# kspalaiologos/bzip3

Hardware: AMD Instinct MI355X
Metric: MiB/s encode+decode round-trip, 8 MiB blocks (higher is better)
Workload: dtype u8

## Files before the change

### bzip3_amd/__init__.py

```python
import ctypes as C
import os

_HERE = os.path.dirname(os.path.abspath(__file__))
LIB_PATH = os.path.join(_HERE, "lib", "libbzip3.so")

BZ3_OK = 0
BZ3_ERR_OUT_OF_BOUNDS = -1
BZ3_ERR_BWT = -2
BZ3_ERR_CRC = -3
BZ3_ERR_MALFORMED_HEADER = -4
BZ3_ERR_TRUNCATED_DATA = -5
BZ3_ERR_DATA_TOO_BIG = -6
BZ3_ERR_INIT = -7
BZ3_ERR_DATA_SIZE_TOO_SMALL = -8

T_NAMES = ["crc", "rle", "lzp", "bwt", "cm", "copy", "_6", "_7"]

_lib = None


def _declare(L, strict=True):
    vp, i32, u32, sz = C.c_void_p, C.c_int32, C.c_uint32, C.c_size_t
    sig = {
        "bz3_version": (C.c_char_p, []),
        "bz3_last_error": (C.c_int8, [vp]),
        "bz3_strerror": (C.c_char_p, [vp]),
        "bz3_new": (vp, [i32]),
        "bz3_free": (None, [vp]),
        "bz3_bound": (sz, [sz]),
        "bz3_compress": (C.c_int, [u32, vp, vp, sz, C.POINTER(sz)]),
        "bz3_decompress": (C.c_int, [vp, vp, sz, C.POINTER(sz)]),
        "bz3_min_memory_needed": (sz, [i32]),
        "bz3_encode_block": (i32, [vp, vp, i32]),
        "bz3_decode_block": (i32, [vp, vp, sz, i32, i32]),
        "bz3_encode_blocks": (None, [vp, vp, vp, i32]),
        "bz3_decode_blocks": (None, [vp, vp, vp, vp, vp, i32]),
        "bz3_orig_size_sufficient_for_decode": (C.c_int, [vp, sz, i32]),
        "bz3_hip_device_count": (C.c_int, []),
        "bz3_hip_bind_device": (C.c_int, [C.c_int]),
        "bz3_hip_state_device": (C.c_int, [vp]),
        "bz3_hip_set_cm_mode": (C.c_int, [C.c_int]),
        "bz3_hip_cm_blocks_given_up": (C.c_uint, []),
        "bz3_hip_cm_blocks_routed_full": (C.c_uint, []),
        "bz3_hip_debug_bwt_big_rounds": (None, [C.c_int]),
        "bz3_hip_debug_peak_concurrent_groups": (C.c_int, [C.c_int]),
        "bz3_hip_debug_front_end_ring": (C.c_int, []),
        "bz3_hip_debug_arena_swap_buffers": (C.c_int, [C.c_int]),
        "bz3_hip_cm_variant_for": (C.c_int, [C.c_int, C.c_int, C.c_int]),
        "bz3_hip_set_lean_states": (C.c_int, [C.c_int]),
        "bz3_hip_release_cached_memory": (None, []),
        "bz3_hip_set_keep_workspace": (C.c_int, [C.c_int]),
        "bz3_hip_set_front_end_duo": (C.c_int, [C.c_int]),
        "bz3_hip_set_workspace_headroom": (None, [C.c_longlong]),
        "bz3_hip_workspace_headroom": (sz, []),
        "bz3_hip_debug_headroom_events": (C.c_uint, [C.c_int, C.POINTER(C.c_uint)]),
        "bz3_hip_debug_ring_contexts": (sz, [sz, sz, sz, sz, sz, sz, C.c_int, sz]),
        "bz3_hip_debug_arena_slack": (sz, [sz]),
        "bz3_hip_debug_cm_launches": (C.c_uint, [C.c_int]),
        "bz3_hip_debug_workspace_bytes": (sz, [sz, C.c_int]),
        "bz3_hip_debug_cached_bytes": (sz, [C.c_int]),
        "bz3_hip_encode_block_device": (i32, [vp, vp, i32]),
        "bz3_hip_decode_block_device": (i32, [vp, vp, sz, i32, i32]),
        "bz3_hip_encode_blocks_device": (None, [vp, vp, vp, i32]),
        "bz3_hip_decode_blocks_device": (None, [vp, vp, vp, vp, vp, i32]),
        "bz3_hip_compress_device": (C.c_int, [u32, vp, vp, sz, C.POINTER(sz)]),
        "bz3_hip_decompress_device": (C.c_int, [vp, vp, sz, C.POINTER(sz)]),
        "bz3_hip_frame_decoded_size_device": (C.c_int, [vp, sz, C.POINTER(sz)]),
        "bz3_hip_compress_device_many": (C.c_int, [u32, i32, C.POINTER(vp), C.POINTER(sz), C.POINTER(vp), C.POINTER(sz), C.POINTER(C.c_int)]),
        "bz3_hip_decompress_device_many": (C.c_int, [i32, C.POINTER(vp), C.POINTER(sz), C.POINTER(vp), C.POINTER(sz), C.POINTER(C.c_int)]),
        "bz3_hip_frame_decoded_sizes_device": (C.c_int, [i32, C.POINTER(vp), C.POINTER(sz), C.POINTER(sz), C.POINTER(C.c_int)]),
        "bz3_hip_debug_copy_segments": (i32, [vp, vp, C.POINTER(C.c_uint64), i32]),
        "bz3_hip_compress_device_planes": (C.c_int, [u32, u32, vp, vp, sz, C.POINTER(sz)]),
        "bz3_hip_decompress_device_planes": (C.c_int, [u32, vp, vp, sz, C.POINTER(sz)]),
        "bz3_hip_compress_device_planes_many": (C.c_int, [u32, i32, C.POINTER(u32), C.POINTER(vp), C.POINTER(sz), C.POINTER(vp), C.POINTER(sz), C.POINTER(C.c_int)]),
        "bz3_hip_decompress_device_planes_many": (C.c_int, [i32, C.POINTER(u32), C.POINTER(vp), C.POINTER(sz), C.POINTER(vp), C.POINTER(sz), C.POINTER(C.c_int)]),
        "bz3_hip_debug_planes": (i32, [vp, vp, C.POINTER(C.c_uint64), i32]),
        "bz3_hip_compress_device_delta": (C.c_int, [u32, u32, vp, vp, vp, sz, C.POINTER(sz)]),
        "bz3_hip_decompress_device_delta": (C.c_int, [u32, vp, vp, sz, vp, sz, C.POINTER(sz)]),
        "bz3_hip_compress_device_delta_many": (C.c_int, [u32, i32, C.POINTER(u32), C.POINTER(vp), C.POINTER(vp), C.POINTER(sz), C.POINTER(vp), C.POINTER(sz), C.POINTER(C.c_int)]),
        "bz3_hip_decompress_device_delta_many": (C.c_int, [i32, C.POINTER(u32), C.POINTER(vp), C.POINTER(sz), C.POINTER(vp), C.POINTER(sz), C.POINTER(vp), C.POINTER(sz), C.POINTER(C.c_int)]),
        "bz3_hip_crc32c_device": (C.c_int, [vp, sz, u32, C.POINTER(u32)]),
        "bz3_hip_debug_delta": (i32, [vp, vp, vp, C.POINTER(C.c_uint64), i32]),
        "bz3_hip_decompress_device_range": (C.c_int, [u32, vp, sz, C.c_uint64, vp, sz, vp, C.POINTER(sz)]),
        "bz3_hip_decompress_device_range_many": (C.c_int, [i32, C.POINTER(u32), C.POINTER(vp), C.POINTER(sz), C.POINTER(C.c_uint64), C.POINTER(vp), C.POINTER(sz),
                                                           C.POINTER(vp), C.POINTER(sz), C.POINTER(C.c_int)]),
        "bz3_hip_debug_range": (i32, [vp, vp, vp, C.POINTER(C.c_uint64), i32]),
        "bz3_hip_last_timings": (None, [vp, C.POINTER(C.c_float)]),
        "bz3_hip_last_bwt_stats": (None, [vp, C.POINTER(i32), C.POINTER(i32), C.POINTER(C.c_uint64)]),
        "bz3_hip_stage_crc32c": (u32, [vp, sz, u32]),
        "bz3_hip_stage_mrle_encode": (i32, [vp, i32, vp]),
        "bz3_hip_stage_mrle_decode": (C.c_int, [vp, vp, i32, i32]),
        "bz3_hip_stage_lzp_encode": (i32, [vp, i32, vp]),
        "bz3_hip_stage_lzp_decode": (i32, [vp, i32, vp, i32]),
        "bz3_hip_stage_bwt": (i32, [vp, vp, i32]),
        "bz3_hip_stage_unbwt": (i32, [vp, vp, i32, i32]),
        "bz3_hip_stage_last_ms": (C.c_float, []),
        "bz3_hip_debug_sort_u32": (i32, [vp, u32, C.c_int, C.c_int, vp, vp]),
        "bz3_hip_debug_scan_u32": (i32, [vp, u32, vp]),
        "bz3_hip_debug_cu_masks": (i32, [C.c_int, C.c_int, vp, vp]),
        "bz3_hip_set_collect_window_us": (None, [C.c_int]),
        "bz3_hip_debug_collected_batches": (C.c_uint, [C.c_int, C.POINTER(C.c_uint)]),
        "bz3_hip_stage_cm_encode": (i32, [vp, i32, vp]),
        "bz3_hip_stage_cm_decode": (None, [vp, i32, vp, i32]),
        "bz3_hip_stage_cm_decode_many": (C.c_float, [vp, i32, vp, i32, i32, vp]),
        "bz3_hip_stage_cm_encode_many": (C.c_float, [vp, i32, vp, C.POINTER(i32), i32]),
        "bz3_hip_encode_stream": (C.c_int, [C.c_int, C.c_int, i32, i32]),
        "bz3_hip_decode_stream": (C.c_int, [C.c_int, C.c_int, i32]),
    }
    for name, (res, args) in sig.items():
        if not strict and not hasattr(L, name):
            continue
        fn = getattr(L, name)
        fn.restype = res
        fn.argtypes = args
    return L


EXPORTED_SYMBOLS = None


def _share_hip_runtime_with_torch():
    if os.environ.get("BZ3_HIP_SYSTEM_RUNTIME") == "1":
        return
    try:
        import importlib.util

        spec = importlib.util.find_spec("torch")
        if spec is None or not spec.origin:
            return
        cand = os.path.join(os.path.dirname(spec.origin), "lib", "libamdhip64.so")
        if os.path.exists(cand):
            C.CDLL(cand, mode=C.RTLD_GLOBAL)
    except Exception:
        pass


def load(path=None):
    global _lib
    if _lib is not None and path is None:
        return _lib
    if path is None:
        _share_hip_runtime_with_torch()
    p = path or LIB_PATH
    if not os.path.exists(p):
        raise RuntimeError(
            f"{p} is missing: the HIP extension has not been built (python -m bzip3_amd.build). "
            "bzip3_amd has no CPU or PyTorch fallback by design."
        )
    L = _declare(C.CDLL(p), strict=path is None)
    if path is None:
        _lib = L
    return L


def _cbuf(data, cap):
    cap = max(1, cap)
    if len(data) == cap:
        return (C.c_uint8 * cap).from_buffer_copy(data)
    buf = (C.c_uint8 * cap)()
    if len(data):
        C.memmove(buf, data if isinstance(data, bytes) else bytes(data), len(data))
    return buf


class StageApi:

    def __init__(self, lib=None):
        self.lib = lib or load()

    def crc32c(self, data, init=1):
        return self.lib.bz3_hip_stage_crc32c(_cbuf(data, len(data)), len(data), init)

    def mrle_encode(self, data):
        out = (C.c_uint8 * (len(data) + 64))()
        n = self.lib.bz3_hip_stage_mrle_encode(_cbuf(data, len(data)), len(data), out)
        return C.string_at(out, n)

    def mrle_decode(self, data, outlen, maxin=None):
        maxin = len(data) if maxin is None else maxin
        out = (C.c_uint8 * max(1, outlen))()
        rc = self.lib.bz3_hip_stage_mrle_decode(_cbuf(data, len(data)), out, outlen, maxin)
        return rc, C.string_at(out, outlen)

    def lzp_encode(self, data):
        out = (C.c_uint8 * (len(data) + 64))()
        n = self.lib.bz3_hip_stage_lzp_encode(_cbuf(data, len(data)), len(data), out)
        return n, (C.string_at(out, n) if n > 0 else b"")

    def lzp_decode(self, data, maxout):
        out = (C.c_uint8 * max(8, maxout))()
        n = self.lib.bz3_hip_stage_lzp_decode(_cbuf(data, len(data)), len(data), out, maxout)
        return n, (C.string_at(out, n) if n > 0 else b"")

    def bwt(self, data):
        out = (C.c_uint8 * max(1, len(data)))()
        idx = self.lib.bz3_hip_stage_bwt(_cbuf(data, len(data)), out, len(data))
        return idx, C.string_at(out, len(data))

    def unbwt(self, data, idx):
        out = (C.c_uint8 * max(1, len(data)))()
        rc = self.lib.bz3_hip_stage_unbwt(_cbuf(data, len(data)), out, len(data), idx)
        return rc, C.string_at(out, len(data))

    def cm_encode(self, data):
        out = (C.c_uint8 * (len(data) + len(data) // 50 + 64))()
        n = self.lib.bz3_hip_stage_cm_encode(_cbuf(data, len(data)), len(data), out)
        return C.string_at(out, n)

    def cm_decode(self, data, n):
        out = (C.c_uint8 * max(1, n))()
        self.lib.bz3_hip_stage_cm_decode(_cbuf(data, len(data)), len(data), out, n)
        return C.string_at(out, n)


class State:

    def __init__(self, block_size, lib=None):
        self.lib = lib or load()
        self.block_size = block_size
        self.ptr = self.lib.bz3_new(block_size)
        if not self.ptr:
            raise RuntimeError(f"bz3_new({block_size}) returned NULL (invalid size, no HIP device, or out of device memory)")

    def close(self):
        if self.ptr:
            self.lib.bz3_free(self.ptr)
            self.ptr = None

    def __del__(self):
        try:
            self.close()
        except Exception:
            pass

    def __enter__(self):
        return self

    def __exit__(self, *a):
        self.close()

    @property
    def last_error(self):
        return self.lib.bz3_last_error(self.ptr)

    def strerror(self):
        return self.lib.bz3_strerror(self.ptr).decode()

    def timings(self):
        t = (C.c_float * 8)()
        self.lib.bz3_hip_last_timings(self.ptr, t)
        return {T_NAMES[i]: t[i] for i in range(6)}

    def bwt_stats(self):
        r, p, e = C.c_int32(), C.c_int32(), C.c_uint64()
        self.lib.bz3_hip_last_bwt_stats(self.ptr, C.byref(r), C.byref(p), C.byref(e))
        return {"rounds": r.value, "radix_passes": p.value, "sorted_elements": e.value}

    def encode_block(self, data):
        cap = self.lib.bz3_bound(max(len(data), self.block_size)) + 64
        buf = _cbuf(data, cap)
        n = self.lib.bz3_encode_block(self.ptr, buf, len(data))
        return n, self.last_error, (C.string_at(buf, n) if n > 0 else b"")

    def decode_block(self, data, orig_size, buffer_size=None, comp_size=None):
        cap = self.lib.bz3_bound(self.block_size) + 64
        buffer_size = cap if buffer_size is None else buffer_size
        comp_size = len(data) if comp_size is None else comp_size
        buf = _cbuf(data, max(cap, buffer_size, len(data) + 1))
        n = self.lib.bz3_decode_block(self.ptr, buf, buffer_size, comp_size, orig_size)
        return n, self.last_error, (C.string_at(buf, n) if n > 0 else b"")


def encode_block(data, block_size, lib=None):
    with State(block_size, lib) as st:
        return st.encode_block(data)


def decode_block(data, orig_size, block_size, lib=None, **kw):
    with State(block_size, lib) as st:
        return st.decode_block(data, orig_size, **kw)


class Bz3Error(RuntimeError):

    def __init__(self, code, what, out=None, index=None, codes=None, outs=None):
        super().__init__(f"{what} failed with {code} ({_ERR_NAMES.get(code, 'unknown error')})" + ("" if index is None else f" at frame {index}"))
        self.code = code
        self.out = out
        self.index = index
        self.codes = codes
        self.outs = outs


_ERR_NAMES = {v: k for k, v in globals().items() if k.startswith("BZ3_ERR_")}


def _device_u8(x, what):
    import torch

    if not isinstance(x, torch.Tensor) or x.device.type != "cuda" or x.dtype != torch.uint8 or not x.is_contiguous():
        raise TypeError(f"{what} must be a contiguous torch.uint8 tensor on a GPU")
    return x


def _planes_arg(planes, n):
    ks = [int(planes)] * n if isinstance(planes, int) else [int(k) for k in planes]
    if len(ks) != n:
        raise ValueError(f"planes: {len(ks)} element sizes for {n} tensors")
    for k in ks:
        if k not in (1, 2, 4, 8):
            raise ValueError(f"planes must be 1, 2, 4 or 8, not {k}")
    return ks


def _base_u8(base, x, what, same_size=True):
    if base is None:
        return None
    base = _device_u8(base, what)
    if base.device != x.device:
        raise ValueError(f"{what} is on {base.device}, the tensor on {x.device}")
    if same_size and base.numel() != x.numel():
        raise ValueError(f"{what} holds {base.numel()} bytes, the tensor {x.numel()}")
    return base


def _bases_arg(bases, n):
    bases = [None] * n if bases is None else list(bases)
    if len(bases) != n:
        raise ValueError(f"bases: {len(bases)} entries for {n} tensors")
    return bases


def _ptrs_or_null(ts):
    return (C.c_void_p * len(ts))(*[None if t is None else t.data_ptr() for t in ts])


def compress_tensor(x, block_size=16 << 20, lib=None, planes=1, base=None):
    import torch

    x = _device_u8(x, "x")
    (k,) = _planes_arg(planes, 1)
    base = _base_u8(base, x, "base")
    L = lib or load()
    n = x.numel()
    out = torch.empty(L.bz3_bound(n), dtype=torch.uint8, device=x.device)
    size = C.c_size_t(out.numel())
    torch.cuda.synchronize(x.device)
    rc = L.bz3_hip_compress_device_delta(block_size, k, C.c_void_p(x.data_ptr()), None if base is None else C.c_void_p(base.data_ptr()),
                                         C.c_void_p(out.data_ptr()), n, C.byref(size))
    if rc != BZ3_OK:
        raise Bz3Error(rc, "bz3_hip_compress_device_delta")
    return out[: size.value]


def decompress_tensor(frame, out=None, lib=None, planes=1, base=None):
    import torch

    frame = _device_u8(frame, "frame")
    (k,) = _planes_arg(planes, 1)
    base = _base_u8(base, frame, "base", same_size=False)
    L = lib or load()
    torch.cuda.synchronize(frame.device)
    if out is None:
        need = C.c_size_t(0)
        L.bz3_hip_frame_decoded_size_device(C.c_void_p(frame.data_ptr()), frame.numel(), C.byref(need))
        out = torch.empty(need.value, dtype=torch.uint8, device=frame.device)
    else:
        out = _device_u8(out, "out")
    size = C.c_size_t(out.numel())
    rc = L.bz3_hip_decompress_device_delta(k, C.c_void_p(frame.data_ptr()), None if base is None else C.c_void_p(base.data_ptr()),
                                           0 if base is None else base.numel(), C.c_void_p(out.data_ptr()), frame.numel(), C.byref(size))
    if rc != BZ3_OK:
        raise Bz3Error(rc, "bz3_hip_decompress_device_delta", out[: size.value])
    return out[: size.value]


def _same_device(ts, what):
    dev = ts[0].device
    for t in ts:
        if t.device != dev:
            raise ValueError(f"{what}: all tensors must be on one GPU ({dev} and {t.device})")
    return dev


def _ptrs(ts):
    return (C.c_void_p * len(ts))(*[t.data_ptr() for t in ts])


def _carve(total, sizes, device):
    import torch

    offs, o = [], 0
    for n in sizes:
        offs.append(o)
        o += (n + 15) & ~15
    buf = torch.empty(max(o, 1), dtype=torch.uint8, device=device)
    return [buf[a : a + n] for a, n in zip(offs, sizes)]


def _compress_many(L, xs, block_sizes, ks, dev, slack=False, bases=None):
    import torch

    n = len(xs)
    bases = _bases_arg(bases, n)
    caps = [L.bz3_bound(x.numel()) + ((13 + 8 * (x.numel() // _KiB65 + 2) + 15) & ~15 if slack else 0) for x in xs]
    outs = _carve(sum(caps), caps, dev)
    frames, codes = [None] * n, [BZ3_OK] * n
    torch.cuda.synchronize(dev)
    for bs in sorted(set(block_sizes)):
        idx = [i for i in range(n) if block_sizes[i] == bs]
        g = len(idx)
        out_sizes = (C.c_size_t * g)(*[caps[i] for i in idx])
        rcs = (C.c_int * g)()
        L.bz3_hip_compress_device_delta_many(bs, g, (C.c_uint32 * g)(*[ks[i] for i in idx]), _ptrs([xs[i] for i in idx]), _ptrs_or_null([bases[i] for i in idx]),
                                             (C.c_size_t * g)(*[xs[i].numel() for i in idx]), _ptrs([outs[i] for i in idx]), out_sizes, rcs)
        for j, i in enumerate(idx):
            frames[i], codes[i] = outs[i][: out_sizes[j]], rcs[j]
    if any(c != BZ3_OK for c in codes):
        idx = next(i for i, c in enumerate(codes) if c != BZ3_OK)
        raise Bz3Error(codes[idx], "bz3_hip_compress_device_delta_many", index=idx, codes=codes, outs=frames)
    return frames


def compress_tensors(xs, block_size=16 << 20, lib=None, planes=1, bases=None):
    xs = [_device_u8(x, f"xs[{i}]") for i, x in enumerate(xs)]
    if not xs:
        return []
    ks = _planes_arg(planes, len(xs))
    bases = [_base_u8(b, x, f"bases[{i}]") for i, (b, x) in enumerate(zip(_bases_arg(bases, len(xs)), xs))]
    dev = _same_device(xs, "compress_tensors")
    return _compress_many(lib or load(), xs, [block_size] * len(xs), ks, dev, bases=bases)


def decompress_tensors(frames, outs=None, lib=None, planes=1, bases=None):
    import torch

    frames = [_device_u8(f, f"frames[{i}]") for i, f in enumerate(frames)]
    if not frames:
        return []
    ks = _planes_arg(planes, len(frames))
    bases = [_base_u8(b, f, f"bases[{i}]", same_size=False) for i, (b, f) in enumerate(zip(_bases_arg(bases, len(frames)), frames))]
    dev = _same_device(frames, "decompress_tensors")
    L = lib or load()
    n = len(frames)
    in_ptrs = _ptrs(frames)
    in_sizes = (C.c_size_t * n)(*[f.numel() for f in frames])
    torch.cuda.synchronize(dev)
    if outs is None:
        need = (C.c_size_t * n)()
        rcs = (C.c_int * n)()
        L.bz3_hip_frame_decoded_sizes_device(n, in_ptrs, in_sizes, need, rcs)
        outs = _carve(sum(need), list(need), dev)
    else:
        outs = [_device_u8(o, f"outs[{i}]") for i, o in enumerate(outs)]
        if len(outs) != n:
            raise ValueError(f"decompress_tensors: {n} frames and {len(outs)} outputs")
        _same_device(frames + outs, "decompress_tensors")
    out_sizes = (C.c_size_t * n)(*[o.numel() for o in outs])
    rcs = (C.c_int * n)()
    rc = L.bz3_hip_decompress_device_delta_many(n, (C.c_uint32 * n)(*ks), in_ptrs, in_sizes, _ptrs_or_null(bases),
                                                (C.c_size_t * n)(*[0 if b is None else b.numel() for b in bases]), _ptrs(outs), out_sizes, rcs)
    res = [o[: out_sizes[i]] for i, o in enumerate(outs)]
    if rc != BZ3_OK:
        codes = list(rcs)
        idx = next(i for i, c in enumerate(codes) if c != BZ3_OK)
        raise Bz3Error(rc, "bz3_hip_decompress_device_delta_many", index=idx, codes=codes, outs=res)
    return res


def decompress_tensors_range(frames, offsets, nbytes, outs=None, planes=1, bases=None, lib=None):
    import torch

    frames = [_device_u8(f, f"frames[{i}]") for i, f in enumerate(frames)]
    n = len(frames)
    offsets, nbytes = [int(o) for o in offsets], [int(w) for w in nbytes]
    if len(offsets) != n or len(nbytes) != n:
        raise ValueError(f"decompress_tensors_range: {n} frames, {len(offsets)} offsets and {len(nbytes)} sizes")
    if any(o < 0 for o in offsets) or any(w < 0 for w in nbytes):
        raise ValueError("decompress_tensors_range: offsets and sizes must not be negative")
    if not frames:
        return []
    ks = _planes_arg(planes, n)
    bases = [_base_u8(b, f, f"bases[{i}]", same_size=False) for i, (b, f) in enumerate(zip(_bases_arg(bases, n), frames))]
    dev = _same_device(frames, "decompress_tensors_range")
    L = lib or load()
    if outs is None:
        outs = _carve(sum(nbytes), nbytes, dev)
    else:
        outs = [_device_u8(o, f"outs[{i}]") for i, o in enumerate(outs)]
        if len(outs) != n:
            raise ValueError(f"decompress_tensors_range: {n} frames and {len(outs)} outputs")
        _same_device(frames + outs, "decompress_tensors_range")
    for i, (o, b, w) in enumerate(zip(outs, bases, nbytes)):
        if o.numel() < w or (b is not None and b.numel() < w):
            raise ValueError(f"decompress_tensors_range: outs[{i}] / bases[{i}] hold fewer than the {w} bytes asked for")
    torch.cuda.synchronize(dev)
    out_sizes = (C.c_size_t * n)(*nbytes)
    rcs = (C.c_int * n)()
    rc = L.bz3_hip_decompress_device_range_many(n, (C.c_uint32 * n)(*ks), _ptrs(frames), (C.c_size_t * n)(*[f.numel() for f in frames]), (C.c_uint64 * n)(*offsets),
                                                _ptrs_or_null(bases), (C.c_size_t * n)(*[0 if b is None else w for b, w in zip(bases, nbytes)]), _ptrs(outs), out_sizes, rcs)
    res = [o[: out_sizes[i]] for i, o in enumerate(outs)]
    if rc != BZ3_OK:
        codes = list(rcs)
        idx = next(i for i, c in enumerate(codes) if c != BZ3_OK)
        raise Bz3Error(rc, "bz3_hip_decompress_device_range_many", index=idx, codes=codes, outs=res)
# ... 285 lines not shown
```

### bzip3_amd/csrc/api.hip

```cpp
#include <atomic>
#include <chrono>
#include <condition_variable>
#include <cstdio>
#include <cstdlib>
#include <exception>
#include <mutex>
#include <new>
#include <stdexcept>
#include <thread>
#include <type_traits>
#include <vector>

#include "../../include/bz3_hip.h"
#include "frame.hpp"
#include "planes.hpp"
#include "prims.hpp"
#include "sort.hpp"
#include "stages.hpp"

using namespace bz3;

namespace {

constexpr s32 KiB65 = 65 * 1024;
// ... 193 lines not shown
__attribute__((constructor)) static void bz3_hip_on_load() {
    const char * e = getenv("BZ3_HIP_SET_HW_QUEUES");
    if (!e || atoi(e) != 0) (void)setenv("GPU_MAX_HW_QUEUES", "8", 0);
}
#endif

int device_count() {
    std::lock_guard<std::mutex> lk(g_mu);
    if (g_device_count < 0) {
        int n = 0;
        if (hipGetDeviceCount(&n) != hipSuccess) n = 0;
        g_device_count = n;
        g_ctx.assign((size_t)(n > 0 ? n : 0), nullptr);
    }
    return g_device_count;
}

DeviceCtx * get_ctx(int dev) {
    const int n = device_count();
    if (dev < 0 || dev >= n) return nullptr;
    std::lock_guard<std::mutex> lk(g_mu);
    if (!g_ctx[dev]) {
        HIP_CHECK(hipSetDevice(dev));
        DeviceCtx * c = new DeviceCtx;
        c->device = dev;
        CrcTables t;
        memset(&t, 0, sizeof t);
        crc_build_tables(t);
        HIP_CHECK(hipMalloc((void **)&c->d_crc, sizeof(CrcTables)));
        HIP_CHECK(hipMemcpy(c->d_crc, &t, sizeof t, hipMemcpyHostToDevice));
#ifndef BZ3_EMU
        int cus = 0;
        if (hipDeviceGetAttribute(&cus, hipDeviceAttributeMultiprocessorCount, dev) == hipSuccess && cus > 0) c->cus = cus;
#endif
        if (const char * e = getenv("BZ3_HIP_CUS"))
            if (atoi(e) > 0) c->cus = atoi(e);
        g_ctx[dev] = c;
    }
    return g_ctx[dev];
}

int pick_device() {
    const int n = device_count();
    if (n <= 0) return -1;
    int b = g_bound_device.load();
    if (b == -2) {
        const char * e = getenv("BZ3_HIP_DEVICE");
        b = (e && *e) ? atoi(e) : -1;
        if (b >= n) b = -1;
        g_bound_device.store(b);
    }
    if (b >= 0) return b;
    return (int)(g_rr.fetch_add(1) % (unsigned)n);
}

size_t front_a_scratch_bytes(u64 n) { return (size_t)n * 30 + radix_temp_bytes(n, 9) + scan_temp_words(n / 8 + 4096) * 4 + (4u << 20); }
size_t front_b_scratch_bytes(u64 n) { return bwt_workspace_bytes(n) + (size_t)(n / 1024 + 4096) * 4; }
size_t workspace_bytes_for(u64 n) {
    size_t a = bwt_workspace_bytes(n), b = unbwt_workspace_bytes(n);
    size_t c = (size_t)n * 30 + radix_temp_bytes(n, 9) + scan_temp_words(n / 8 + 4096) * 4 + (4u << 20);
    size_t m = a > b ? a : b;
    return m > c ? m : c;
}

std::atomic<int> g_cm_mode{-2};

int cm_mode() {
    int m = g_cm_mode.load();
    if (m == -2) {
        const char * e = getenv("BZ3_HIP_CM_MODE");
        m = -1;
        if (e && !strcmp(e, "full")) m = CM_VARIANT_FULL;
        else if (e && !strcmp(e, "rows")) m = CM_VARIANT_ROWS;
        else if (e && !strcmp(e, "rows3")) m = CM_VARIANT_ROWS3;
#ifdef BZ3_EMU
        else if (e && !strcmp(e, "rows-test")) m = CM_VARIANT_ROWS_TEST;
#endif
        g_cm_mode.store(m);
    }
    return m;
}

bool lean_states() {
    int v = g_lean.load();
    if (v < 0) {
        const char * e = getenv("BZ3_HIP_LEAN");
        v = (e && *e && strcmp(e, "0")) ? 1 : 0;
        g_lean.store(v);
    }
    return v != 0;
}

int cm_variant_for(const DeviceCtx * ctx, size_t njobs, bool encode) {
    (void)encode;
    const int m = cm_mode();
    const size_t c = (size_t)ctx->cus;
    if (m >= 0) return m;
    if (njobs > 2 * c) return CM_VARIANT_ROWS3;
    if (njobs > c) return CM_VARIANT_ROWS;
    return CM_VARIANT_FULL;
}

size_t cm_scratch_bytes(size_t njobs) { return njobs * (CM_SPILL_BYTES + 256) + 4096 + CM_CLAIM_WORDS * 4 + 256; }

template <class Job, class Launch>
float run_cm_jobs(const DeviceCtx * ctx, Arena & arena, std::vector<Job> & jobs, Job * d_jobs, hipStream_t s, hipEvent_t ev0, hipEvent_t ev1, Launch && go,
                  const std::vector<char> * to_full = nullptr) {
    if (jobs.empty()) return 0.f;
    std::vector<Job> direct;
    if (to_full && cm_mode() < 0 && cm_variant_has_rows(cm_variant_for(ctx, jobs.size(), std::is_same<Job, CmEncodeJob>::value))) {
        std::vector<Job> keep;
        for (size_t i = 0; i < jobs.size(); i++) ((*to_full)[i] ? direct : keep).push_back(jobs[i]);
        if (!direct.empty()) {
            g_cm_routed_full.fetch_add((unsigned)direct.size());
            jobs.swap(keep);
        }
    }
    if (jobs.empty()) {
        float ms0 = 0.f;
        HIP_CHECK(hipMemcpyAsync(d_jobs, direct.data(), sizeof(Job) * direct.size(), hipMemcpyHostToDevice, s));
        HIP_CHECK(hipEventRecord(ev0, s));
        g_cm_launches.fetch_add(1);
        go(d_jobs, (u32)direct.size(), s, (int)CM_VARIANT_FULL);
        HIP_CHECK(hipEventRecord(ev1, s));
        HIP_CHECK(hipStreamSynchronize(s));
        (void)hipEventElapsedTime(&ms0, ev0, ev1);
        jobs.swap(direct);
        return ms0;
    }
    const int variant = cm_variant_for(ctx, jobs.size(), std::is_same<Job, CmEncodeJob>::value);
    const size_t mk = arena.mark();
    if constexpr (std::is_same<Job, CmEncodeJob>::value) {
        static const bool no_claim = getenv("BZ3_CM_NO_CLAIM") != nullptr;
        if (!no_claim) {
            u32 * claim = arena.take<u32>(CM_CLAIM_WORDS);
            HIP_CHECK(hipMemsetAsync(claim, 0, CM_CLAIM_WORDS * sizeof(u32), s));
            for (auto & j : jobs) j.claim = dev_addr(claim);
            for (auto & j : direct) j.claim = dev_addr(claim);
        }
    }
    u32 * d_status = nullptr;
    if (cm_variant_has_rows(variant)) {
        u8 * spill = arena.take<u8>(jobs.size() * CM_SPILL_BYTES);
        d_status = arena.take<u32>(jobs.size());
        HIP_CHECK(hipMemsetAsync(d_status, 0, jobs.size() * 4, s));
        for (size_t i = 0; i < jobs.size(); i++) {
            jobs[i].spill = dev_addr(spill + i * CM_SPILL_BYTES);
            jobs[i].status = dev_addr(d_status + i);
            jobs[i].miss_base = cm_variant_is_test(variant) ? 64u : CM_MISS_BASE;
            jobs[i].miss_shift = cm_variant_is_test(variant) ? 3u : CM_MISS_SHIFT;
        }
    }
    float ms = 0.f, ms2 = 0.f;
    HIP_CHECK(hipMemcpyAsync(d_jobs, jobs.data(), sizeof(Job) * jobs.size(), hipMemcpyHostToDevice, s));
    HIP_CHECK(hipEventRecord(ev0, s));
    g_cm_launches.fetch_add(1);
    go(d_jobs, (u32)jobs.size(), s, variant);
    HIP_CHECK(hipEventRecord(ev1, s));
    HIP_CHECK(hipStreamSynchronize(s));
    (void)hipEventElapsedTime(&ms, ev0, ev1);
    if (cm_variant_has_rows(variant)) {
        std::vector<u32> status(jobs.size());
        HIP_CHECK(hipMemcpyAsync(status.data(), d_status, jobs.size() * 4, hipMemcpyDeviceToHost, s));
        HIP_CHECK(hipStreamSynchronize(s));
        std::vector<Job> again;
        for (size_t i = 0; i < jobs.size(); i++)
            if (status[i]) again.push_back(jobs[i]);
        g_cm_given_up.fetch_add((unsigned)again.size());
        again.insert(again.end(), direct.begin(), direct.end());
        direct.clear();
        if (!again.empty()) {
            HIP_CHECK(hipMemcpyAsync(d_jobs, again.data(), sizeof(Job) * again.size(), hipMemcpyHostToDevice, s));
            HIP_CHECK(hipEventRecord(ev0, s));
            g_cm_launches.fetch_add(1);
            go(d_jobs, (u32)again.size(), s, (int)CM_VARIANT_FULL);
            HIP_CHECK(hipEventRecord(ev1, s));
            HIP_CHECK(hipStreamSynchronize(s));
            (void)hipEventElapsedTime(&ms2, ev0, ev1);
        }
    }
    if (!direct.empty()) {
        HIP_CHECK(hipMemcpyAsync(d_jobs, direct.data(), sizeof(Job) * direct.size(), hipMemcpyHostToDevice, s));
        HIP_CHECK(hipEventRecord(ev0, s));
        g_cm_launches.fetch_add(1);
        go(d_jobs, (u32)direct.size(), s, (int)CM_VARIANT_FULL);
        HIP_CHECK(hipEventRecord(ev1, s));
        HIP_CHECK(hipStreamSynchronize(s));
        float ms3 = 0.f;
        (void)hipEventElapsedTime(&ms3, ev0, ev1);
        ms2 += ms3;
    }
    arena.release(mk);
    return ms + ms2;
}

__global__ void k_write_header(u8 * __restrict__ b, const u32 * __restrict__ crc, const u32 * __restrict__ idx_word, u32 model, u32 lzp_size, u32 rle_size) {
    if (threadIdx.x != 0) return;
    const u32 c = *crc, idx = *idx_word;
    b[0] = (u8)c; b[1] = (u8)(c >> 8); b[2] = (u8)(c >> 16); b[3] = (u8)(c >> 24);
    b[4] = (u8)idx; b[5] = (u8)(idx >> 8); b[6] = (u8)(idx >> 16); b[7] = (u8)(idx >> 24);
    b[8] = (u8)model;
    u32 o = 9;
    if (model & 2u) { b[o] = (u8)lzp_size; b[o + 1] = (u8)(lzp_size >> 8); b[o + 2] = (u8)(lzp_size >> 16); b[o + 3] = (u8)(lzp_size >> 24); o += 4; }
    if (model & 4u) { b[o] = (u8)rle_size; b[o + 1] = (u8)(rle_size >> 8); b[o + 2] = (u8)(rle_size >> 16); b[o + 3] = (u8)(rle_size >> 24); }
}

__global__ void __launch_bounds__(64) k_store_small(u8 * __restrict__ b, u32 n, const u32 * __restrict__ crc) {
    const u32 t = threadIdx.x;
    const u8 v = t < n ? b[t] : (u8)0;
    __syncthreads();
    if (t < n) b[8 + t] = v;
    if (t == 0) {
        const u32 c = *crc;
        b[0] = (u8)c; b[1] = (u8)(c >> 8); b[2] = (u8)(c >> 16); b[3] = (u8)(c >> 24);
        b[4] = b[5] = b[6] = b[7] = 0xFF;
    }
}
__global__ void __launch_bounds__(128) k_unstore_small(u8 * __restrict__ b, u32 n) {
    const u32 t = threadIdx.x;
    const u8 v = t < n ? b[8 + t] : (u8)0;
    __syncthreads();
    if (t < n) b[t] = v;
}

}

struct bz3_state {
    s32 block_size = 0;
    s8 last_error = BZ3_OK;
    int device = 0;
    DeviceCtx * ctx = nullptr;
    hipStream_t stream = nullptr;
    hipStream_t xs = nullptr;
    u8 * d_swap = nullptr;
    bool lean = false;
    bool timed = true;
    u8 * d_io = nullptr;
    size_t cap = 0;
    u32 * d_words = nullptr;
    hipEvent_t ev0 = nullptr, ev1 = nullptr;
    float t[BZ3_HIP_T_COUNT] = {0};
    BwtStats bwt;

    enum Pending { NONE, ENC_STORED, ENC_CODED, DEC_STORED, DEC_CODED, FAILED } pending = NONE;
    u8 * user = nullptr;
    u8 * b1 = nullptr, * b2 = nullptr;
    s32 size = 0, overhead = 0, result = -1;
    u32 n_cm = 0;
    const u8 * cm_in = nullptr;
    u32 cm_in_size = 0;
    u8 * side = nullptr;
    bool hold_swap = false;
    bool skip = false;
    size_t buffer_size = 0;
    u32 crc = 0;
    s32 bwt_idx = 0, model = 0, lzp_size = -1, rle_size = -1, orig_size = 0, size_before_bwt = 0, size_src = 0;
};

namespace {

struct DeviceGuard {
    explicit DeviceGuard(int d) { HIP_CHECK(hipSetDevice(d)); }
};

struct DrainOnUnwind {
    hipStream_t main;
    hipStream_t * side;
    int n_side;
    int live = std::uncaught_exceptions();
    ~DrainOnUnwind() {
        if (std::uncaught_exceptions() > live) {
            if (main) (void)hipStreamSynchronize(main);
            for (int k = 0; k < n_side; k++)
                if (side[k]) (void)hipStreamSynchronize(side[k]);
        }
    }
};

void state_release(bz3_state * st) {
    if (!st) return;
    (void)hipSetDevice(st->device);
    if (st->stream) (void)hipStreamSynchronize(st->stream);
    if (st->ev0) (void)hipEventDestroy(st->ev0);
    if (st->ev1) (void)hipEventDestroy(st->ev1);
    if (st->d_swap && st->lean && st->ctx) st->ctx->temp_put(st->d_swap);
    else if (st->d_swap) (void)hipFree(st->d_swap);
    if (st->d_io) (void)hipFree(st->d_io);
    if (st->d_words) (void)hipFree(st->d_words);
    if (st->stream) (void)hipStreamDestroy(st->stream);
    delete st;
}

void ensure_io(bz3_state * st) {
    if (!st->d_io) HIP_CHECK(hipMalloc((void **)&st->d_io, st->cap));
}

u32 read_word(hipStream_t s, const u32 * d) {
    u32 v = 0;
    HIP_CHECK(hipMemcpyAsync(&v, d, 4, hipMemcpyDeviceToHost, s));
    HIP_CHECK(hipStreamSynchronize(s));
    return v;
}

inline bool sizes_fit(size_t buffer_size, s32 lzp_size, s32 rle_size, s32 orig_size) {
    const size_t a = lzp_size < 0 ? 0 : (size_t)lzp_size, b = rle_size < 0 ? 0 : (size_t)rle_size, c = orig_size < 0 ? 0 : (size_t)orig_size;
    return a <= buffer_size && b <= buffer_size && c <= buffer_size;
}

std::atomic<long long> g_ws_headroom{-1};
inline size_t ws_headroom() {
    static const long long env = [] {
        const char * e = getenv("BZ3_HIP_WS_HEADROOM_MB");
        return e && *e ? (long long)strtoull(e, nullptr, 10) << 20 : (long long)4 << 30;
    }();
    const long long v = g_ws_headroom.load();
    return (size_t)(v < 0 ? env : v);
}
inline size_t ring_contexts_for(size_t free_b, size_t have, size_t need, size_t fixed, size_t ctx_bytes, size_t cap, bool lean, size_t headroom) {
    const size_t total = free_b + have;
    const size_t base = need + fixed;
    if (total <= base || !ctx_bytes) return 0;
    size_t by_share = (total - base) / 10 * 7 / ctx_bytes;
    const size_t aside = headroom + ((size_t)513 << 20) + ((size_t)64 << 20);
    const size_t room = total > base + aside ? total - base - aside : 0;
    if (!lean) {
        const size_t by_room = room / ctx_bytes;
        return by_share < by_room ? by_share : by_room;
    }
    return room / (ctx_bytes + cap);
}
void enforce_headroom(DeviceCtx * ctx, hipStream_t s);

#ifndef BZ3_FRONT_DUO_DEFAULT
#define BZ3_FRONT_DUO_DEFAULT 0
#endif
std::atomic<int> g_keep_ws{-1};
inline bool keep_workspace() {
    static const bool env_on = [] {
        const char * e = getenv("BZ3_HIP_KEEP_WS");
        return e && atoi(e) != 0;
    }();
    const int v = g_keep_ws.load();
    return v < 0 ? env_on : v != 0;
}
std::atomic<int> g_front_duo{-1};
inline bool front_end_duo() {
    static const int env_on = [] {
        const char * e = getenv("BZ3_HIP_FRONT_DUO");
        return e ? (atoi(e) != 0 ? 1 : 0) : BZ3_FRONT_DUO_DEFAULT;
    }();
    const int v = g_front_duo.load();
    return v < 0 ? env_on != 0 : v != 0;
}
inline void lean_borrow(bz3_state * st) {
    if (st->lean && !st->d_swap) st->d_swap = st->ctx->temp_get(st->cap);
}
inline void lean_return(bz3_state * st) {
    if (st->lean && st->d_swap) {
        st->ctx->temp_put(st->d_swap);
        st->d_swap = nullptr;
    }
}
constexpr u32 CM_SIDE_BYTES = 64 * 1024;

void encode_front_a(bz3_state * st, u8 * buf, s32 data_size, Arena & arena, Arena & ctx_arena, LzpEncodeCtx & c) {
    st->pending = bz3_state::FAILED;
    st->result = -1;
    c.active = false;
    if (st->skip) return;
    if (data_size > st->block_size || data_size < 0) {
        st->last_error = BZ3_ERR_DATA_TOO_BIG;
        return;
    }
    hipStream_t s = st->xs;
    for (float & x : st->t) x = 0.f;
    double t0 = now_ms();
    crc32c_device(buf, (u64)data_size, 1u, st->ctx->d_crc, st->d_words, s);
    st->user = buf;
    st->size = data_size;
    if (data_size < 64) {
        launch(k_store_small, dim3(1), dim3(64), 0, s, buf, (u32)data_size, (const u32 *)(st->d_words + 1));
        st->pending = bz3_state::ENC_STORED;
        return;
    }
    if (st->timed) {
        HIP_CHECK(hipStreamSynchronize(s));
        st->t[BZ3_HIP_T_CRC] = (float)(now_ms() - t0);
    }

    u32 n = (u32)data_size;
    lean_borrow(st);
    u8 *b1 = buf, *b2 = st->d_swap;
    st->model = 0;
    st->rle_size = 0;
    t0 = now_ms();
    {
        MrleEncScratch sc;
        const size_t mk = arena.mark();
        mrle_encode_size(b1, n, sc, arena, s);
        st->rle_size = (s32)(32u + read_word(s, sc.total));
        if (st->rle_size < (s32)n) {
            mrle_encode_write(b1, n, sc, b2, s);
            if (st->timed) HIP_CHECK(hipStreamSynchronize(s));
            u8 * tmp = b1; b1 = b2; b2 = tmp;
            n = (u32)st->rle_size;
            st->model |= 4;
        }
        arena.release(mk);
    }
    st->t[BZ3_HIP_T_RLE] = (float)(now_ms() - t0);
    st->b1 = b1;
    st->b2 = b2;
    st->n_cm = n;
    t0 = now_ms();
    lzp_encode_prepare(b1, n, c, ctx_arena, arena, s);
    st->t[BZ3_HIP_T_LZP] = (float)(now_ms() - t0);
    st->pending = bz3_state::ENC_CODED;
}

void encode_front_b(bz3_state * st, Arena & arena, const LzpEncodeCtx & c, float driver_ms) {
    if (st->pending != bz3_state::ENC_CODED) return;
    st->pending = bz3_state::FAILED;
    hipStream_t s = st->xs;
    u8 *b1 = st->b1, *b2 = st->b2;
    u32 n = st->n_cm;
    double t0 = now_ms();
    const s32 lzp_size = lzp_encode_finish(c, b2, arena, s);
    if (lzp_size > 0 && lzp_size < (s32)n) {
        u8 * tmp = b1; b1 = b2; b2 = tmp;
        n = (u32)lzp_size;
        st->model |= 2;
    }
    st->lzp_size = lzp_size;
    st->t[BZ3_HIP_T_LZP] += driver_ms + (float)(now_ms() - t0);

    t0 = now_ms();
    u32 * const d_idx = st->d_words + 6;
    u32 * const d_out8 = st->d_words + 8;
    if (!st->lean) {
        (void)bwt_forward(b1, n, b2, arena, s, &st->bwt, d_idx, d_out8);
    } else {
        u8 * tail = st->user + bz3_bound((size_t)st->size) - n;
        if (b1 != st->user) {
            (void)bwt_forward(b1, n, tail, arena, s, &st->bwt, d_idx, d_out8);
        } else {
            (void)bwt_forward(b1, n, b2, arena, s, &st->bwt, d_idx, d_out8);
            HIP_CHECK(hipMemcpyAsync(tail, b2, n, hipMemcpyDeviceToDevice, s));
        }
        b1 = st->user;
        b2 = tail;
    }
    if (st->timed) {
        HIP_CHECK(hipStreamSynchronize(s));
        st->t[BZ3_HIP_T_BWT] = (float)(now_ms() - t0);
    }
    s32 overhead = 2;
    if (st->model & 2) overhead++;
    if (st->model & 4) overhead++;
    launch(k_write_header, dim3(1), dim3(64), 0, s, b1, (const u32 *)(st->d_words + 1), (const u32 *)d_idx, (u32)st->model, (u32)lzp_size, (u32)st->rle_size);
    if (st->lean && !st->hold_swap) lean_return(st);
    st->b1 = b1;
    st->b2 = b2;
    st->n_cm = n;
    st->overhead = overhead;
    st->pending = bz3_state::ENC_CODED;
}

void encode_finish(bz3_state * st, float cm_ms) {
    const bz3_state::Pending p = st->pending;
    st->pending = bz3_state::NONE;
    if (p == bz3_state::FAILED || p == bz3_state::NONE) return;
    HIP_CHECK(hipStreamSynchronize(st->xs));
    if (p == bz3_state::ENC_STORED) {
        st->result = st->size + 8;
        return;
    }
    st->t[BZ3_HIP_T_CM] = cm_ms;
    const u32 coded = read_word(st->xs, st->d_words + 2);
    if (coded == 0xFFFFFFFFu) {
        st->last_error = BZ3_ERR_BWT;
        return;
    }
    const s32 total = (s32)coded + st->overhead * 4 + 1;
    if (st->lean) {
        const u32 sw = read_word(st->xs, st->d_words + 3);
        if (sw != 0xFFFFFFFFu && coded > sw)
            HIP_CHECK(hipMemcpyAsync(st->user + st->overhead * 4 + 1 + sw, st->side, coded - sw, hipMemcpyDeviceToDevice, st->xs));
        HIP_CHECK(hipStreamSynchronize(st->xs));
    }
    st->last_error = BZ3_OK;
    if (st->b1 != st->user) {
        double t0 = now_ms();
        HIP_CHECK(hipMemcpyAsync(st->user, st->b1, (size_t)total, hipMemcpyDeviceToDevice, st->xs));
        HIP_CHECK(hipStreamSynchronize(st->xs));
        st->t[BZ3_HIP_T_COPY] += (float)(now_ms() - t0);
    }
    st->result = total;
}

std::atomic<unsigned> g_headroom_trims{0}, g_headroom_releases{0};
void enforce_headroom(DeviceCtx * ctx, hipStream_t s) {
    const size_t h = ws_headroom();
    size_t free_b = 0, total_b = 0;
    if (!h || hipMemGetInfo(&free_b, &total_b) != hipSuccess || free_b >= h) return;
    if (ctx->temp_idle_bytes() > 0) {
        ctx->temp_trim();
        g_headroom_trims.fetch_add(1);
        if (hipMemGetInfo(&free_b, &total_b) != hipSuccess || free_b >= h) return;
    }
    if (ctx->ws) {
        (void)hipStreamSynchronize(s);
        (void)hipDeviceSynchronize();
        (void)hipFree(ctx->ws);
        ctx->ws = nullptr;
        ctx->ws_cap = 0;
        g_headroom_releases.fetch_add(1);
    }
}

void pipeline_shape(s32 contexts, s32 n, s32 & window, s32 & ns) {
    if (contexts < 2) contexts = 2;
    ns = 2;
    for (s32 cand = DeviceCtx::RING_SLOTS; cand > 2; cand--)
        if (contexts / cand >= 3 && n >= cand * 3) {
            ns = cand;
            break;
        }
    window = contexts / ns;
    if (window > 8) window = 8;
    if (const char * e = getenv("BZ3_HIP_LZP_PIPE")) {
        int w = 0, q = 0;
        if (sscanf(e, "%d,%d", &w, &q) == 2 && w >= 1 && q >= 2 && q <= DeviceCtx::AUX) {
            window = w;
            ns = q;
        }
    }
    if (window > n) window = n;
    if (window < 1) window = 1;
}

void encode_group(bz3_state ** sts, u8 ** bufs, const s32 * sizes, s32 n) {
    if (n <= 0) return;
    bz3_state * lead = sts[0];
    DeviceGuard g(lead->device);
    std::lock_guard<std::mutex> lk(lead->ctx->mu);
    for (s32 i = 0; i < n; i++) {
        sts[i]->xs = lead->stream;
        sts[i]->timed = i == 0;
    }
    size_t need = 0, need_a = 0, need_b = 0;
    for (s32 i = 0; i < n; i++) {
        const u64 nb = (u64)(sizes[i] > 0 ? sizes[i] : 0) + 64;
        const size_t w = workspace_bytes_for(nb), wa = front_a_scratch_bytes(nb), wb = front_b_scratch_bytes(nb);
        if (w > need) need = w;
        if (wa > need_a) need_a = wa;
        if (wb > need_b) need_b = wb;
    }
    const bool duo_wanted = front_end_duo() && n >= 16;
    if (duo_wanted) need = need_a + need_b + 65536;
    u64 n_max = 64;
    for (s32 i = 0; i < n; i++)
        if (sizes[i] > 0 && (u64)sizes[i] > n_max) n_max = (u64)sizes[i];
    const size_t ctx_bytes = lzp_encode_ctx_bytes(n_max + 64) + 65536;
    const size_t headroom = ws_headroom();
    const size_t fixed = (size_t)n * (sizeof(CmEncodeJob) + CM_SIDE_BYTES + 256) + cm_scratch_bytes((size_t)n) + 65536 + (size_t)DeviceCtx::AUX * 8 * (sizeof(LzpDriverJob) + 256);
    size_t contexts = ((size_t)32 << 30) / ctx_bytes;
    {
        size_t free_b = 0, total_b = 0;
        const s32 full = DeviceCtx::RING_SLOTS * 8;
        if (lead->lean && lead->ctx->temp_idle_bytes() > 0 && hipMemGetInfo(&free_b, &total_b) == hipSuccess) {
            if (ring_contexts_for(free_b, lead->ctx->ws_cap, need, fixed, ctx_bytes, lead->cap, true, headroom) < (size_t)(n < full ? n : full)) lead->ctx->temp_trim();
        }
        if (hipMemGetInfo(&free_b, &total_b) == hipSuccess)
            contexts = ring_contexts_for(free_b, lead->ctx->ws_cap, need, fixed, ctx_bytes, lead->cap, lead->lean, headroom);
    }
    s32 window = 1, ns = 2;
    pipeline_shape((s32)(contexts < 1024 ? contexts : 1024), n, window, ns);
    lead->ctx->ensure_aux();
    hipStream_t s = lead->stream;
    DrainOnUnwind drain{s, lead->ctx->aux, DeviceCtx::AUX};
    static const bool front_rest = [] { const char * e = getenv("BZ3_HIP_FRONT_REST"); return e && atoi(e) != 0; }();
    if (front_rest && lead->ctx->rest && n > 1) {
        s = lead->ctx->rest;
        for (s32 i = 0; i < n; i++) sts[i]->xs = s;
    }
    DrainOnUnwind drain_rest{s == lead->stream ? nullptr : s, nullptr, 0};
    Arena arena;
    for (;;) {
        try {
            arena = lead->ctx->arena_for(need + (size_t)ns * (size_t)window * (ctx_bytes + sizeof(LzpDriverJob) + 256) +
                                         (size_t)n * (sizeof(CmEncodeJob) + CM_SIDE_BYTES + 256) + cm_scratch_bytes((size_t)n) + 65536);
            break;
        } catch (const HipError &) {
            if (ns == 2 && window == 1) throw;
            (void)hipGetLastError();
            if (ns > 2) ns = 2;
            else window = (window + 1) / 2;
        }
    }
    g_front_end_ring.store(window | (ns << 16));
    CmEncodeJob * d_jobs = arena.take<CmEncodeJob>((size_t)n);
    u8 * sides = arena.take<u8>((size_t)n * CM_SIDE_BYTES);
    struct Window {
        s32 w0 = 0, w1 = 0;
        Arena slot;
        LzpDriverJob * d_lz = nullptr;
        std::vector<LzpEncodeCtx> ctxs;
        std::vector<LzpDriverJob> lz;
    } win[DeviceCtx::AUX];
    for (int k = 0; k < ns; k++) {
        win[k].slot.base = arena.take<char>((size_t)window * ctx_bytes);
        win[k].slot.cap = (size_t)window * ctx_bytes;
        win[k].d_lz = arena.take<LzpDriverJob>((size_t)window);
    }
    std::vector<CmEncodeJob> jobs;
    std::vector<s32> job_owner;
    const s32 nwin = (n + window - 1) / window;
    const s32 lag = ns - 1;
    static const bool trace_rings = getenv("BZ3_HIP_TRACE_RINGS") != nullptr;
    double tr_prep = 0, tr_wait = 0, tr_fin = 0, tr_t0 = now_ms();
    auto prepare = [&](s32 k, hipStream_t sp, Arena & scr, hipEvent_t ev) {
        const int q = (int)(k % ns);
        Window & w = win[q];
        w.w0 = k * window;
        w.w1 = (w.w0 + window < n) ? w.w0 + window : n;
        w.slot.used = 0;
        w.ctxs.assign((size_t)(w.w1 - w.w0), LzpEncodeCtx());
        w.lz.clear();
        for (s32 i = w.w0; i < w.w1; i++) {
            sts[i]->xs = sp;
            sts[i]->hold_swap = false;
            encode_front_a(sts[i], bufs[i], sizes[i], scr, w.slot, w.ctxs[(size_t)(i - w.w0)]);
            if (sts[i]->pending == bz3_state::ENC_CODED && w.ctxs[(size_t)(i - w.w0)].active) w.lz.push_back(lzp_driver_job(w.ctxs[(size_t)(i - w.w0)]));
        }
        HIP_CHECK(hipEventRecord(ev, sp));
        if (!w.lz.empty()) {
            hipStream_t sq = lead->ctx->aux[q];
            HIP_CHECK(hipStreamWaitEvent(sq, ev, 0));
            HIP_CHECK(hipEventRecord(lead->ctx->ev_d0[q], sq));
            lzp_driver_batch(w.lz.data(), w.d_lz, (u32)w.lz.size(), sq);
            HIP_CHECK(hipEventRecord(lead->ctx->ev_d1[q], sq));
        }
    };
    auto finish = [&](s32 j, hipStream_t sf, Arena & scr, std::vector<bz3_state *> * held) {
        const int q = (int)(j % ns);
        Window & w = win[q];
        float driver_ms = 0.f;
        if (!w.lz.empty()) {
            const double t0 = now_ms();
            HIP_CHECK(hipEventSynchronize(lead->ctx->ev_d1[q]));
            (void)hipEventElapsedTime(&driver_ms, lead->ctx->ev_d0[q], lead->ctx->ev_d1[q]);
            tr_wait += now_ms() - t0;
        }
        for (s32 i = w.w0; i < w.w1; i++) {
            sts[i]->xs = sf;
            sts[i]->hold_swap = held != nullptr;
            encode_front_b(sts[i], scr, w.ctxs[(size_t)(i - w.w0)], driver_ms);
            sts[i]->hold_swap = false;
            if (sts[i]->pending == bz3_state::ENC_CODED) {
                CmEncodeJob j2{dev_addr(sts[i]->b2), dev_addr(sts[i]->b1 + sts[i]->overhead * 4 + 1), dev_addr(sts[i]->d_words + 2), sts[i]->n_cm, 0u};
                if (sts[i]->lean) {
                    sts[i]->side = sides + (size_t)i * CM_SIDE_BYTES;
                    j2.gap = (u32)(sts[i]->b2 - (sts[i]->b1 + sts[i]->overhead * 4 + 1));
                    j2.side = dev_addr(sts[i]->side);
                    j2.side_cap = CM_SIDE_BYTES;
                }
                jobs.push_back(j2);
                job_owner.push_back(i);
            }
            if (held) {
                if (sts[i]->lean && sts[i]->d_swap) held->push_back(sts[i]);
            } else {
                lean_return(sts[i]);
            }
        }
    };
    const bool duo = duo_wanted && nwin >= 3 && lead->ctx->aux_ready && s == lead->stream;
    if (!duo) {
        for (s32 k = 0; k < nwin + lag; k++) {
            const double tr_a = now_ms();
            if (k < nwin) prepare(k, s, arena, lead->ctx->ev_prep);
            const double tr_b = now_ms();
            tr_prep += tr_b - tr_a;
            if (k >= lag) finish(k - lag, s, arena, nullptr);
            tr_fin += now_ms() - tr_b;
        }
    } else {
        g_front_end_ring.fetch_or(1 << 29);
        hipStream_t sA = lead->ctx->duo;
        DrainOnUnwind drain_duo{sA, nullptr, 0};
        Arena scr_a;
        scr_a.base = arena.take<char>(need_a);
        scr_a.cap = need_a;
        struct Events {
            std::vector<hipEvent_t> e;
            ~Events() {
                for (hipEvent_t x : e)
                    if (x) (void)hipEventDestroy(x);
            }
        } evs;
        evs.e.assign((size_t)2 * (size_t)nwin, nullptr);
        for (auto & x : evs.e) HIP_CHECK(hipEventCreateWithFlags(&x, hipEventDisableTiming));
        hipEvent_t * evA = evs.e.data(), * evB = evs.e.data() + nwin;
        struct Shared {
            std::mutex m;
            std::condition_variable cv;
            s32 prepared = 0, finished = 0;
            bool abort = false;
            std::exception_ptr err;
            std::mutex pool;
            hipEvent_t last_return = nullptr;
            double prep_ms = 0;
        } sh;
        const int device = lead->device;
        std::thread ta([&] {
            try {
                DeviceGuard gd(device);
                for (s32 k = 0; k < nwin; k++) {
                    {
                        std::unique_lock<std::mutex> ul(sh.m);
                        sh.cv.wait(ul, [&] { return sh.abort || sh.finished >= k - ns + 1; });
                        if (sh.abort) return;
                    }
                    const double t0 = now_ms();
                    if (k >= ns) HIP_CHECK(hipStreamWaitEvent(sA, evB[k - ns], 0));
                    {
                        hipEvent_t ev = nullptr;
                        const s32 w0 = k * window, w1 = (w0 + window < n) ? w0 + window : n;
                        {
                            std::lock_guard<std::mutex> pl(sh.pool);
                            for (s32 i = w0; i < w1; i++) lean_borrow(sts[i]);
                            ev = sh.last_return;
                        }
                        if (ev) HIP_CHECK(hipStreamWaitEvent(sA, ev, 0));
                    }
                    prepare(k, sA, scr_a, evA[k]);
                    {
                        std::lock_guard<std::mutex> ul(sh.m);
                        sh.prepared = k + 1;
                        sh.prep_ms += now_ms() - t0;
                    }
                    sh.cv.notify_all();
                }
            } catch (...) {
                {
                    std::lock_guard<std::mutex> ul(sh.m);
                    sh.err = std::current_exception();
                    sh.abort = true;
                }
                sh.cv.notify_all();
            }
        });
        struct Joiner {
            std::thread & t;
            Shared & sh;
            int live = std::uncaught_exceptions();
            ~Joiner() {
                if (std::uncaught_exceptions() > live) {
                    std::lock_guard<std::mutex> ul(sh.m);
                    sh.abort = true;
                }
                sh.cv.notify_all();
                if (t.joinable()) t.join();
            }
        } joiner{ta, sh};
        std::vector<bz3_state *> held;
        for (s32 j = 0; j < nwin; j++) {
            const double tr_b = now_ms();
            {
                std::unique_lock<std::mutex> ul(sh.m);
                sh.cv.wait(ul, [&] { return sh.abort || sh.prepared >= j + 1; });
                if (sh.abort) break;
            }
            HIP_CHECK(hipStreamWaitEvent(s, evA[j], 0));
            held.clear();
            finish(j, s, arena, &held);
            HIP_CHECK(hipEventRecord(evB[j], s));
            {
                std::lock_guard<std::mutex> pl(sh.pool);
                for (bz3_state * st : held) lean_return(st);
                sh.last_return = evB[j];
            }
            {
                std::lock_guard<std::mutex> ul(sh.m);
                sh.finished = j + 1;
            }
            sh.cv.notify_all();
            tr_fin += now_ms() - tr_b;
        }
        ta.join();
        if (sh.err) std::rethrow_exception(sh.err);
        HIP_CHECK(hipStreamSynchronize(sA));
        tr_prep = sh.prep_ms;
        for (s32 i = 0; i < n; i++) sts[i]->xs = s;
    }
    if (trace_rings)
        fprintf(stderr, "[bz3 rings] encode front end: %d blocks, %d windows of %d x %d slots: %.1f ms = CRC / mRLE / LZP prepare %.1f + waiting for a window's LZP drivers %.1f + LZP emit / BWT / header %.1f\n",
                (int)n, (int)nwin, (int)window, (int)ns, now_ms() - tr_t0, tr_prep, tr_wait, tr_fin - tr_wait);
    if (s != lead->stream) {
        HIP_CHECK(hipStreamSynchronize(s));
        s = lead->stream;
        for (s32 i = 0; i < n; i++) sts[i]->xs = s;
    }
    std::vector<char> to_full(jobs.size(), 0);
    if (jobs.size() > (size_t)lead->ctx->cus) {
        std::vector<u32> outside(jobs.size(), 0u);
        for (size_t k = 0; k < jobs.size(); k++) HIP_CHECK(hipMemcpyAsync(&outside[k], sts[job_owner[k]]->d_words + 8, 4, hipMemcpyDeviceToHost, lead->stream));
        HIP_CHECK(hipStreamSynchronize(lead->stream));
        for (size_t k = 0; k < jobs.size(); k++) to_full[k] = outside[k] > jobs[k].n / 4u ? 1 : 0;
    }
    const float cm_ms = run_cm_jobs(lead->ctx, arena, jobs, d_jobs, lead->stream, lead->ev0, lead->ev1,
                                    [](const CmEncodeJob * j, u32 nj, hipStream_t st, int variant) { cm_encode_batch(j, nj, st, variant); }, &to_full);
    for (s32 i = 0; i < n; i++) encode_finish(sts[i], cm_ms);
    size_t slack = (size_t)16 << 30;
    if (const char * e = getenv("BZ3_HIP_WS_KEEP_MB")) slack = (size_t)strtoull(e, nullptr, 10) << 20;
    if (lead->ctx->ws_cap > 2 * need + slack && !(keep_workspace() && lead->lean)) {
        HIP_CHECK(hipStreamSynchronize(s));
        (void)hipFree(lead->ctx->ws);
        lead->ctx->ws = nullptr;
        lead->ctx->ws_cap = 0;
        g_front_end_ring.fetch_or(1 << 30);
    }
    enforce_headroom(lead->ctx, lead->stream);
}

void decode_front(bz3_state * st, u8 * buf, size_t buffer_size, s32 compressed_size, s32 orig_size, const u8 * hdr) {
    st->pending = bz3_state::FAILED;
    st->result = -1;
    if (st->skip) return;
    if (buffer_size < 9 || buffer_size < (size_t)compressed_size) {
        st->last_error = BZ3_ERR_DATA_SIZE_TOO_SMALL;
        return;
    }
    const u32 crc = rd_le32(hdr);
    const s32 bwt_idx = (s32)rd_le32(hdr + 4);
    const size_t bound = bz3_bound((size_t)st->block_size);
    if (compressed_size < 0 || (size_t)compressed_size > bound) {
        st->last_error = BZ3_ERR_MALFORMED_HEADER;
        return;
    }
    hipStream_t s = st->xs;
    for (float & x : st->t) x = 0.f;
    st->user = buf;
    st->buffer_size = buffer_size;
    st->crc = crc;
    if (bwt_idx == -1) {
        if (compressed_size - 8 > 64 || compressed_size < 8) {
            st->last_error = BZ3_ERR_MALFORMED_HEADER;
            return;
        }
        if ((size_t)(compressed_size - 8) > buffer_size) {
            st->last_error = BZ3_ERR_DATA_SIZE_TOO_SMALL;
            return;
        }
        st->size = compressed_size - 8;
        launch(k_unstore_small, dim3(1), dim3(128), 0, s, buf, (u32)st->size);
        crc32c_device(buf, (u64)st->size, 1u, st->ctx->d_crc, st->d_words, s);
        st->pending = bz3_state::DEC_STORED;
        return;
    }
    const s32 model = (s8)hdr[8];
    const size_t need = 9 + (size_t)((model & 2) * 4) + (size_t)((model & 4) * 4);
    if (buffer_size < need) {
        st->last_error = BZ3_ERR_DATA_SIZE_TOO_SMALL;
        return;
    }
    s32 lzp_size = -1, rle_size = -1, p = 0;
    if (model & 2) lzp_size = (s32)rd_le32(hdr + 9 + 4 * p++);
    if (model & 4) rle_size = (s32)rd_le32(hdr + 9 + 4 * p++);
    p += 2;
    compressed_size -= p * 4 + 1;
    if (((model & 2) && (lzp_size < 0 || (size_t)lzp_size > bound)) || ((model & 4) && (rle_size < 0 || (size_t)rle_size > bound))) {
        st->last_error = BZ3_ERR_MALFORMED_HEADER;
        return;
    }
    if (orig_size < 0 || (size_t)orig_size > bound) {
        st->last_error = BZ3_ERR_MALFORMED_HEADER;
        return;
    }
    const s32 size_before_bwt = (model & 2) ? lzp_size : (model & 4) ? rle_size : orig_size;
    if (!sizes_fit(buffer_size, lzp_size, rle_size, orig_size)) {
        st->last_error = BZ3_ERR_DATA_SIZE_TOO_SMALL;
        return;
    }
    st->bwt_idx = bwt_idx;
    st->model = model;
    st->lzp_size = lzp_size;
    st->rle_size = rle_size;
    st->orig_size = orig_size;
    st->size_before_bwt = size_before_bwt;
    st->cm_in = buf + p * 4 + 1;
    st->cm_in_size = (u32)(compressed_size < 0 ? 0 : compressed_size);
    st->pending = bz3_state::DEC_CODED;
}

bool decode_unbwt(bz3_state * st, Arena & arena, float cm_ms) {
    hipStream_t s = st->xs;
    st->t[BZ3_HIP_T_CM] = cm_ms;
    const s32 n = st->size_before_bwt;
    if (st->bwt_idx > n) {
        st->last_error = BZ3_ERR_MALFORMED_HEADER;
        return false;
    }
    u8 *b1 = st->d_swap, *b2 = st->user;
    if (st->lean) {
        b1 = st->user;
        b2 = st->d_swap;
    }
    const double t0 = now_ms();
    if (n <= 1) {
        if (st->bwt_idx != n) { st->last_error = BZ3_ERR_BWT; return false; }
        if (n == 1) HIP_CHECK(hipMemcpyAsync(b2, b1, 1, hipMemcpyDeviceToDevice, s));
    } else {
        if (st->bwt_idx <= 0) { st->last_error = BZ3_ERR_BWT; return false; }
        bwt_inverse(b1, (u32)n, (u32)st->bwt_idx, b2, arena, s);
    }
    st->b1 = b2;
    st->b2 = b1;
    st->size_src = n;
    st->t[BZ3_HIP_T_BWT] = (float)(now_ms() - t0);
    return true;
}

void decode_finish(bz3_state * st, Arena & arena) {
    hipStream_t s = st->xs;
    const size_t bound = bz3_bound((size_t)st->block_size);
    (void)bound;
    u8 *b1 = st->b1, *b2 = st->b2;
    s32 size_src = st->size_src;
    if (st->model & 2) {
        size_src = (s32)read_word(s, st->d_words + 5);
        if (size_src == -1) { st->last_error = BZ3_ERR_CRC; return; }
        if ((size_t)size_src > st->buffer_size) { st->last_error = BZ3_ERR_DATA_SIZE_TOO_SMALL; return; }
        u8 * tmp = b1; b1 = b2; b2 = tmp;
    }
    if (st->model & 4) {
        const double t0 = now_ms();
        bool bad = size_src < 32;
        if (!bad) {
            mrle_decode(b1, (u32)size_src, b2, (u32)st->orig_size, st->d_words + 4, arena, s);
            bad = read_word(s, st->d_words + 4) != (u32)st->orig_size;
        }
        st->t[BZ3_HIP_T_RLE] = (float)(now_ms() - t0);
        if (bad) { st->last_error = BZ3_ERR_CRC; return; }
        size_src = st->orig_size;
        u8 * tmp = b1; b1 = b2; b2 = tmp;
    }
    st->last_error = BZ3_OK;
    if (size_src > st->block_size || size_src < 0) {
        st->last_error = BZ3_ERR_MALFORMED_HEADER;
        return;
    }
    if (b1 != st->user) {
        const double t0 = now_ms();
        HIP_CHECK(hipMemcpyAsync(st->user, b1, (size_t)size_src, hipMemcpyDeviceToDevice, s));
        HIP_CHECK(hipStreamSynchronize(s));
        st->t[BZ3_HIP_T_COPY] += (float)(now_ms() - t0);
    }
    const double t0 = now_ms();
    crc32c_device(st->user, (u64)size_src, 1u, st->ctx->d_crc, st->d_words, s);
    const u32 got = read_word(s, st->d_words + 1);
    st->t[BZ3_HIP_T_CRC] = (float)(now_ms() - t0);
    if (got != st->crc) {
        st->last_error = BZ3_ERR_CRC;
        return;
    }
    st->result = size_src;
}

void decode_group(bz3_state ** sts, u8 ** bufs, const size_t * buffer_sizes, const s32 * sizes, const s32 * orig_sizes, const u8 * hdrs, s32 n) {
    if (n <= 0) return;
    bz3_state * lead = sts[0];
    DeviceGuard g(lead->device);
    std::lock_guard<std::mutex> lk(lead->ctx->mu);
    hipStream_t s = lead->stream;
    for (s32 i = 0; i < n; i++) sts[i]->xs = s;
    size_t need = 0;
    bool any_lean = false;
    for (s32 i = 0; i < n; i++) {
        const size_t w = workspace_bytes_for(bz3_bound((size_t)sts[i]->block_size) + 64);
        if (w > need) need = w;
        any_lean = any_lean || sts[i]->lean;
    }
    std::vector<s32> coded;
    for (s32 i = 0; i < n; i++) {
        decode_front(sts[i], bufs[i], buffer_sizes[i], sizes[i], orig_sizes[i], hdrs + 17 * (size_t)i);
        if (sts[i]->pending == bz3_state::DEC_CODED) coded.push_back(i);
    }
    auto stage_bytes = [&](s32 i) { return sts[i]->lean ? (((size_t)sts[i]->cm_in_size + 64 + 255) & ~(size_t)255) : (size_t)0; };
    size_t stage_budget = (size_t)48 << 30;
    {
        size_t free_b = 0, total_b = 0;
        if (any_lean && hipMemGetInfo(&free_b, &total_b) == hipSuccess) {
            const size_t have = lead->ctx->ws_cap;
            const size_t aside = need + ws_headroom() + ((size_t)577 << 20);
            const size_t room = free_b + have > aside ? free_b + have - aside : 0;
            stage_budget = room - room / 4;
        }
    }
    std::vector<size_t> round_end;
    size_t max_round = 0;
    for (size_t k = 0; k < coded.size();) {
        size_t bytes = 0, e = k;
        while (e < coded.size() && (e == k || bytes + stage_bytes(coded[e]) <= stage_budget)) bytes += stage_bytes(coded[e++]);
        round_end.push_back(e);
        if (bytes > max_round) max_round = bytes;
        k = e;
    }
    s32 tail_slots = n >= 128 ? 4 : 2;
    s32 tail_window = tail_slots == 4 ? 16 : 32;
    if (tail_slots == 4) {
        size_t cap_max = 0;
        for (s32 i = 0; i < n; i++)
            if (sts[i]->lean && sts[i]->cap > cap_max) cap_max = sts[i]->cap;
        const size_t cap_al = (cap_max + 255) & ~(size_t)255;
        size_t free_b = 0, total_b = 0;
        const bool have_info = hipMemGetInfo(&free_b, &total_b) == hipSuccess;
        for (s32 w : {30, 25, 20}) {
            if (n < 4 * w || lead->ctx->reserved_cus_wanted() < 64) continue;
            const size_t bufs = (size_t)4 * (size_t)w;
            const bool from_arena = keep_workspace() && any_lean && lead->ctx->ws_cap >= need + need / 16 + bufs * cap_al + ((size_t)64 << 20);
            if (!any_lean || from_arena || (have_info && free_b >= bufs * cap_max + ws_headroom() + ((size_t)2 << 30) + max_round)) {
                tail_window = w;
                break;
            }
        }
    }
    lead->ctx->ensure_aux();
    if (const char * e = getenv("BZ3_HIP_TAIL_PIPE")) {
        int w = 0, q = 0;
        if (sscanf(e, "%d,%d", &w, &q) == 2 && w >= 1 && q >= 2 && q <= DeviceCtx::AUX) {
            tail_window = w;
            tail_slots = q;
        }
    }
    if (tail_window > n) tail_window = n;
    size_t lzp_in_window = 0;
    for (s32 w0 = 0; w0 < n; w0 += tail_window) {
        size_t c = 0;
        for (s32 i = w0; i < n && i < w0 + tail_window; i++)
            if (sts[i]->pending == bz3_state::DEC_CODED && (sts[i]->model & 2)) c++;
        if (c > lzp_in_window) lzp_in_window = c;
    }
    Arena arena = lead->ctx->arena_for(need + (size_t)tail_slots * lzp_in_window * (LZP_LUT_WORDS * 4 + sizeof(LzpDecodeJob) + 256) + (size_t)n * 256 + cm_scratch_bytes(coded.size()) + max_round + 65536);
    float cm_ms = 0.f;
    for (size_t r = 0, k0 = 0; r < round_end.size(); k0 = round_end[r++]) {
        const size_t mk = arena.mark();
        std::vector<CmDecodeJob> cm_jobs;
        std::vector<char> to_full;
        for (size_t k = k0; k < round_end[r]; k++) {
            bz3_state * st = sts[coded[k]];
            to_full.push_back((u64)st->cm_in_size * 10u >= (u64)(u32)st->size_before_bwt * 9u ? 1 : 0);
            const u8 * in = st->cm_in;
            if (st->lean) {
                u8 * stage = arena.take<u8>(stage_bytes(coded[k]));
                if (st->cm_in_size) HIP_CHECK(hipMemcpyAsync(stage, st->cm_in, st->cm_in_size, hipMemcpyDeviceToDevice, s));
                in = stage;
            }
            cm_jobs.push_back(CmDecodeJob{dev_addr(in), dev_addr(st->lean ? st->user : st->d_swap), st->cm_in_size, (u32)st->size_before_bwt, 0u, 0u});
        }
        CmDecodeJob * d_jobs = arena.take<CmDecodeJob>(cm_jobs.size());
        cm_ms += run_cm_jobs(lead->ctx, arena, cm_jobs, d_jobs, s, lead->ev0, lead->ev1,
                             [](const CmDecodeJob * j, u32 nj, hipStream_t st, int variant) { cm_decode_batch(j, nj, st, variant); }, &to_full);
        arena.release(mk);
    }
    struct TailWindow {
        s32 w0 = 0, w1 = 0;
        std::vector<LzpDecodeJob> lz_jobs;
        std::vector<s32> lz_owner;
        std::vector<char> alive;
        LzpDecodeJob * d_lz = nullptr;
        u32 * luts = nullptr;
    } tw[DeviceCtx::AUX];
    for (int k = 0; k < tail_slots; k++) {
        tw[k].d_lz = lzp_in_window ? arena.take<LzpDecodeJob>(lzp_in_window) : nullptr;
        tw[k].luts = lzp_in_window ? arena.take<u32>(lzp_in_window * LZP_LUT_WORDS) : nullptr;
    }
    std::vector<u8 *> arena_swaps;
    size_t swap_cap = 0;
    if (keep_workspace() && any_lean) {
        for (s32 i = 0; i < n; i++)
            if (sts[i]->lean && sts[i]->cap > swap_cap) swap_cap = sts[i]->cap;
        const size_t want = (size_t)tail_slots * (size_t)tail_window;
        const size_t step = (swap_cap + 255) & ~(size_t)255;
        const size_t keep_free = need + need / 32 + 65536;
        while (swap_cap && arena_swaps.size() < want && arena.cap - arena.used >= keep_free + step) arena_swaps.push_back(arena.take<u8>(swap_cap));
    }
    std::vector<char> from_arena((size_t)n, 0);
    auto borrow = [&](s32 i) {
        bz3_state * st = sts[i];
        if (st->lean && !st->d_swap && !arena_swaps.empty() && st->cap <= swap_cap) {
            st->d_swap = arena_swaps.back();
            arena_swaps.pop_back();
            from_arena[(size_t)i] = 1;
            g_arena_swaps.fetch_add(1);
        } else {
            lean_borrow(st);
        }
    };
    auto give_back = [&](s32 i) {
        bz3_state * st = sts[i];
        if (from_arena[(size_t)i]) {
            if (st->d_swap) arena_swaps.push_back(st->d_swap);
            st->d_swap = nullptr;
            from_arena[(size_t)i] = 0;
        } else {
            lean_return(st);
        }
    };
    lead->ctx->ensure_aux();
    DrainOnUnwind drain{s, lead->ctx->aux, DeviceCtx::AUX};
    hipStream_t s_cm = s;
    hipStream_t * side_streams = lead->ctx->aux;
    static const s32 part_min = [] { const char * e = getenv("BZ3_HIP_CU_PARTITION_MIN_BLOCKS"); return e && atoi(e) > 0 ? (s32)atoi(e) : (s32)128; }();
    if (lead->ctx->rest && n >= part_min && tail_slots <= DeviceCtx::RING_SLOTS) {
        side_streams = lead->ctx->aux_m;
        HIP_CHECK(hipStreamSynchronize(s));
        s = lead->ctx->rest;
        for (s32 i = 0; i < n; i++) sts[i]->xs = s;
    }
    DrainOnUnwind drain_rest{s == s_cm ? nullptr : s, side_streams == lead->ctx->aux ? nullptr : side_streams, side_streams == lead->ctx->aux ? 0 : DeviceCtx::AUX};
    const s32 nwin = (n + tail_window - 1) / tail_window;
    const s32 lag = tail_slots - 1;
    static const bool trace_rings = getenv("BZ3_HIP_TRACE_RINGS") != nullptr;
    double tr_unbwt = 0, tr_wait = 0, tr_finish = 0, tr_t0 = now_ms();
    for (s32 k = 0; k < nwin + lag; k++) {
        const double tr_a = now_ms();
        if (k < nwin) {
            const int q = (int)(k % tail_slots);
            hipStream_t s2 = side_streams[q];
            TailWindow & w = tw[q];
            w.w0 = k * tail_window;
            w.w1 = (w.w0 + tail_window < n) ? w.w0 + tail_window : n;
            w.lz_jobs.clear();
            w.lz_owner.clear();
            w.alive.assign((size_t)(w.w1 - w.w0), 0);
            for (s32 i = w.w0; i < w.w1; i++) {
                bz3_state * st = sts[i];
                if (st->pending == bz3_state::DEC_STORED) {
                    HIP_CHECK(hipStreamSynchronize(st->xs));
                    if (read_word(st->xs, st->d_words + 1) != st->crc) st->last_error = BZ3_ERR_CRC;
                    else st->result = st->size;
                    continue;
                }
                if (st->pending != bz3_state::DEC_CODED) continue;
                borrow(i);
                if (!decode_unbwt(st, arena, cm_ms)) continue;
                w.alive[(size_t)(i - w.w0)] = 1;
                if (st->model & 2) {
                    if (st->lzp_size < 4) {
                        st->last_error = BZ3_ERR_CRC;
                        w.alive[(size_t)(i - w.w0)] = 0;
                        continue;
                    }
                    const size_t bound = bz3_bound((size_t)st->block_size);
                    const size_t room = st->lean && st->buffer_size < bound ? st->buffer_size : bound;
                    w.lz_jobs.push_back(LzpDecodeJob{dev_addr(st->b1), dev_addr(st->b2), dev_addr(w.luts + w.lz_jobs.size() * LZP_LUT_WORDS), dev_addr(st->d_words + 5),
                                                     (u32)st->lzp_size, (u32)room});
                    w.lz_owner.push_back(i);
                }
            }
            if (!w.lz_jobs.empty()) {
                HIP_CHECK(hipEventRecord(lead->ctx->ev_prep, s));
                HIP_CHECK(hipStreamWaitEvent(s2, lead->ctx->ev_prep, 0));
                HIP_CHECK(hipEventRecord(lead->ctx->ev_d0[q], s2));
                lzp_decode_batch(w.lz_jobs.data(), w.d_lz, (u32)w.lz_jobs.size(), s2);
                HIP_CHECK(hipEventRecord(lead->ctx->ev_d1[q], s2));
            }
        }
        const double tr_b = now_ms();
        tr_unbwt += tr_b - tr_a;
        if (k >= lag) {
            const int q = (int)((k - lag) % tail_slots);
            TailWindow & w = tw[q];
            if (!w.lz_jobs.empty()) {
                HIP_CHECK(hipEventSynchronize(lead->ctx->ev_d1[q]));
                tr_wait += now_ms() - tr_b;
                float ms = 0.f;
                (void)hipEventElapsedTime(&ms, lead->ctx->ev_d0[q], lead->ctx->ev_d1[q]);
                for (s32 i : w.lz_owner) sts[i]->t[BZ3_HIP_T_LZP] = ms;
                for (size_t j = 0; j < w.lz_jobs.size(); j++) {
                    bz3_state * st = sts[w.lz_owner[j]];
                    const size_t bound = bz3_bound((size_t)st->block_size);
                    if (!st->lean || st->buffer_size >= bound || read_word(s, st->d_words + 5) != w.lz_jobs[j].max_out) continue;
                    u8 * big = st->ctx->temp_get(st->cap);
                    LzpDecodeJob again = w.lz_jobs[j];
                    again.out = dev_addr(big);
                    again.max_out = (u32)bound;
                    again.lut = dev_addr(w.luts);
                    lzp_decode_batch(&again, w.d_lz, 1u, s);
                    HIP_CHECK(hipStreamSynchronize(s));
                    st->ctx->temp_put(big);
                }
            }
            for (s32 i = w.w0; i < w.w1; i++) {
                if (w.alive[(size_t)(i - w.w0)]) decode_finish(sts[i], arena);
                give_back(i);
            }
        }
        tr_finish += now_ms() - tr_b;
    }
    if (trace_rings)
        fprintf(stderr, "[bz3 rings] decode tail: %d blocks, %d windows of %d x %d slots: %.1f ms = inverse BWTs + LZP launches %.1f + waiting for a window's LZP decoders %.1f + mRLE / CRC / hand-back %.1f\n",
                (int)n, (int)nwin, (int)tail_window, (int)tail_slots, now_ms() - tr_t0, tr_unbwt, tr_wait, tr_finish - tr_wait);
    for (s32 i = 0; i < n; i++) sts[i]->pending = bz3_state::NONE;
    if (s != s_cm) (void)hipStreamSynchronize(s);
    enforce_headroom(lead->ctx, s_cm);
}

void on_failure(bz3_state * st) {
    if (st) {
        lean_return(st);
        st->last_error = BZ3_ERR_BWT;
        st->pending = bz3_state::NONE;
        st->result = -1;
    }
}

std::atomic<int> g_groups_running{0}, g_groups_peak{0};

template <typename F>
void for_each_device_group(bz3_state ** states, s32 n, F && f) {
    std::vector<std::vector<s32>> groups;
    std::vector<char> done((size_t)n, 0);
    for (s32 i = 0; i < n; i++) {
        if (done[(size_t)i]) continue;
        groups.emplace_back();
        for (s32 j = i; j < n; j++)
            if (!done[(size_t)j] && states[j]->device == states[i]->device) { groups.back().push_back(j); done[(size_t)j] = 1; }
    }
    auto run = [&](const std::vector<s32> & idx) {
        const int now = g_groups_running.fetch_add(1) + 1;
        int peak = g_groups_peak.load();
        while (now > peak && !g_groups_peak.compare_exchange_weak(peak, now)) {}
        try {
            f(idx);
        } catch (const HipError & e) {
            fprintf(stderr, "bzip3_amd: HIP failure '%s' at %s:%d\n", e.what, e.file, e.line);
            for (s32 j : idx) on_failure(states[j]);
        } catch (...) {
            for (s32 j : idx) on_failure(states[j]);
        }
        g_groups_running.fetch_sub(1);
    };
    std::vector<std::thread> workers;
    struct Joiner {
        std::vector<std::thread> & w;
        ~Joiner() {
            for (std::thread & t : w)
                if (t.joinable()) t.join();
        }
    } joiner{workers};
    size_t spawned = 1;
    for (size_t g = 1; g < groups.size(); g++) {
        try {
            workers.emplace_back(run, std::cref(groups[g]));
        } catch (const std::system_error &) {
            break;
        }
        spawned = g + 1;
    }
    if (!groups.empty()) run(groups[0]);
    for (size_t g = spawned; g < groups.size(); g++) run(groups[g]);
}

void stage_in(bz3_state * st, const void * host, size_t bytes, hipStream_t s) {
    try {
        ensure_io(st);
        if (bytes) HIP_CHECK(hipMemcpyAsync(st->d_io, host, bytes, hipMemcpyHostToDevice, s));
    } catch (...) {
        on_failure(st);
        st->skip = true;
    }
}

void run_encode(bz3_state ** states, void ** buffers, s32 * sizes, s32 n, bool host) {
    for_each_device_group(states, n, [&](const std::vector<s32> & idx) {
        std::vector<bz3_state *> sts;
        std::vector<u8 *> bufs;
        std::vector<s32> szs;
        DeviceGuard g(states[idx[0]]->device);
        hipStream_t s = states[idx[0]]->stream;
        const double t0 = now_ms();
        for (s32 j : idx) {
            bz3_state * st = states[j];
            st->skip = false;
            if (host) stage_in(st, buffers[j], (sizes[j] >= 0 && sizes[j] <= st->block_size) ? (size_t)sizes[j] : 0, s);
            sts.push_back(st);
            bufs.push_back(host ? st->d_io : (u8 *)buffers[j]);
            szs.push_back(sizes[j]);
        }
        if (host) HIP_CHECK(hipStreamSynchronize(s));
        const float in_ms = (float)(now_ms() - t0);
        encode_group(sts.data(), bufs.data(), szs.data(), (s32)idx.size());
        if (!host) return;
        const double t1 = now_ms();
        for (s32 j : idx) {
            bz3_state * st = states[j];
            if (st->result > 0 && !st->skip) HIP_CHECK(hipMemcpyAsync(buffers[j], st->d_io, (size_t)st->result, hipMemcpyDeviceToHost, s));
        }
        HIP_CHECK(hipStreamSynchronize(s));
        const float out_ms = (float)(now_ms() - t1);
        for (s32 j : idx) states[j]->t[BZ3_HIP_T_COPY] += (in_ms + out_ms) / (float)idx.size();
    });
    for (s32 i = 0; i < n; i++) {
        sizes[i] = states[i]->result;
        states[i]->skip = false;
    }
}

void run_decode(bz3_state ** states, void ** buffers, const size_t * buffer_sizes, const s32 * sizes, const s32 * orig_sizes, const u8 * hdrs, s32 n, bool host) {
    for_each_device_group(states, n, [&](const std::vector<s32> & idx) {
        std::vector<bz3_state *> sts;
        std::vector<u8 *> bufs;
        std::vector<size_t> bsz;
        std::vector<s32> csz, osz;
        std::vector<u8> hd;
        DeviceGuard g(states[idx[0]]->device);
        hipStream_t s = states[idx[0]]->stream;
        const double t0 = now_ms();
        for (s32 j : idx) {
            bz3_state * st = states[j];
            st->skip = false;
            if (host) {
                const bool copy_ok = buffer_sizes[j] >= 9 && buffer_sizes[j] >= (size_t)sizes[j] && sizes[j] >= 0 &&
                                     (size_t)sizes[j] <= bz3_bound((size_t)st->block_size);
                stage_in(st, buffers[j], copy_ok ? (size_t)sizes[j] : 0, s);
            }
            sts.push_back(st); bufs.push_back(host ? st->d_io : (u8 *)buffers[j]); bsz.push_back(buffer_sizes[j]); csz.push_back(sizes[j]); osz.push_back(orig_sizes[j]);
            hd.insert(hd.end(), hdrs + 17 * (size_t)j, hdrs + 17 * (size_t)j + 17);
        }
        if (host) HIP_CHECK(hipStreamSynchronize(s));
        const float in_ms = (float)(now_ms() - t0);
        decode_group(sts.data(), bufs.data(), bsz.data(), csz.data(), osz.data(), hd.data(), (s32)idx.size());
        if (!host) return;
        const double t1 = now_ms();
        for (s32 j : idx) {
            bz3_state * st = states[j];
            if (st->result > 0 && !st->skip) HIP_CHECK(hipMemcpyAsync(buffers[j], st->d_io, (size_t)st->result, hipMemcpyDeviceToHost, s));
        }
        HIP_CHECK(hipStreamSynchronize(s));
        const float out_ms = (float)(now_ms() - t1);
        for (s32 j : idx) states[j]->t[BZ3_HIP_T_COPY] += (in_ms + out_ms) / (float)idx.size();
    });
    for (s32 i = 0; i < n; i++) states[i]->skip = false;
}

void fetch_headers(bz3_state ** states, void ** buffers, const size_t * buffer_sizes, s32 n, std::vector<u8> & hdrs) {
    hdrs.assign(17 * (size_t)n, 0);
    for (s32 i = 0; i < n; i++) {
        const size_t take = buffer_sizes[i] < 17 ? buffer_sizes[i] : 17;
        if (take < 9) continue;
        try {
            HIP_CHECK(hipSetDevice(states[i]->device));
            HIP_CHECK(hipMemcpyAsync(hdrs.data() + 17 * (size_t)i, buffers[i], take, hipMemcpyDeviceToHost, states[i]->stream));
            HIP_CHECK(hipStreamSynchronize(states[i]->stream));
        } catch (const HipError &) {
        }
    }
}

bz3_state * new_state_on(int32_t block_size, int dev) {
    if (block_size < KiB65 || block_size > MiB511) return nullptr;
    bz3_state * st = nullptr;
    try {
        DeviceCtx * ctx = get_ctx(dev);
        if (!ctx) return nullptr;
        st = new bz3_state;
        st->block_size = block_size;
        st->device = dev;
        st->ctx = ctx;
        HIP_CHECK(hipSetDevice(dev));
        HIP_CHECK(hipStreamCreateWithFlags(&st->stream, hipStreamNonBlocking));
        st->xs = st->stream;
        HIP_CHECK(hipEventCreate(&st->ev0));
        HIP_CHECK(hipEventCreate(&st->ev1));
        st->cap = (bz3_bound((size_t)block_size) + 4096 + 255) & ~(size_t)255;
        st->lean = lean_states();
        if (!st->lean) HIP_CHECK(hipMalloc((void **)&st->d_swap, st->cap));
        HIP_CHECK(hipMalloc((void **)&st->d_words, 64 * sizeof(u32)));
        st->last_error = BZ3_OK;
        return st;
    } catch (const HipError & e) {
        fprintf(stderr, "bzip3_amd: bz3_new failed: %s (%s:%d)\n", e.what, e.file, e.line);
        state_release(st);
        return nullptr;
    } catch (const std::bad_alloc &) {
        state_release(st);
        return nullptr;
    }
}

}

extern "C" {

BZIP3_API const char * bz3_version(void) { return "1.5.2-mi355x"; }

BZIP3_API int8_t bz3_last_error(struct bz3_state * state) { return state->last_error; }

BZIP3_API size_t bz3_bound(size_t input_size) { return input_size + input_size / 50 + 32; }

BZIP3_API const char * bz3_strerror(struct bz3_state * state) {
    switch (state->last_error) {
        case BZ3_OK: return "No error";
        case BZ3_ERR_OUT_OF_BOUNDS: return "Data index out of bounds";
        case BZ3_ERR_BWT: return "Burrows-Wheeler transform failed";
        case BZ3_ERR_CRC: return "CRC32 check failed";
        case BZ3_ERR_MALFORMED_HEADER: return "Malformed header";
        case BZ3_ERR_TRUNCATED_DATA: return "Truncated data";
        case BZ3_ERR_DATA_TOO_BIG: return "Too much data";
        case BZ3_ERR_DATA_SIZE_TOO_SMALL:
            return "Size of buffer `buffer_size` passed to the block decoder (bz3_decode_block) is too small. See function docs for details.";
        default: return "Unknown error";
    }
}

BZIP3_API struct bz3_state * bz3_new(int32_t block_size) {
    if (block_size < KiB65 || block_size > MiB511) return nullptr;
    const int dev = pick_device();
    if (dev < 0) {
        fprintf(stderr, "bzip3_amd: no HIP device available -- this library has no CPU code path\n");
        return nullptr;
    }
    return new_state_on(block_size, dev);
}

BZIP3_API void bz3_free(struct bz3_state * state) { state_release(state); }

BZIP3_API size_t bz3_min_memory_needed(int32_t block_size) {
    if (block_size < KiB65 || block_size > MiB511) return 0;
    const size_t cap = (bz3_bound((size_t)block_size) + 4096 + 255) & ~(size_t)255;
    return sizeof(bz3_state) + cap + 64 * sizeof(u32);
}

BZIP3_API void bz3_hip_encode_blocks_device(struct bz3_state * states[], void * buffers[], int32_t sizes[], int32_t n) {
    run_encode(states, buffers, sizes, n, false);
}

BZIP3_API void bz3_hip_decode_blocks_device(struct bz3_state * states[], void * buffers[], size_t buffer_sizes[], int32_t sizes[],
                                            int32_t orig_sizes[], int32_t n) {
    std::vector<u8> hdrs;
    fetch_headers(states, buffers, buffer_sizes, n, hdrs);
    run_decode(states, buffers, buffer_sizes, sizes, orig_sizes, hdrs.data(), n, false);
}

BZIP3_API int32_t bz3_hip_encode_block_device(struct bz3_state * st, void * buffer, int32_t size) {
    s32 sz = size;
    run_encode(&st, &buffer, &sz, 1, false);
    return sz;
}

BZIP3_API int32_t bz3_hip_decode_block_device(struct bz3_state * st, void * buffer, size_t buffer_size, int32_t compressed_size,
                                              int32_t orig_size) {
    bz3_hip_decode_blocks_device(&st, &buffer, &buffer_size, &compressed_size, &orig_size, 1);
    return st->result;
}

BZIP3_API void bz3_encode_blocks(struct bz3_state * states[], uint8_t * buffers[], int32_t sizes[], int32_t n) {
    run_encode(states, (void **)buffers, sizes, n, true);
}

BZIP3_API void bz3_decode_blocks(struct bz3_state * states[], uint8_t * buffers[], size_t buffer_sizes[], int32_t sizes[], int32_t orig_sizes[],
                                 int32_t n) {
    std::vector<u8> hdrs(17 * (size_t)n, 0);
    for (s32 i = 0; i < n; i++) memcpy(hdrs.data() + 17 * (size_t)i, buffers[i], buffer_sizes[i] < 17 ? buffer_sizes[i] : 17);
    run_decode(states, (void **)buffers, buffer_sizes, sizes, orig_sizes, hdrs.data(), n, true);
}

namespace {
struct SingleReq {
    bz3_state * st;
    u8 * buffer;
    size_t buffer_size;
    s32 size, orig_size;
    bool done = false;
};
struct Collector {
    std::mutex mu;
    std::condition_variable cv;
    std::vector<SingleReq *> pending[2];
    bool leader[2] = {false, false};
    size_t last_size[2] = {0, 0};
    int lonely[2] = {0, 0};
};
Collector g_collect;
std::atomic<int> g_collect_window_us{200};
std::atomic<unsigned> g_collect_batches{0}, g_collect_largest{0};

void run_collected(int kind, std::vector<SingleReq *> & batch) {
    const s32 n = (s32)batch.size();
    g_collect_batches.fetch_add(1u);
    unsigned big = g_collect_largest.load();
    while ((unsigned)n > big && !g_collect_largest.compare_exchange_weak(big, (unsigned)n)) {}
    std::vector<bz3_state *> sts((size_t)n);
    std::vector<u8 *> bufs((size_t)n);
    std::vector<s32> sizes((size_t)n), orig((size_t)n);
    std::vector<size_t> bsz((size_t)n);
    for (s32 i = 0; i < n; i++) {
        sts[(size_t)i] = batch[(size_t)i]->st;
        bufs[(size_t)i] = batch[(size_t)i]->buffer;
        sizes[(size_t)i] = batch[(size_t)i]->size;
        orig[(size_t)i] = batch[(size_t)i]->orig_size;
        bsz[(size_t)i] = batch[(size_t)i]->buffer_size;
    }
    if (kind == 0) {
        bz3_encode_blocks(sts.data(), bufs.data(), sizes.data(), n);
// ... 893 lines not shown
bool ranges_overlap(const void * a, size_t a_size, const void * b, size_t b_size) {
    const u64 x = (u64)a, y = (u64)b;
    return a_size && b_size && x < y + b_size && y < x + a_size;
}

bool elem_sizes_ok(s32 n, const u32 * elem_sizes) {
    for (s32 i = 0; i < n; i++)
        if (!planes_elem_size_ok(elem_sizes[i])) return false;
    return true;
}

}

BZIP3_API int bz3_hip_compress_device_delta(uint32_t block_size, uint32_t elem_size, const void * in, const void * base, void * out, size_t in_size,
                                            size_t * out_size) {
    if (!planes_elem_size_ok(elem_size)) return BZ3_ERR_INIT;
    const int dev = device_of(out);
    if (dev < 0 || (in_size && device_of(in) != dev)) return BZ3_ERR_INIT;
    if (base && in_size && (device_of(base) != dev || ranges_overlap(out, *out_size, base, in_size) || ranges_overlap(out, *out_size, in, in_size))) return BZ3_ERR_INIT;
    const u8 * ins[1] = {(const u8 *)in};
    const u8 * bases[1] = {(const u8 *)base};
    u8 * outs[1] = {(u8 *)out};
    int rc = BZ3_OK;
    compress_frames(dev, block_size, 1, &elem_size, ins, bases, &in_size, outs, out_size, &rc);
    return rc;
}

BZIP3_API int bz3_hip_compress_device_planes(uint32_t block_size, uint32_t elem_size, const void * in, void * out, size_t in_size, size_t * out_size) {
    return bz3_hip_compress_device_delta(block_size, elem_size, in, nullptr, out, in_size, out_size);
}

BZIP3_API int bz3_hip_compress_device(uint32_t block_size, const void * in, void * out, size_t in_size, size_t * out_size) {
    return bz3_hip_compress_device_planes(block_size, 1, in, out, in_size, out_size);
}

BZIP3_API int bz3_hip_decompress_device_delta(uint32_t elem_size, const void * in, const void * base, size_t base_size, void * out, size_t in_size,
                                              size_t * out_size) {
    if (!planes_elem_size_ok(elem_size)) return BZ3_ERR_INIT;
    if (in_size < 13) return BZ3_ERR_MALFORMED_HEADER;
    const int dev = device_of(in);
    if (dev < 0 || (*out_size && device_of(out) != dev)) return BZ3_ERR_INIT;
    if (base && base_size && (device_of(base) != dev || (base != out && ranges_overlap(out, *out_size, base, base_size)))) return BZ3_ERR_INIT;
    const u8 * ins[1] = {(const u8 *)in};
    const u8 * bases[1] = {(const u8 *)base};
    u8 * outs[1] = {(u8 *)out};
    int rc = BZ3_OK;
    decompress_frames(dev, 1, &elem_size, ins, &in_size, bases, &base_size, outs, out_size, &rc);
    return rc;
}

BZIP3_API int bz3_hip_decompress_device_planes(uint32_t elem_size, const void * in, void * out, size_t in_size, size_t * out_size) {
    return bz3_hip_decompress_device_delta(elem_size, in, nullptr, 0, out, in_size, out_size);
}

BZIP3_API int bz3_hip_decompress_device(const void * in, void * out, size_t in_size, size_t * out_size) {
    return bz3_hip_decompress_device_planes(1, in, out, in_size, out_size);
}

BZIP3_API int bz3_hip_frame_decoded_size_device(const void * in, size_t in_size, size_t * decoded_size) {
    *decoded_size = 0;
    if (in_size < 13) return BZ3_ERR_MALFORMED_HEADER;
    const int dev = device_of(in);
    if (dev < 0) return BZ3_ERR_INIT;
    const u8 * ins[1] = {(const u8 *)in};
    int rc = BZ3_OK;
    decoded_sizes_frames(dev, 1, ins, &in_size, decoded_size, &rc);
    return rc;
}

BZIP3_API int bz3_hip_compress_device_delta_many(uint32_t block_size, int32_t n, const uint32_t elem_sizes[], const void * const ins[], const void * const bases[],
                                                 const size_t in_sizes[], void * const outs[], size_t out_sizes[], int rcs[]) {
    if (n == 0) return BZ3_OK;
    if (n < 0 || !ins || !in_sizes || !outs || !out_sizes || !rcs) return fail_frames(n, rcs, out_sizes, BZ3_ERR_INIT);
    if (elem_sizes && !elem_sizes_ok(n, elem_sizes)) return fail_frames(n, rcs, out_sizes, BZ3_ERR_INIT);
    int dev = frames_device(n, ins, in_sizes, (const void * const *)outs, out_sizes);
    if (dev == -2) return fail_frames(n, rcs, out_sizes, BZ3_ERR_INIT);
    for (s32 i = 0; bases && i < n; i++) {
        if (!bases[i] || !in_sizes[i]) continue;
        if (device_of(bases[i]) != dev || ranges_overlap(outs[i], out_sizes[i], bases[i], in_sizes[i]) || ranges_overlap(outs[i], out_sizes[i], ins[i], in_sizes[i]))
            return fail_frames(n, rcs, out_sizes, BZ3_ERR_INIT);
    }
    compress_frames(dev, block_size, n, elem_sizes, (const u8 * const *)ins, (const u8 * const *)bases, in_sizes, (u8 * const *)outs, out_sizes, rcs);
    return first_error(n, rcs);
}

BZIP3_API int bz3_hip_compress_device_planes_many(uint32_t block_size, int32_t n, const uint32_t elem_sizes[], const void * const ins[], const size_t in_sizes[],
                                                  void * const outs[], size_t out_sizes[], int rcs[]) {
    return bz3_hip_compress_device_delta_many(block_size, n, elem_sizes, ins, nullptr, in_sizes, outs, out_sizes, rcs);
}

BZIP3_API int bz3_hip_compress_device_many(uint32_t block_size, int32_t n, const void * const ins[], const size_t in_sizes[], void * const outs[],
                                           size_t out_sizes[], int rcs[]) {
    return bz3_hip_compress_device_planes_many(block_size, n, nullptr, ins, in_sizes, outs, out_sizes, rcs);
}

BZIP3_API int bz3_hip_decompress_device_delta_many(int32_t n, const uint32_t elem_sizes[], const void * const ins[], const size_t in_sizes[],
                                                   const void * const bases[], const size_t base_sizes[], void * const outs[], size_t out_sizes[], int rcs[]) {
    if (n == 0) return BZ3_OK;
    if (n < 0 || !ins || !in_sizes || !outs || !out_sizes || !rcs || (bases && !base_sizes)) return fail_frames(n, rcs, out_sizes, BZ3_ERR_INIT);
    if (elem_sizes && !elem_sizes_ok(n, elem_sizes)) return fail_frames(n, rcs, out_sizes, BZ3_ERR_INIT);
    const int dev = frames_device(n, ins, in_sizes, (const void * const *)outs, out_sizes);
    if (dev == -2) return fail_frames(n, rcs, out_sizes, BZ3_ERR_INIT);
    for (s32 i = 0; bases && i < n; i++) {
        if (!bases[i] || !base_sizes[i]) continue;
        if (device_of(bases[i]) != dev || (bases[i] != outs[i] && ranges_overlap(outs[i], out_sizes[i], bases[i], base_sizes[i])))
            return fail_frames(n, rcs, out_sizes, BZ3_ERR_INIT);
    }
    decompress_frames(dev, n, elem_sizes, (const u8 * const *)ins, in_sizes, (const u8 * const *)bases, base_sizes, (u8 * const *)outs, out_sizes, rcs);
    return first_error(n, rcs);
}

BZIP3_API int bz3_hip_decompress_device_range_many(int32_t n, const uint32_t elem_sizes[], const void * const ins[], const size_t in_sizes[],
                                                   const uint64_t offsets[], const void * const bases[], const size_t base_sizes[], void * const outs[],
                                                   size_t out_sizes[], int rcs[]) {
    if (n == 0) return BZ3_OK;
    if (n < 0 || !ins || !in_sizes || !outs || !out_sizes || !rcs || (bases && !base_sizes)) return fail_frames(n, rcs, out_sizes, BZ3_ERR_INIT);
    if (elem_sizes && !elem_sizes_ok(n, elem_sizes)) return fail_frames(n, rcs, out_sizes, BZ3_ERR_INIT);
    const int dev = frames_device(n, ins, in_sizes, (const void * const *)outs, out_sizes);
    if (dev == -2) return fail_frames(n, rcs, out_sizes, BZ3_ERR_INIT);
    for (s32 i = 0; bases && i < n; i++) {
        if (!bases[i] || !base_sizes[i]) continue;
        const u64 w = out_sizes[i] < base_sizes[i] ? out_sizes[i] : base_sizes[i], x = (u64)outs[i], y = (u64)bases[i];
        if (device_of(bases[i]) != dev || (x != y && (x > y ? x - y : y - x) < w)) return fail_frames(n, rcs, out_sizes, BZ3_ERR_INIT);
    }
    decompress_frames(dev, n, elem_sizes, (const u8 * const *)ins, in_sizes, (const u8 * const *)bases, base_sizes, (u8 * const *)outs, out_sizes, rcs, true,
                      (const u64 *)offsets);
    return first_error(n, rcs);
}

BZIP3_API int bz3_hip_decompress_device_range(uint32_t elem_size, const void * in, size_t in_size, uint64_t offset, const void * base, size_t base_size, void * out,
                                              size_t * out_size) {
    if (!out_size) return BZ3_ERR_INIT;
    const void * ins[1] = {in};
    const void * bases[1] = {base};
    void * outs[1] = {out};
    int rc = BZ3_OK;
    return bz3_hip_decompress_device_range_many(1, &elem_size, ins, &in_size, &offset, bases, &base_size, outs, out_size, &rc);
}

BZIP3_API int bz3_hip_decompress_device_planes_many(int32_t n, const uint32_t elem_sizes[], const void * const ins[], const size_t in_sizes[], void * const outs[],
                                                    size_t out_sizes[], int rcs[]) {
    return bz3_hip_decompress_device_delta_many(n, elem_sizes, ins, in_sizes, nullptr, nullptr, outs, out_sizes, rcs);
}

BZIP3_API int bz3_hip_decompress_device_many(int32_t n, const void * const ins[], const size_t in_sizes[], void * const outs[], size_t out_sizes[],
                                             int rcs[]) {
    return bz3_hip_decompress_device_planes_many(n, nullptr, ins, in_sizes, outs, out_sizes, rcs);
}

BZIP3_API int bz3_hip_frame_decoded_sizes_device(int32_t n, const void * const ins[], const size_t in_sizes[], size_t decoded_sizes[], int rcs[]) {
    if (n == 0) return BZ3_OK;
    if (n < 0 || !ins || !in_sizes || !decoded_sizes || !rcs) return fail_frames(n, rcs, decoded_sizes, BZ3_ERR_INIT);
    const int dev = frames_device(n, ins, in_sizes, nullptr, nullptr);
    if (dev == -2) return fail_frames(n, rcs, decoded_sizes, BZ3_ERR_INIT);
    decoded_sizes_frames(dev, n, (const u8 * const *)ins, in_sizes, decoded_sizes, rcs);
    return first_error(n, rcs);
}

namespace {
int32_t debug_move_segments(const void * src, const void * base, void * dst, const uint64_t * segs, int32_t n, int width) {
    if (n < 0 || (n > 0 && !segs)) return BZ3_ERR_INIT;
    for (s32 i = 0; width >= 4 && i < n; i++) {
        const u64 mode = segs[width * i + width - 1];
        if (!planes_elem_size_ok(mode & 0xff) || (mode >> 9)) return BZ3_ERR_INIT;
    }
    const int dev = device_of(dst);
    if (dev < 0 || device_of(src) != dev || (width == 5 && device_of(base) != dev)) return BZ3_ERR_INIT;
    u8 * d_tab = nullptr;
    hipStream_t s = nullptr;
    int rc = BZ3_OK;
    try {
        DeviceGuard g(dev);
        std::vector<CopySeg> v((size_t)n);
        for (s32 i = 0; i < n; i++) {
            const uint64_t * q = segs + (size_t)width * i;
            if (width == 5) v[(size_t)i] = {(u64)src + q[0], (u64)dst + q[2], q[3], q[4], q[1] == UINT64_MAX ? 0 : (u64)base + q[1]};
            else v[(size_t)i] = {(u64)src + q[0], (u64)dst + q[1], q[2], width == 4 ? q[3] : 0, 0};
        }
        std::vector<u8> staging;
        HIP_CHECK(hipStreamCreateWithFlags(&s, hipStreamNonBlocking));
        HIP_CHECK(hipMalloc((void **)&d_tab, copy_table_bytes((size_t)n)));
        copy_segments(v, staging, d_tab, s);
        HIP_CHECK(hipStreamSynchronize(s));
    } catch (...) {
        rc = BZ3_ERR_INIT;
    }
    if (s) (void)hipStreamSynchronize(s);
    if (d_tab) (void)hipFree(d_tab);
    if (s) (void)hipStreamDestroy(s);
    return rc;
}
}

BZIP3_API int32_t bz3_hip_debug_copy_segments(const void * src, void * dst, const uint64_t * segs, int32_t n) { return debug_move_segments(src, nullptr, dst, segs, n, 3); }

BZIP3_API int32_t bz3_hip_debug_planes(const void * src, void * dst, const uint64_t * segs, int32_t n) { return debug_move_segments(src, nullptr, dst, segs, n, 4); }

BZIP3_API int32_t bz3_hip_debug_delta(const void * src, const void * base, void * dst, const uint64_t * segs, int32_t n) {
    return debug_move_segments(src, base, dst, segs, n, 5);
}

BZIP3_API int32_t bz3_hip_debug_range(const void * src, const void * base, void * dst, const uint64_t * segs, int32_t n) {
    if (n < 0 || (n > 0 && !segs)) return BZ3_ERR_INIT;
    bool any_base = false;
    for (s32 i = 0; i < n; i++) {
        const uint64_t * q = segs + (size_t)7 * i;
        if (!planes_elem_size_ok(q[4] & 0xff) || (q[4] >> 8) != 1 || q[5] > q[6] || q[6] > q[3]) return BZ3_ERR_INIT;
        any_base |= q[1] != UINT64_MAX;
    }
    const int dev = device_of(dst);
    if (dev < 0 || device_of(src) != dev || (any_base && device_of(base) != dev)) return BZ3_ERR_INIT;
    u8 * d_tab = nullptr;
    hipStream_t s = nullptr;
    int rc = BZ3_OK;
    try {
        DeviceGuard g(dev);
        std::vector<CopySeg> v;
        std::vector<u64> clips;
        for (s32 i = 0; i < n; i++) {
            const uint64_t * q = segs + (size_t)7 * i;
            push_range_segment(v, clips, (u64)src + q[0], q[3], q[4] & 0xff, q[5], q[6], (u64)dst + q[2], q[1] == UINT64_MAX ? 0 : (u64)base + q[1]);
        }
        std::vector<u8> staging;
        HIP_CHECK(hipStreamCreateWithFlags(&s, hipStreamNonBlocking));
        HIP_CHECK(hipMalloc((void **)&d_tab, range_table_bytes((size_t)n)));
        copy_segments(v, staging, d_tab, s, &clips);
        HIP_CHECK(hipStreamSynchronize(s));
    } catch (...) {
        rc = BZ3_ERR_INIT;
    }
    if (s) (void)hipStreamSynchronize(s);
    if (d_tab) (void)hipFree(d_tab);
    if (s) (void)hipStreamDestroy(s);
    return rc;
}

BZIP3_API int bz3_hip_crc32c_device(const void * p, size_t n, uint32_t init, uint32_t * crc) {
    if (!crc) return BZ3_ERR_INIT;
    if (!n) {
        *crc = init;
        return BZ3_OK;
    }
    const int dev = device_of(p);
    DeviceCtx * ctx = nullptr;
    try {
        ctx = dev < 0 ? nullptr : get_ctx(dev);
    } catch (...) {
        ctx = nullptr;
    }
    if (!ctx) return BZ3_ERR_INIT;
    hipStream_t s = nullptr;
    u32 * d_words = nullptr;
    int rc = BZ3_OK;
    try {
        DeviceGuard g(dev);
        HIP_CHECK(hipStreamCreateWithFlags(&s, hipStreamNonBlocking));
        HIP_CHECK(hipMalloc((void **)&d_words, 64));
        const u8 * d = (const u8 *)p;
        const size_t head = std::min(n, (size_t)((0 - (u64)d) & 3));
        u32 reg = init;
        if (head) {
            u8 h[4] = {0};
            HIP_CHECK(hipMemcpyAsync(h, d, head, hipMemcpyDeviceToHost, s));
            HIP_CHECK(hipStreamSynchronize(s));
            for (size_t i = 0; i < head; i++) {
                reg ^= h[i];
                for (int k = 0; k < 8; k++) reg = (reg >> 1) ^ (0x82F63B78u & (0u - (reg & 1u)));
            }
        }
        if (n > head) {
            crc32c_device(d + head, (u64)(n - head), reg, ctx->d_crc, d_words, s);
            reg = read_word(s, d_words + 1);
        }
        *crc = reg;
    } catch (...) {
        rc = BZ3_ERR_INIT;
    }
    if (s) (void)hipStreamSynchronize(s);
    if (d_words) (void)hipFree(d_words);
    if (s) (void)hipStreamDestroy(s);
    return rc;
}

BZIP3_API int bz3_hip_device_count(void) { return device_count(); }

BZIP3_API int bz3_hip_bind_device(int device) {
    if (device < -1 || device >= device_count()) return -1;
    g_bound_device.store(device);
    return 0;
}

BZIP3_API int bz3_hip_state_device(struct bz3_state * st) { return st->device; }

BZIP3_API int bz3_hip_set_cm_mode(int mode) {
    bool ok = mode >= -1 && mode <= CM_VARIANT_ROWS3;
#ifdef BZ3_EMU
    ok = ok || mode == CM_VARIANT_ROWS_TEST;
#endif
    if (!ok) return -1;
    g_cm_mode.store(mode);
    return 0;
}

BZIP3_API unsigned bz3_hip_cm_blocks_given_up(void) { return g_cm_given_up.load(); }

BZIP3_API void bz3_hip_debug_bwt_big_rounds(int k) { bwt_set_big_rounds(k); }

BZIP3_API int bz3_hip_cm_variant_for(int device, int blocks, int encode) {
    DeviceCtx * c = get_ctx(device);
    return (c && blocks > 0) ? cm_variant_for(c, (size_t)blocks, encode != 0) : -1;
}

BZIP3_API int bz3_hip_debug_front_end_ring(void) { return g_front_end_ring.load(); }
BZIP3_API int bz3_hip_debug_arena_swap_buffers(int reset) { return reset ? g_arena_swaps.exchange(0) : g_arena_swaps.load(); }

BZIP3_API int bz3_hip_debug_peak_concurrent_groups(int reset) {
    const int v = g_groups_peak.load();
    if (reset) g_groups_peak.store(0);
    return v;
}

BZIP3_API int bz3_hip_set_lean_states(int on) {
    g_lean.store(on ? 1 : 0);
    return 0;
}

BZIP3_API void bz3_hip_release_cached_memory(void) {
    const int n = device_count();
    for (int d = 0; d < n; d++) {
        DeviceCtx * c = nullptr;
        {
            std::lock_guard<std::mutex> lk(g_mu);
            c = g_ctx[(size_t)d];
        }
        if (!c) continue;
        (void)hipSetDevice(d);
        std::lock_guard<std::mutex> lk(c->mu);
        c->temp_trim();
        if (c->ws) (void)hipFree(c->ws);
        c->ws = nullptr;
        c->ws_cap = 0;
    }
}

BZIP3_API void bz3_hip_last_timings(struct bz3_state * st, float ms[BZ3_HIP_T_COUNT]) {
    for (int i = 0; i < BZ3_HIP_T_COUNT; i++) ms[i] = st->t[i];
}

BZIP3_API void bz3_hip_last_bwt_stats(struct bz3_state * st, int32_t * rounds, int32_t * radix_passes, uint64_t * sorted_elements) {
    if (rounds) *rounds = st->bwt.rounds;
    if (radix_passes) *radix_passes = st->bwt.radix_passes;
    if (sorted_elements) *sorted_elements = st->bwt.sorted_elements;
}

}

namespace {

struct StageEnv {
    DeviceCtx * ctx = nullptr;
    hipStream_t s = nullptr;
    std::vector<void *> allocs;
    std::unique_lock<std::mutex> lock;
    StageEnv() {
        int dev = pick_device();
        if (dev < 0) {
            fprintf(stderr, "bzip3_amd: no HIP device available -- this library has no CPU code path\n");
            abort();
        }
        ctx = get_ctx(dev);
        HIP_CHECK(hipSetDevice(dev));
        HIP_CHECK(hipStreamCreateWithFlags(&s, hipStreamNonBlocking));
        lock = std::unique_lock<std::mutex>(ctx->mu);
    }
    ~StageEnv() {
        (void)hipStreamSynchronize(s);
        for (void * p : allocs) (void)hipFree(p);
        (void)hipStreamDestroy(s);
    }
    u8 * dev(size_t bytes, const void * init = nullptr, size_t init_bytes = 0) {
        void * p = nullptr;
        HIP_CHECK(hipMalloc(&p, bytes + 4096));
        allocs.push_back(p);
        if (init && init_bytes) HIP_CHECK(hipMemcpy(p, init, init_bytes, hipMemcpyHostToDevice));
        return (u8 *)p;
    }
    void down(void * host, const void * d, size_t bytes) {
        HIP_CHECK(hipStreamSynchronize(s));
        if (bytes) HIP_CHECK(hipMemcpy(host, d, bytes, hipMemcpyDeviceToHost));
    }
    u32 word(const u32 * d) {
        u32 v = 0;
        down(&v, d, 4);
        return v;
    }
};

template <typename F>
auto stage_guard(F && f) -> decltype(f()) {
    try {
        return f();
    } catch (const HipError & e) {
        fprintf(stderr, "bzip3_amd: HIP failure '%s' at %s:%d\n", e.what, e.file, e.line);
        abort();
    }
}

}

extern "C" {

BZIP3_API uint32_t bz3_hip_stage_crc32c(const uint8_t * data, size_t n, uint32_t init) {
    return stage_guard([&]() -> u32 {
        StageEnv e;
        u8 * d = e.dev(n + 16, data, n);
        u32 * w = (u32 *)e.dev(64);
        crc32c_device(d, n, init, e.ctx->d_crc, w, e.s);
        return e.word(w + 1);
    });
}

BZIP3_API int32_t bz3_hip_stage_mrle_encode(const uint8_t * in, int32_t n, uint8_t * out) {
    return stage_guard([&]() -> s32 {
        StageEnv e;
        u8 * d = e.dev((size_t)n + 16, in, (size_t)n);
        u8 * o = e.dev((size_t)n + 64);
        Arena a = e.ctx->arena_for(workspace_bytes_for((u64)n + 64));
        MrleEncScratch sc;
        mrle_encode_size(d, (u32)n, sc, a, e.s);
        const s32 size = (s32)(32u + e.word(sc.total));
        mrle_encode_write(d, (u32)n, sc, o, e.s);
        e.down(out, o, (size_t)size);
        return size;
    });
}

BZIP3_API int bz3_hip_stage_mrle_decode(const uint8_t * in, uint8_t * out, int32_t outlen, int32_t maxin) {
    return stage_guard([&]() -> int {
        if (maxin < 32) return 1;
        StageEnv e;
        u8 * d = e.dev((size_t)maxin + 16, in, (size_t)maxin);
        u8 * o = e.dev((size_t)outlen + 64);
        u32 * w = (u32 *)e.dev(64);
        Arena a = e.ctx->arena_for(workspace_bytes_for((u64)maxin + 64));
        mrle_decode(d, (u32)maxin, o, (u32)outlen, w, a, e.s);
        const u32 got = e.word(w);
        e.down(out, o, (size_t)(got < (u32)outlen ? got : (u32)outlen));
        return got != (u32)outlen;
    });
}

BZIP3_API int32_t bz3_hip_stage_lzp_encode(const uint8_t * in, int32_t n, uint8_t * out) {
    return stage_guard([&]() -> s32 {
        StageEnv e;
        u8 * d = e.dev((size_t)n + 64, in, (size_t)n);
        u8 * o = e.dev((size_t)n + 64);
        Arena a = e.ctx->arena_for(workspace_bytes_for((u64)n + 64));
        const s32 r = lzp_encode(d, (u32)n, o, a, e.s);
        if (r > 0) e.down(out, o, (size_t)r);
        return r;
    });
}

BZIP3_API int32_t bz3_hip_stage_lzp_decode(const uint8_t * in, int32_t n, uint8_t * out, int32_t max) {
    return stage_guard([&]() -> s32 {
        StageEnv e;
        u8 * d = e.dev((size_t)n + 64, in, (size_t)n);
        u8 * o = e.dev((size_t)max + 64);
        Arena a = e.ctx->arena_for(workspace_bytes_for((u64)n + 64));
        if (n < 4) return -1;
        u32 * d_result = a.take<u32>(4);
        LzpDecodeJob job{dev_addr(d), dev_addr(o), dev_addr(a.take<u32>(LZP_LUT_WORDS)), dev_addr(d_result), (u32)n, (u32)max};
        LzpDecodeJob * d_job = a.take<LzpDecodeJob>(1);
        lzp_decode_batch(&job, d_job, 1, e.s);
        const s32 r = (s32)e.word(d_result);
        if (r > 0) e.down(out, o, (size_t)r);
        return r;
    });
}

static std::atomic<float> g_stage_ms{0.f};
BZIP3_API float bz3_hip_stage_last_ms(void) { return g_stage_ms.load(); }

BZIP3_API int32_t bz3_hip_stage_bwt(const uint8_t * in, uint8_t * out, int32_t n) {
    return stage_guard([&]() -> s32 {
        StageEnv e;
        u8 * d = e.dev((size_t)n + 64, in, (size_t)n);
        u8 * o = e.dev((size_t)n + 64);
        Arena a = e.ctx->arena_for(workspace_bytes_for((u64)n + 64));
        HIP_CHECK(hipStreamSynchronize(e.s));
        const auto t0 = std::chrono::steady_clock::now();
        const s32 idx = bwt_forward(d, (u32)n, o, a, e.s, nullptr);
        g_stage_ms.store(std::chrono::duration<float, std::milli>(std::chrono::steady_clock::now() - t0).count());
        e.down(out, o, (size_t)n);
        return idx;
    });
}

BZIP3_API int32_t bz3_hip_stage_unbwt(const uint8_t * in, uint8_t * out, int32_t n, int32_t idx) {
    return stage_guard([&]() -> s32 {
        if (n < 0) return -1;
        if (n <= 1) {
            if (idx != n) return -1;
            if (n == 1) out[0] = in[0];
            return 0;
        }
        if (idx <= 0 || idx > n) return -1;
        StageEnv e;
        u8 * d = e.dev((size_t)n + 64, in, (size_t)n);
        u8 * o = e.dev((size_t)n + 64);
        Arena a = e.ctx->arena_for(workspace_bytes_for((u64)n + 64));
        HIP_CHECK(hipStreamSynchronize(e.s));
        const auto t0 = std::chrono::steady_clock::now();
        bwt_inverse(d, (u32)n, (u32)idx, o, a, e.s);
        HIP_CHECK(hipStreamSynchronize(e.s));
        g_stage_ms.store(std::chrono::duration<float, std::milli>(std::chrono::steady_clock::now() - t0).count());
        e.down(out, o, (size_t)n);
        return 0;
    });
}

BZIP3_API int32_t bz3_hip_debug_cu_masks(int cus, int reserve, uint32_t * side, uint32_t * rest) {
    if (cus < 32 || cus > 1024 || reserve < 8 || !side || !rest) return -1;
    std::vector<uint32_t> a, b;
    DeviceCtx::cu_masks(cus, reserve, a, b);
    for (size_t k = 0; k < a.size(); k++) {
        side[k] = a[k];
        rest[k] = b[k];
    }
    return (int32_t)a.size();
}

BZIP3_API int32_t bz3_hip_debug_scan_u32(uint32_t * data, uint32_t n, uint32_t * total) {
    return stage_guard([&]() -> s32 {
        if (n == 0) return -1;
        StageEnv e;
        u32 * d = (u32 *)e.dev((size_t)n * 4 + 64, data, (size_t)n * 4);
        u32 * t = (u32 *)e.dev(64);
        Arena a = e.ctx->arena_for(scan_temp_words(n) * 4 + (1u << 20));
        exclusive_scan_u32(d, n, t, a, e.s);
        e.down(data, d, (size_t)n * 4);
        if (total) *total = e.word(t);
        return 0;
    });
}

BZIP3_API int32_t bz3_hip_debug_sort_u32(const uint32_t * keys, uint32_t n, int key_bits, int digit_bits, uint32_t * sorted_keys, uint32_t * sorted_index) {
    return stage_guard([&]() -> s32 {
        if ((digit_bits != 8 && digit_bits != 9) || key_bits < 1 || key_bits > 32 || n == 0) return -1;
        StageEnv e;
        u32 * k[2] = {(u32 *)e.dev((size_t)n * 4 + 64, keys, (size_t)n * 4), (u32 *)e.dev((size_t)n * 4 + 64)};
        u32 * v[2] = {(u32 *)e.dev((size_t)n * 4 + 64), (u32 *)e.dev((size_t)n * 4 + 64)};
        Arena a = e.ctx->arena_for(radix_temp_bytes(n, digit_bits) + (1u << 20));
        int cur = 0, passes = 0;
        for (int shift = 0; shift < key_bits; shift += digit_bits, passes++) {
            const u32 * vin = passes ? v[cur] : nullptr;
            if (digit_bits == 9) radix_pass_bits<u32, 9>(k[cur], k[cur ^ 1], vin, v[cur ^ 1], n, shift, 0xFFFFFFFFu, 0u, a, e.s);
            else radix_pass<u32>(k[cur], k[cur ^ 1], vin, v[cur ^ 1], n, shift, 0xFFFFFFFFu, 0u, a, e.s);
            cur ^= 1;
        }
        e.down(sorted_keys, k[cur], (size_t)n * 4);
        e.down(sorted_index, v[cur], (size_t)n * 4);
        return passes;
    });
}

extern "C++" template <class Job, class Launch>
void stage_cm_job(StageEnv & e, Job job, Launch && go) {
    const int variant = cm_variant_for(e.ctx, 1, std::is_same<Job, CmEncodeJob>::value);
    u32 * status = nullptr;
    if (cm_variant_has_rows(variant)) {
        job.spill = dev_addr(e.dev(CM_SPILL_BYTES));
        status = (u32 *)e.dev(64);
        HIP_CHECK(hipMemsetAsync(status, 0, 64, e.s));
        job.status = dev_addr(status);
        job.miss_base = cm_variant_is_test(variant) ? 64u : CM_MISS_BASE;
        job.miss_shift = cm_variant_is_test(variant) ? 3u : CM_MISS_SHIFT;
    }
    Job * d_job = (Job *)e.dev(sizeof job, &job, sizeof job);
    go(d_job, 1u, e.s, variant);
    if (cm_variant_has_rows(variant) && e.word(status) != 0u) {
        g_cm_given_up.fetch_add(1u);
        go(d_job, 1u, e.s, (int)CM_VARIANT_FULL);
    }
}

BZIP3_API int32_t bz3_hip_stage_cm_encode(const uint8_t * in, int32_t n, uint8_t * out) {
    return stage_guard([&]() -> s32 {
        StageEnv e;
        u8 * d = e.dev((size_t)n + 64, in, (size_t)n);
        u8 * o = e.dev(bz3_bound((size_t)n) + 64);
        u32 * w = (u32 *)e.dev(64);
        const char * dbg = getenv("BZ3_CM_DEBUG");
        CmEncodeJob job{dev_addr(d), dev_addr(o), dev_addr(w), (u32)n, dbg ? (u32)atoi(dbg) : 0u};
        const char * tg = getenv("BZ3_CM_TEST_GAP");
        u8 * side = nullptr;
        if (tg) {
            const size_t g = (size_t)atol(tg);
            const char * ts = getenv("BZ3_CM_TEST_SIDE");
            const size_t side_cap = ts ? (size_t)atol(ts) : CM_SIDE_BYTES;
            u8 * both = e.dev(g + (size_t)n + 64);
            HIP_CHECK(hipMemcpy(both + g, d, (size_t)n, hipMemcpyDeviceToDevice));
            side = e.dev(side_cap + 64);
            o = both;
            job.in = dev_addr(both + g);
            job.out = dev_addr(both);
            job.gap = (u32)g;
            job.side = dev_addr(side);
            job.side_cap = (u32)side_cap;
        }
        stage_cm_job(e, job, [](const CmEncodeJob * j, u32 nj, hipStream_t st, int variant) { cm_encode_batch(j, nj, st, variant); });
        const u32 coded = e.word(w), sw = e.word(w + 1);
        if (coded == 0xFFFFFFFFu) return -1;
        const u32 head = (tg && sw < coded) ? sw : coded;
        e.down(out, o, (size_t)head);
        if (head < coded) e.down(out + head, side, (size_t)(coded - head));
        return (s32)coded;
    });
}

BZIP3_API void bz3_hip_stage_cm_decode(const uint8_t * in, int32_t in_size, uint8_t * out, int32_t n) {
    stage_guard([&]() -> int {
        StageEnv e;
        u8 * d = e.dev((size_t)in_size + 64, in, (size_t)in_size);
        u8 * o = e.dev((size_t)n + 64);
        const char * dbg = getenv("BZ3_CM_DEBUG");
        CmDecodeJob job{dev_addr(d), dev_addr(o), (u32)in_size, (u32)n, dbg ? (u32)atoi(dbg) : 0u, 0u};
        stage_cm_job(e, job, [](const CmDecodeJob * j, u32 nj, hipStream_t st, int variant) { cm_decode_batch(j, nj, st, variant); });
        e.down(out, o, (size_t)n);
        return 0;
    });
}

BZIP3_API float bz3_hip_stage_cm_decode_many(const uint8_t * in, int32_t in_size, uint8_t * out, int32_t n, int32_t copies, uint64_t * counters) {
    return stage_guard([&]() -> float {
        StageEnv e;
        if (copies < 1 || n < 256) return -1.f;
        u8 * d = e.dev((size_t)in_size + 64, in, (size_t)in_size);
        const size_t stride = ((size_t)n + 64 + 255) & ~(size_t)255;
        u8 * o = e.dev(stride * (size_t)copies);
        const char * dbg = getenv("BZ3_CM_DEBUG");
        const u32 debug = dbg ? (u32)atoi(dbg) : 0u;
        const int variant = cm_variant_for(e.ctx, (size_t)copies, false);
        u8 * spill = cm_variant_has_rows(variant) ? e.dev(CM_SPILL_BYTES * (size_t)copies) : nullptr;
        u32 * status = (u32 *)e.dev(4 * (size_t)copies + 64);
        HIP_CHECK(hipMemsetAsync(status, 0, 4 * (size_t)copies, e.s));
        std::vector<CmDecodeJob> jobs;
        for (int32_t k = 0; k < copies; k++) {
            CmDecodeJob j{dev_addr(d), dev_addr(o + stride * (size_t)k), (u32)in_size, (u32)n, debug, 0u};
            if (spill) {
                j.spill = dev_addr(spill + CM_SPILL_BYTES * (size_t)k);
                j.status = dev_addr(status + k);
                j.miss_base = CM_MISS_BASE;
                j.miss_shift = CM_MISS_SHIFT;
            }
            jobs.push_back(j);
        }
        CmDecodeJob * d_jobs = (CmDecodeJob *)e.dev(sizeof(CmDecodeJob) * jobs.size(), jobs.data(), sizeof(CmDecodeJob) * jobs.size());
        hipEvent_t e0, e1;
        HIP_CHECK(hipEventCreate(&e0));
        HIP_CHECK(hipEventCreate(&e1));
        HIP_CHECK(hipEventRecord(e0, e.s));
        cm_decode_batch(d_jobs, (u32)copies, e.s, variant, (debug & 15u) == 3u);
        HIP_CHECK(hipEventRecord(e1, e.s));
        HIP_CHECK(hipStreamSynchronize(e.s));
        float ms = 0.f;
        (void)hipEventElapsedTime(&ms, e0, e1);
        (void)hipEventDestroy(e0);
        (void)hipEventDestroy(e1);
        e.down(out, o, (size_t)n);
        if (counters)
            for (int32_t k = 0; k < copies; k++) e.down(counters + 16 * (size_t)k, o + stride * (size_t)k, 128);
        if (getenv("BZ3_CM_MANY_CHECK")) {
            std::vector<u8> other((size_t)n);
            for (int32_t k = 1; k < copies; k++) {
                e.down(other.data(), o + stride * (size_t)k, (size_t)n);
                if (memcmp(other.data(), out, (size_t)n) != 0) return -2.f;
            }
        }
        return ms;
    });
}

BZIP3_API float bz3_hip_stage_cm_encode_many(const uint8_t * in, int32_t n, uint8_t * out, int32_t * coded, int32_t copies) {
    return stage_guard([&]() -> float {
        StageEnv e;
        if (copies < 1 || n < 1) return -1.f;
        u8 * d = e.dev((size_t)n + 64, in, (size_t)n);
        const size_t stride = (bz3_bound((size_t)n) + 64 + 255) & ~(size_t)255;
        u8 * o = e.dev(stride * (size_t)copies);
        u32 * w = (u32 *)e.dev(16 * (size_t)copies + 64);
        const char * dbg = getenv("BZ3_CM_DEBUG");
        const u32 debug = dbg ? (u32)atoi(dbg) : 0u;
        const int variant = cm_variant_for(e.ctx, (size_t)copies, true);
        u8 * spill = cm_variant_has_rows(variant) ? e.dev(CM_SPILL_BYTES * (size_t)copies) : nullptr;
        u32 * status = (u32 *)e.dev(4 * (size_t)copies + 64);
        HIP_CHECK(hipMemsetAsync(status, 0, 4 * (size_t)copies, e.s));
        u32 * claim = getenv("BZ3_CM_NO_CLAIM") ? nullptr : (u32 *)e.dev(CM_CLAIM_WORDS * 4);
        if (claim) HIP_CHECK(hipMemsetAsync(claim, 0, CM_CLAIM_WORDS * 4, e.s));
        std::vector<CmEncodeJob> jobs;
        for (int32_t k = 0; k < copies; k++) {
            CmEncodeJob j{dev_addr(d), dev_addr(o + stride * (size_t)k), dev_addr(w + 4 * (size_t)k), (u32)n, debug};
            j.claim = claim ? dev_addr(claim) : 0;
            if (spill) {
                j.spill = dev_addr(spill + CM_SPILL_BYTES * (size_t)k);
                j.status = dev_addr(status + k);
                j.miss_base = CM_MISS_BASE;
                j.miss_shift = CM_MISS_SHIFT;
            }
            jobs.push_back(j);
        }
        CmEncodeJob * d_jobs = (CmEncodeJob *)e.dev(sizeof(CmEncodeJob) * jobs.size(), jobs.data(), sizeof(CmEncodeJob) * jobs.size());
        hipEvent_t e0, e1;
        HIP_CHECK(hipEventCreate(&e0));
        HIP_CHECK(hipEventCreate(&e1));
        HIP_CHECK(hipEventRecord(e0, e.s));
        cm_encode_batch(d_jobs, (u32)copies, e.s, variant);
        HIP_CHECK(hipEventRecord(e1, e.s));
        HIP_CHECK(hipStreamSynchronize(e.s));
        float ms = 0.f;
        (void)hipEventElapsedTime(&ms, e0, e1);
        (void)hipEventDestroy(e0);
        (void)hipEventDestroy(e1);
        const u32 got = e.word(w);
        if (coded) *coded = (int32_t)got;
        if (got != 0xFFFFFFFFu && got <= bz3_bound((size_t)n) && !(debug & 15u)) {
            e.down(out, o, (size_t)got);
            if (getenv("BZ3_CM_MANY_CHECK")) {
                std::vector<u8> other((size_t)got);
                for (int32_t k = 1; k < copies; k++) {
                    if (e.word(w + 4 * (size_t)k) != got) return -2.f;
                    e.down(other.data(), o + stride * (size_t)k, (size_t)got);
                    if (memcmp(other.data(), out, (size_t)got) != 0) return -2.f;
                }
            }
        }
        return ms;
    });
}

}
```

### bzip3_amd/csrc/stages.hpp

```cpp
#pragma once
#include "hipx.hpp"
#include "sort.hpp"

namespace bz3 {

struct CrcTables {
    u32 pow2[64];
    u32 lane[64];
    u32 row;
    u32 pad[3];
};
void crc_build_tables(CrcTables & t);
void crc32c_device(const u8 * d_data, u64 n, u32 init, const CrcTables * d_tables, u32 * d_scratch, hipStream_t s);

struct MrleEncScratch {
    u32 tiles = 0;
    u32 * carry = nullptr;
    u32 * tile_sum = nullptr;
    s32 * gain = nullptr;
    u32 * total = nullptr;
};
void mrle_encode_size(const u8 * d_in, u32 n, MrleEncScratch & sc, Arena & tmp, hipStream_t s);
void mrle_encode_write(const u8 * d_in, u32 n, const MrleEncScratch & sc, u8 * d_out, hipStream_t s);
void mrle_decode(const u8 * d_enc, u32 m, u8 * d_out, u32 outlen, u32 * d_total, Arena & tmp, hipStream_t s);

struct LzDriverOut {
    u32 end_pos;
    u32 n_matches;
    u32 iterations;
    u32 evaluated;
};
struct LzpEncodeCtx {
    bool active = false;
    const u8 * in = nullptr;
    u32 n = 0, nwords = 0;
    u32 *prev = nullptr, *next = nullptr, *skip = nullptr, *mstart = nullptr, *cand_bits = nullptr, *mpos = nullptr, *mlen = nullptr;
    LzDriverOut * d_res = nullptr;
};
struct LzpDriverJob {
    u64 in;
    u64 prev, next, cand_bits, skip, mstart, mpos, mlen;
    u64 result;
    u32 n, nwords;
};
size_t lzp_encode_ctx_bytes(u64 n);
void lzp_encode_prepare(const u8 * d_in, u32 n, LzpEncodeCtx & c, Arena & tmp, hipStream_t s);
void lzp_encode_prepare(const u8 * d_in, u32 n, LzpEncodeCtx & c, Arena & ctx, Arena & tmp, hipStream_t s);
LzpDriverJob lzp_driver_job(const LzpEncodeCtx & c);
void lzp_driver_batch(const LzpDriverJob * h_jobs, LzpDriverJob * d_jobs, u32 njobs, hipStream_t s);
s32 lzp_encode_finish(const LzpEncodeCtx & c, u8 * d_out, Arena & tmp, hipStream_t s);
s32 lzp_encode(const u8 * d_in, u32 n, u8 * d_out, Arena & tmp, hipStream_t s);
struct LzpDecodeJob {
    u64 in;
    u64 out;
    u64 lut;
    u64 result;
    u32 n, max_out;
};
constexpr size_t LZP_LUT_WORDS = (size_t)1 << 18;
void lzp_decode_batch(const LzpDecodeJob * h_jobs, LzpDecodeJob * d_jobs, u32 njobs, hipStream_t s);

struct BwtStats {
    int rounds = 0;
    u64 sorted_elements = 0;
    int radix_passes = 0;
};
constexpr int BWT_ROUTE_KEEP = 40;
s32 bwt_forward(const u8 * d_in, u32 n, u8 * d_out, Arena & tmp, hipStream_t s, BwtStats * stats, u32 * d_idx = nullptr, u32 * d_outside = nullptr);
size_t bwt_workspace_bytes(u64 n);
void bwt_set_big_rounds(int k);

void bwt_inverse(const u8 * d_in, u32 n, u32 idx, u8 * d_out, Arena & tmp, hipStream_t s);
size_t unbwt_workspace_bytes(u64 n);

constexpr u32 CM_NO_GAP = 0xFFFFFFFFu;
struct CmEncodeJob {
    u64 in;
    u64 out;
    u64 out_size;
    u32 n;
    u32 debug;
    u64 spill = 0;
    u64 status = 0;
    u32 miss_base = 0, miss_shift = 0;
    u32 gap = CM_NO_GAP, side_cap = 0;
    u64 side = 0;
    u64 claim = 0;
};
constexpr u32 CM_CLAIM_WORDS = 4096;
struct CmDecodeJob {
    u64 in;
    u64 out;
    u32 in_size;
    u32 n;
    u32 debug;
    u32 pad;
    u64 spill = 0, status = 0;
    u32 miss_base = 0, miss_shift = 0;
};
enum { CM_VARIANT_FULL = 0, CM_VARIANT_ROWS = 1, CM_VARIANT_ROWS3 = 2, CM_VARIANT_ROWS_TEST = 9  };
inline bool cm_variant_has_rows(int v) { return v != CM_VARIANT_FULL; }
inline bool cm_variant_is_test(int v) { return v == CM_VARIANT_ROWS_TEST; }
constexpr size_t CM_SPILL_BYTES = 256 * 256 * 2;
constexpr u32 CM_MISS_BASE = 1024, CM_MISS_SHIFT = 5;
void cm_encode_batch(const CmEncodeJob * d_jobs, u32 njobs, hipStream_t s, int variant = CM_VARIANT_FULL);
void cm_decode_batch(const CmDecodeJob * d_jobs, u32 njobs, hipStream_t s, int variant = CM_VARIANT_FULL, bool prof = false);

}
```

### bzip3_amd/csrc/unbwt.hip

```cpp
#include "prims.hpp"
#include "sort.hpp"
#include "stages.hpp"

namespace bz3 {

constexpr int UB_BLOCK = 256;

__device__ __forceinline__ bool ub_is_splitter(u32 row, u32 idx, int log_stride) {
    if (row == 0 || row == idx || log_stride == 0) return true;
    return ((row * 0x9E3779B1u) >> (32 - log_stride)) == 0u;
}

__global__ void __launch_bounds__(UB_BLOCK) k_ub_hist(const u8 * __restrict__ in, u32 n, u32 * __restrict__ hist) {
    __shared__ u32 bins[256];
    bins[threadIdx.x] = 0;
    __syncthreads();
    const u64 base = (u64)blockIdx.x * (UB_BLOCK * 64);
    const u64 last = (u64)n - 1;
    for (u32 g = 0; g < 4; g++) {
        u8 c[16];
#pragma unroll
        for (u32 k = 0; k < 16; k++) {
            const u64 i = base + (u64)(g * 16 + k) * UB_BLOCK + threadIdx.x;
            c[k] = in[i < n ? i : last];
        }
#pragma unroll
        for (u32 k = 0; k < 16; k++) {
            const u64 i = base + (u64)(g * 16 + k) * UB_BLOCK + threadIdx.x;
            if (i < n) atomicAdd(&bins[c[k]], 1u);
        }
    }
    __syncthreads();
    if (bins[threadIdx.x]) atomicAdd(&hist[threadIdx.x], bins[threadIdx.x]);
}

__global__ void __launch_bounds__(256) k_ub_cum(const u32 * __restrict__ hist, u32 * __restrict__ cum, u32 * __restrict__ psi, u32 idx) {
    __shared__ u32 lds[256 / WAVE + 1];
    u32 tot;
    u32 pre = block_excl_add<256>(hist[threadIdx.x], lds, tot);
    cum[threadIdx.x] = pre + 1;
    if (threadIdx.x == 0) {
        cum[256] = tot + 1;
        psi[0] = idx;
    }
}

__global__ void __launch_bounds__(UB_BLOCK) k_ub_flags(u32 rows, u32 idx, int log_stride, u32 * __restrict__ flags) {
    const u32 r = blockIdx.x * UB_BLOCK + threadIdx.x;
    if (r < rows) flags[r] = ub_is_splitter(r, idx, log_stride) ? 1u : 0u;
}

__global__ void __launch_bounds__(UB_BLOCK) k_ub_collect(u32 rows, u32 idx, int log_stride, const u32 * __restrict__ sid, u32 * __restrict__ split_row) {
    const u32 r = blockIdx.x * UB_BLOCK + threadIdx.x;
    if (r < rows && ub_is_splitter(r, idx, log_stride)) split_row[sid[r]] = r;
}

__device__ __forceinline__ u32 ub_symbol_lds(const u32 * c, u32 r) {
    u32 lo = 0, hi = 256;
#pragma unroll
    for (int b = 0; b < 8; b++) {
        const u32 mid = (lo + hi) >> 1;
        if (c[mid] <= r) lo = mid; else hi = mid;
    }
    return lo;
}

__global__ void __launch_bounds__(UB_BLOCK) k_ub_walk(const u32 * __restrict__ psi, const u32 * __restrict__ sid, const u32 * __restrict__ split_row, u32 nsplit,
                                                     u32 idx, int log_stride, u32 rows, const u32 * __restrict__ cum, u32 cap, u32 * __restrict__ succ,
                                                     u32 * __restrict__ dist, u8 * __restrict__ slab, u32 * __restrict__ resume) {
    __shared__ u32 c[257];
    for (int k = threadIdx.x; k < 257; k += UB_BLOCK) c[k] = cum[k];
    __syncthreads();
    const u32 j = blockIdx.x * UB_BLOCK + threadIdx.x;
    if (j >= nsplit) return;
    u32 r = split_row[j];
    if (r == 0) {
        succ[j] = j;
        dist[j] = 0;
        return;
    }
    u32 * __restrict__ mine = reinterpret_cast<u32 *>(slab + (size_t)j * cap);
    u32 len = 0, word = 0;
    do {
        const u32 nr = psi[r];
        if (len < cap) {
            word |= ub_symbol_lds(c, r) << (8u * (len & 3u));
            if ((len & 3u) == 3u) {
                mine[len >> 2] = word;
                word = 0;
            }
        } else if (len == cap) {
            resume[j] = r;
        }
        r = nr;
        len++;
    } while (!ub_is_splitter(r, idx, log_stride) && len <= rows);
    if (len < cap && (len & 3u)) mine[len >> 2] = word;
    succ[j] = sid[r];
    dist[j] = len;
}

__global__ void __launch_bounds__(UB_BLOCK) k_ub_jump(const u32 * __restrict__ succ_in, const u32 * __restrict__ dist_in, u32 nsplit, u32 * __restrict__ succ_out,
                                                     u32 * __restrict__ dist_out) {
    const u32 j = blockIdx.x * UB_BLOCK + threadIdx.x;
    if (j >= nsplit) return;
    const u32 sj = succ_in[j];
    u64 d = (u64)dist_in[j] + dist_in[sj];
    dist_out[j] = d > 0xFFFFFFFFull ? 0xFFFFFFFFu : (u32)d;
    succ_out[j] = succ_in[sj];
}

__global__ void __launch_bounds__(UB_BLOCK) k_ub_place(const u8 * __restrict__ slab, const u32 * __restrict__ seg_len, const u32 * __restrict__ dist,
                                                      const u32 * __restrict__ succ, const u32 * __restrict__ sid, u32 idx, u32 cap, u32 nsplit, u32 n,
                                                      u8 * __restrict__ out) {
    const u32 t = blockIdx.x * UB_BLOCK + threadIdx.x;
    const u32 j = t >> 4, part = t & 15u;
    if (j >= nsplit) return;
    if (succ[j] != sid[0]) return;
    const u32 D = dist[sid[idx]];
    const u32 d = dist[j];
    if (d > D) return;
    const u32 len = seg_len[j];
    const u32 m = len < cap ? len : cap;
    const u32 limit = n & ~1u;
    const u64 pos0 = (u64)D - d;
    const u8 * __restrict__ src = slab + (size_t)j * cap;
    for (u32 o = part * 16u; o < m; o += 256u) {
        if (o + 16u <= m && pos0 + o + 16u <= limit) {
            const uint4 q = *reinterpret_cast<const uint4 *>(src + o);
            PackedU128 w;
            w.v[0] = q.x; w.v[1] = q.y; w.v[2] = q.z; w.v[3] = q.w;
            *reinterpret_cast<PackedU128 *>(out + pos0 + o) = w;
        } else {
            for (u32 k = o; k < m && k < o + 16u; k++)
                if (pos0 + k < limit) out[pos0 + k] = src[k];
        }
    }
}

__global__ void __launch_bounds__(UB_BLOCK) k_ub_walk_long(const u32 * __restrict__ psi, const u32 * __restrict__ resume, const u32 * __restrict__ seg_len,
                                                          const u32 * __restrict__ dist, const u32 * __restrict__ succ, const u32 * __restrict__ sid, u32 idx,
                                                          const u32 * __restrict__ cum, u32 cap, u32 nsplit, u32 n, u8 * __restrict__ out) {
    __shared__ u32 c[257];
    for (int k = threadIdx.x; k < 257; k += UB_BLOCK) c[k] = cum[k];
    __syncthreads();
    const u32 j = blockIdx.x * UB_BLOCK + threadIdx.x;
    if (j >= nsplit) return;
    const u32 len = seg_len[j];
    if (len <= cap) return;
    if (succ[j] != sid[0]) return;
    const u32 D = dist[sid[idx]];
    const u32 d = dist[j];
    if (d > D) return;
    const u32 limit = n & ~1u;
    u32 r = resume[j];
    u64 pos = (u64)D - d + cap;
    for (u32 t = cap; t < len; t++) {
        const u32 nr = psi[r];
        const u32 sym = ub_symbol_lds(c, r);
        if (pos < limit) out[pos] = (u8)sym;
        pos++;
        r = nr;
    }
}

__device__ __forceinline__ u32 ub_first_symbol(const u32 * __restrict__ cum, u32 r) {
    u32 lo = 0, hi = 256;
    for (int b = 0; b < 8; b++) {
        const u32 mid = (lo + hi) >> 1;
        if (cum[mid] <= r) lo = mid; else hi = mid;
    }
    return lo;
}

__global__ void __launch_bounds__(UB_BLOCK) k_ub_tail(const u8 * __restrict__ in, const u32 * __restrict__ psi, const u32 * __restrict__ cum,
                                                     const u32 * __restrict__ dist, const u32 * __restrict__ sid, u32 idx, u32 n, u8 * __restrict__ out) {
    const u32 D = dist[sid[idx]];
    const u32 limit = n & ~1u;
    const u32 lastc = in[0];
    const u32 E = cum[lastc];
    const u32 gid = blockIdx.x * UB_BLOCK + threadIdx.x;
    u32 start = D;
    if (D < limit && (D & 1u)) {
        int shift = 0;
        while ((n >> shift) > (1u << 17)) shift++;
        const bool same_group = E >= 2 && ((E - 1) >> shift) == (E >> shift);
        if (gid == 0) {
            if (same_group || E + 1 > n) {
                out[D] = 0;
            } else {
                out[D - 1] = (u8)ub_first_symbol(cum, E + 1);
                out[D] = (u8)ub_first_symbol(cum, psi[E + 1]);
            }
        }
        start = D + 1;
    }
    if (start < limit) {
        const u32 q0 = (E == 1) ? 2u : 1u;
        const u32 hi = ub_first_symbol(cum, q0), lo = ub_first_symbol(cum, psi[q0]);
        for (u64 j = (u64)start + gid; j < limit; j += (u64)gridDim.x * UB_BLOCK)
            if (j != n - 1) out[j] = (u8)((j & 1u) ? lo : hi);
    }
    if (gid == 0) out[n - 1] = (u8)lastc;
}

size_t unbwt_workspace_bytes(u64 n) {
    const u64 splitters = n + 1 < 300000 ? n + 1 : 300000 + (n >> 7);
    return (n + 64) * 8 + radix_temp_bytes(n) + scan_temp_words(n + 1) * 4 + (splitters + 4096) * 32 + (n + (n >> 3)) * 4 + (1u << 20);
}

void bwt_inverse(const u8 * d_in, u32 n, u32 idx, u8 * d_out, Arena & tmp, hipStream_t s) {
    if (n == 0) return;
    if (n == 1) {
        HIP_CHECK(hipMemcpyAsync(d_out, d_in, 1, hipMemcpyDeviceToDevice, s));
        return;
    }
    const size_t mk = tmp.mark();
    const u32 rows = n + 1;
    u32 * psi = tmp.take<u32>(rows);
    u32 * sid = tmp.take<u32>(rows);
    u32 * hist = tmp.take<u32>(256);
    u32 * cum = tmp.take<u32>(257);
    u32 * d_total = tmp.take<u32>(1);

    HIP_CHECK(hipMemsetAsync(hist, 0, 256 * 4, s));
    launch(k_ub_hist, dim3((u32)(((u64)n + UB_BLOCK * 64 - 1) / (UB_BLOCK * 64))), dim3(UB_BLOCK), 0, s, d_in, n, hist);
    launch(k_ub_cum, dim3(1), dim3(256), 0, s, (const u32 *)hist, cum, psi, idx);
    radix_pass<u8>(d_in, (u8 *)nullptr, (const u32 *)nullptr, psi, n, 0, idx, 1u, tmp, s);

    constexpr int max_log_stride = 8;
    int log_stride = 0;
    while (log_stride < max_log_stride && ((u64)rows >> (log_stride + 1)) >= 65536) log_stride++;
    const dim3 grows((rows + UB_BLOCK - 1) / UB_BLOCK);
    launch(k_ub_flags, grows, dim3(UB_BLOCK), 0, s, rows, idx, log_stride, sid);
    exclusive_scan_u32(sid, rows, d_total, tmp, s);
    u32 nsplit = 0;
    HIP_CHECK(hipMemcpyAsync(&nsplit, d_total, 4, hipMemcpyDeviceToHost, s));
    HIP_CHECK(hipStreamSynchronize(s));
    u32 * split_row = tmp.take<u32>(nsplit);
    u32 * seg_len = tmp.take<u32>(nsplit);
    u32 * resume = tmp.take<u32>(nsplit);
    u32 * succ[2] = {tmp.take<u32>(nsplit), tmp.take<u32>(nsplit)};
    u32 * dist[2] = {tmp.take<u32>(nsplit), tmp.take<u32>(nsplit)};
    const u32 cap = 4u << log_stride;
    u8 * slab = tmp.take<u8>((size_t)nsplit * cap + 64);
    const dim3 gs((nsplit + UB_BLOCK - 1) / UB_BLOCK);
    launch(k_ub_collect, grows, dim3(UB_BLOCK), 0, s, rows, idx, log_stride, (const u32 *)sid, split_row);
    launch(k_ub_walk, gs, dim3(UB_BLOCK), 0, s, (const u32 *)psi, (const u32 *)sid, (const u32 *)split_row, nsplit, idx, log_stride, rows, (const u32 *)cum, cap, succ[0],
           dist[0], slab, resume);
    HIP_CHECK(hipMemcpyAsync(seg_len, dist[0], (size_t)nsplit * 4, hipMemcpyDeviceToDevice, s));

    int cur = 0;
    for (u64 span = 1; span < nsplit; span <<= 1) {
        launch(k_ub_jump, gs, dim3(UB_BLOCK), 0, s, (const u32 *)succ[cur], (const u32 *)dist[cur], nsplit, succ[cur ^ 1], dist[cur ^ 1]);
        cur ^= 1;
    }
    launch(k_ub_place, dim3((u32)(((u64)nsplit * 16 + UB_BLOCK - 1) / UB_BLOCK)), dim3(UB_BLOCK), 0, s, (const u8 *)slab, (const u32 *)seg_len, (const u32 *)dist[cur],
           (const u32 *)succ[cur], (const u32 *)sid, idx, cap, nsplit, n, d_out);
    launch(k_ub_walk_long, gs, dim3(UB_BLOCK), 0, s, (const u32 *)psi, (const u32 *)resume, (const u32 *)seg_len, (const u32 *)dist[cur], (const u32 *)succ[cur],
           (const u32 *)sid, idx, (const u32 *)cum, cap, nsplit, n, d_out);
    launch(k_ub_tail, dim3(256), dim3(UB_BLOCK), 0, s, d_in, (const u32 *)psi, (const u32 *)cum, (const u32 *)dist[cur], (const u32 *)sid, idx, n, d_out);
    HIP_CHECK(hipStreamSynchronize(s));
    tmp.release(mk);
}

}
```

### include/bz3_hip.h

```cpp
#ifndef BZ3_HIP_H
#define BZ3_HIP_H
#include <stddef.h>
#include <stdint.h>
#include "libbz3.h"
#define BZ3_HIP 1

#ifdef __cplusplus
extern "C" {
#endif

BZIP3_API int bz3_hip_device_count(void);
BZIP3_API int bz3_hip_bind_device(int device);
BZIP3_API int bz3_hip_state_device(struct bz3_state * state);

BZIP3_API int bz3_hip_set_cm_mode(int mode);
BZIP3_API void bz3_hip_debug_bwt_big_rounds(int k);
BZIP3_API unsigned bz3_hip_cm_blocks_given_up(void);
BZIP3_API unsigned bz3_hip_cm_blocks_routed_full(void);

BZIP3_API int bz3_hip_cm_variant_for(int device, int blocks, int encode);

BZIP3_API int bz3_hip_debug_peak_concurrent_groups(int reset);

BZIP3_API int bz3_hip_debug_front_end_ring(void);
BZIP3_API int bz3_hip_set_keep_workspace(int on);
BZIP3_API int bz3_hip_set_front_end_duo(int on);
BZIP3_API void bz3_hip_set_workspace_headroom(long long bytes);
BZIP3_API size_t bz3_hip_workspace_headroom(void);
BZIP3_API unsigned bz3_hip_debug_headroom_events(int reset, unsigned * releases);
BZIP3_API size_t bz3_hip_debug_ring_contexts(size_t free_bytes, size_t have, size_t need, size_t fixed, size_t ctx_bytes, size_t cap, int lean, size_t headroom);
BZIP3_API size_t bz3_hip_debug_arena_slack(size_t bytes);
BZIP3_API unsigned bz3_hip_debug_cm_launches(int reset);
BZIP3_API size_t bz3_hip_debug_workspace_bytes(size_t block_bytes, int which);
BZIP3_API size_t bz3_hip_debug_cached_bytes(int device);
BZIP3_API int bz3_hip_debug_arena_swap_buffers(int reset);

BZIP3_API int bz3_hip_set_lean_states(int on);
BZIP3_API void bz3_hip_release_cached_memory(void);

BZIP3_API int32_t bz3_hip_encode_block_device(struct bz3_state * state, void * buffer, int32_t size);
BZIP3_API int32_t bz3_hip_decode_block_device(struct bz3_state * state, void * buffer, size_t buffer_size, int32_t compressed_size,
                                              int32_t orig_size);
BZIP3_API void bz3_hip_encode_blocks_device(struct bz3_state * states[], void * buffers[], int32_t sizes[], int32_t n);
BZIP3_API void bz3_hip_decode_blocks_device(struct bz3_state * states[], void * buffers[], size_t buffer_sizes[], int32_t sizes[],
                                            int32_t orig_sizes[], int32_t n);

BZIP3_API int bz3_hip_compress_device(uint32_t block_size, const void * in, void * out, size_t in_size, size_t * out_size);
BZIP3_API int bz3_hip_decompress_device(const void * in, void * out, size_t in_size, size_t * out_size);
BZIP3_API int bz3_hip_frame_decoded_size_device(const void * in, size_t in_size, size_t * decoded_size);
BZIP3_API int bz3_hip_compress_device_many(uint32_t block_size, int32_t n, const void * const ins[], const size_t in_sizes[],
                                           void * const outs[], size_t out_sizes[], int rcs[]);
BZIP3_API int bz3_hip_decompress_device_many(int32_t n, const void * const ins[], const size_t in_sizes[],
                                             void * const outs[], size_t out_sizes[], int rcs[]);
BZIP3_API int bz3_hip_frame_decoded_sizes_device(int32_t n, const void * const ins[], const size_t in_sizes[],
                                                 size_t decoded_sizes[], int rcs[]);
BZIP3_API int32_t bz3_hip_debug_copy_segments(const void * src, void * dst, const uint64_t * segs, int32_t n);

BZIP3_API int bz3_hip_compress_device_planes(uint32_t block_size, uint32_t elem_size, const void * in, void * out, size_t in_size,
                                             size_t * out_size);
BZIP3_API int bz3_hip_decompress_device_planes(uint32_t elem_size, const void * in, void * out, size_t in_size, size_t * out_size);
BZIP3_API int bz3_hip_compress_device_planes_many(uint32_t block_size, int32_t n, const uint32_t elem_sizes[], const void * const ins[],
                                                  const size_t in_sizes[], void * const outs[], size_t out_sizes[], int rcs[]);
BZIP3_API int bz3_hip_decompress_device_planes_many(int32_t n, const uint32_t elem_sizes[], const void * const ins[],
                                                    const size_t in_sizes[], void * const outs[], size_t out_sizes[], int rcs[]);
BZIP3_API int32_t bz3_hip_debug_planes(const void * src, void * dst, const uint64_t * segs, int32_t n);

BZIP3_API int bz3_hip_compress_device_delta(uint32_t block_size, uint32_t elem_size, const void * in, const void * base, void * out,
                                            size_t in_size, size_t * out_size);
BZIP3_API int bz3_hip_decompress_device_delta(uint32_t elem_size, const void * in, const void * base, size_t base_size, void * out,
                                              size_t in_size, size_t * out_size);
BZIP3_API int bz3_hip_compress_device_delta_many(uint32_t block_size, int32_t n, const uint32_t elem_sizes[], const void * const ins[],
                                                 const void * const bases[], const size_t in_sizes[], void * const outs[],
                                                 size_t out_sizes[], int rcs[]);
BZIP3_API int bz3_hip_decompress_device_delta_many(int32_t n, const uint32_t elem_sizes[], const void * const ins[],
                                                   const size_t in_sizes[], const void * const bases[], const size_t base_sizes[],
                                                   void * const outs[], size_t out_sizes[], int rcs[]);
BZIP3_API int bz3_hip_crc32c_device(const void * p, size_t n, uint32_t init, uint32_t * crc);
BZIP3_API int32_t bz3_hip_debug_delta(const void * src, const void * base, void * dst, const uint64_t * segs, int32_t n);

BZIP3_API int bz3_hip_decompress_device_range(uint32_t elem_size, const void * in, size_t in_size, uint64_t offset, const void * base,
                                              size_t base_size, void * out, size_t * out_size);
BZIP3_API int bz3_hip_decompress_device_range_many(int32_t n, const uint32_t elem_sizes[], const void * const ins[], const size_t in_sizes[],
                                                   const uint64_t offsets[], const void * const bases[], const size_t base_sizes[],
                                                   void * const outs[], size_t out_sizes[], int rcs[]);
BZIP3_API int32_t bz3_hip_debug_range(const void * src, const void * base, void * dst, const uint64_t * segs, int32_t n);

enum {
    BZ3_HIP_T_CRC = 0,
    BZ3_HIP_T_RLE = 1,
    BZ3_HIP_T_LZP = 2,
    BZ3_HIP_T_BWT = 3,
    BZ3_HIP_T_CM = 4,
    BZ3_HIP_T_COPY = 5,
    BZ3_HIP_T_COUNT = 8
};
BZIP3_API void bz3_hip_last_timings(struct bz3_state * state, float ms[BZ3_HIP_T_COUNT]);
BZIP3_API void bz3_hip_last_bwt_stats(struct bz3_state * state, int32_t * rounds, int32_t * radix_passes, uint64_t * sorted_elements);

BZIP3_API void bz3_hip_set_collect_window_us(int us);
BZIP3_API unsigned bz3_hip_debug_collected_batches(int reset, unsigned * largest);

BZIP3_API uint32_t bz3_hip_stage_crc32c(const uint8_t * data, size_t n, uint32_t init);
BZIP3_API int32_t bz3_hip_stage_mrle_encode(const uint8_t * in, int32_t n, uint8_t * out);
BZIP3_API int bz3_hip_stage_mrle_decode(const uint8_t * in, uint8_t * out, int32_t outlen, int32_t maxin);
BZIP3_API int32_t bz3_hip_stage_lzp_encode(const uint8_t * in, int32_t n, uint8_t * out);
BZIP3_API int32_t bz3_hip_stage_lzp_decode(const uint8_t * in, int32_t n, uint8_t * out, int32_t max);
BZIP3_API int32_t bz3_hip_stage_bwt(const uint8_t * in, uint8_t * out, int32_t n);
BZIP3_API int32_t bz3_hip_stage_unbwt(const uint8_t * in, uint8_t * out, int32_t n, int32_t idx);
BZIP3_API int32_t bz3_hip_debug_cu_masks(int cus, int reserve, uint32_t * side, uint32_t * rest);
BZIP3_API int32_t bz3_hip_debug_scan_u32(uint32_t * data, uint32_t n, uint32_t * total);
BZIP3_API int32_t bz3_hip_debug_sort_u32(const uint32_t * keys, uint32_t n, int key_bits, int digit_bits, uint32_t * sorted_keys, uint32_t * sorted_index);
BZIP3_API float bz3_hip_stage_last_ms(void);
BZIP3_API int32_t bz3_hip_stage_cm_encode(const uint8_t * in, int32_t n, uint8_t * out);
BZIP3_API void bz3_hip_stage_cm_decode(const uint8_t * in, int32_t in_size, uint8_t * out, int32_t n);

#define BZ3_HIP_ERR_IO (-100)
BZIP3_API int bz3_hip_encode_stream(int in_fd, int out_fd, int32_t block_size, int32_t blocks_per_batch);
BZIP3_API int bz3_hip_decode_stream(int in_fd, int out_fd, int32_t blocks_per_batch);

BZIP3_API float bz3_hip_stage_cm_decode_many(const uint8_t * in, int32_t in_size, uint8_t * out, int32_t n, int32_t copies, uint64_t * counters);

BZIP3_API float bz3_hip_stage_cm_encode_many(const uint8_t * in, int32_t n, uint8_t * out, int32_t * coded, int32_t copies);

#ifdef __cplusplus
}
#endif
#endif
```

Before: 634.9.

## Batch inverse BWT across blocks and fuse decode finish host readbacks

Restructures the inverse BWT into a batched multi-job path with a precomputed splitter layout, so the host no longer has to read back the splitter count mid-pipeline. Per-window decode finishing (LZP size, RLE check, CRC check, stored-block CRC) now collects the device words each block needs and reads them with a single gather kernel and one sync per phase, instead of a separate sync per block. Because UNBWT_GROUP_MAX is 1, inverse BWTs still run one per group unless an environment variable or setter raises it. The batched readbacks and the removal of the mid-BWT host sync do apply by default. The cost is extra workspace sizing logic and more complex layout code.

```diff
diff --git a/bzip3_amd/__init__.py b/bzip3_amd/__init__.py
--- a/bzip3_amd/__init__.py
+++ b/bzip3_amd/__init__.py
@@ -40,6 +40,10 @@
         "bz3_hip_bind_device": (C.c_int, [C.c_int]),
         "bz3_hip_state_device": (C.c_int, [vp]),
         "bz3_hip_set_cm_mode": (C.c_int, [C.c_int]),
+        "bz3_hip_set_unbwt_group": (C.c_int, [C.c_int]),
+        "bz3_hip_debug_unbwt_group": (C.c_int, [sz, sz, sz, sz, sz, sz, sz, C.c_int]),
+        "bz3_hip_debug_unbwt_workspace": (sz, [sz]),
+        "bz3_hip_debug_unbwt_splitters": (u32, [u32, u32]),
         "bz3_hip_cm_blocks_given_up": (C.c_uint, []),
         "bz3_hip_cm_blocks_routed_full": (C.c_uint, []),
         "bz3_hip_debug_bwt_big_rounds": (None, [C.c_int]),
@@ -94,6 +98,7 @@
         "bz3_hip_stage_lzp_decode": (i32, [vp, i32, vp, i32]),
         "bz3_hip_stage_bwt": (i32, [vp, vp, i32]),
         "bz3_hip_stage_unbwt": (i32, [vp, vp, i32, i32]),
+        "bz3_hip_stage_unbwt_many": (i32, [vp, vp, vp, vp, i32]),
         "bz3_hip_stage_last_ms": (C.c_float, []),
         "bz3_hip_debug_sort_u32": (i32, [vp, u32, C.c_int, C.c_int, vp, vp]),
         "bz3_hip_debug_scan_u32": (i32, [vp, u32, vp]),
@@ -201,6 +206,17 @@
         out = (C.c_uint8 * max(1, len(data)))()
         rc = self.lib.bz3_hip_stage_unbwt(_cbuf(data, len(data)), out, len(data), idx)
         return rc, C.string_at(out, len(data))
+
+    def unbwt_many(self, pairs):
+        k = len(pairs)
+        ins = [_cbuf(d, len(d)) for d, _ in pairs]
+        outs = [(C.c_uint8 * max(1, len(d)))() for d, _ in pairs]
+        pi = (C.c_void_p * max(1, k))(*[C.cast(b, C.c_void_p) for b in ins])
+        po = (C.c_void_p * max(1, k))(*[C.cast(b, C.c_void_p) for b in outs])
+        ns = (C.c_int32 * max(1, k))(*[len(d) for d, _ in pairs])
+        idxs = (C.c_int32 * max(1, k))(*[i for _, i in pairs])
+        rc = self.lib.bz3_hip_stage_unbwt_many(pi, po, ns, idxs, k)
+        return rc, [C.string_at(o, len(d)) for o, (d, _) in zip(outs, pairs)]
 
     def cm_encode(self, data):
         out = (C.c_uint8 * (len(data) + len(data) // 50 + 64))()
diff --git a/bzip3_amd/csrc/api.hip b/bzip3_amd/csrc/api.hip
--- a/bzip3_amd/csrc/api.hip
+++ b/bzip3_amd/csrc/api.hip
@@ -519,6 +519,28 @@
     return v;
 }
 
+struct WordAddrs {
+    u64 a[64];
+};
+__global__ void __launch_bounds__(64) k_gather_words(const WordAddrs w, u32 n, u32 * __restrict__ out) {
+    if (threadIdx.x < n) out[threadIdx.x] = *global_ptr<const u32>(w.a[threadIdx.x]);
+}
+void read_words(hipStream_t s, Arena & tmp, const std::vector<const u32 *> & addrs, std::vector<u32> & out) {
+    out.assign(addrs.size(), 0u);
+    if (addrs.empty()) return;
+    const size_t mk = tmp.mark();
+    u32 * d = tmp.take<u32>(addrs.size());
+    for (size_t k0 = 0; k0 < addrs.size(); k0 += 64) {
+        WordAddrs w{};
+        const u32 m = (u32)(addrs.size() - k0 < 64 ? addrs.size() - k0 : 64);
+        for (u32 k = 0; k < m; k++) w.a[k] = dev_addr(addrs[k0 + k]);
+        launch(k_gather_words, dim3(1), dim3(64), 0, s, w, m, d + k0);
+    }
+    HIP_CHECK(hipMemcpyAsync(out.data(), d, addrs.size() * 4, hipMemcpyDeviceToHost, s));
+    HIP_CHECK(hipStreamSynchronize(s));
+    tmp.release(mk);
+}
+
 inline bool sizes_fit(size_t buffer_size, s32 lzp_size, s32 rle_size, s32 orig_size) {
     const size_t a = lzp_size < 0 ? 0 : (size_t)lzp_size, b = rle_size < 0 ? 0 : (size_t)rle_size, c = orig_size < 0 ? 0 : (size_t)orig_size;
     return a <= buffer_size && b <= buffer_size && c <= buffer_size;
@@ -547,6 +569,23 @@
     return room / (ctx_bytes + cap);
 }
 void enforce_headroom(DeviceCtx * ctx, hipStream_t s);
+constexpr int UNBWT_GROUP_MAX = 1;
+std::atomic<int> g_unbwt_group{0};
+inline int unbwt_group_forced() {
+    static const int env = [] { const char * e = getenv("BZ3_HIP_UNBWT_GROUP"); return e && atoi(e) > 0 ? atoi(e) : 0; }();
+    const int g = g_unbwt_group.load();
+    return g > 0 ? g : env;
+}
+inline int unbwt_group_for(size_t free_b, size_t have, size_t base, size_t ring, size_t unit, size_t block_bytes, size_t headroom, int forced) {
+    (void)block_bytes;
+    const size_t want = forced > 0 ? (size_t)forced : (size_t)UNBWT_GROUP_MAX;
+    if (want <= 1 || !unit) return 1;
+    const size_t aside = headroom + ((size_t)513 << 20) + ((size_t)64 << 20);
+    const size_t total = free_b + have;
+    const size_t room = total > base + ring + aside ? total - base - ring - aside : 0;
+    const size_t fit = 1 + room / unit;
+    return (int)(want < fit ? want : fit);
+}
 
 #ifndef BZ3_FRONT_DUO_DEFAULT
 #define BZ3_FRONT_DUO_DEFAULT 0
@@ -1111,78 +1150,119 @@
     st->pending = bz3_state::DEC_CODED;
 }
 
-bool decode_unbwt(bz3_state * st, Arena & arena, float cm_ms) {
+int decode_unbwt_check(bz3_state * st, float cm_ms, UnbwtJob & job) {
     hipStream_t s = st->xs;
     st->t[BZ3_HIP_T_CM] = cm_ms;
+    st->t[BZ3_HIP_T_BWT] = 0.f;
     const s32 n = st->size_before_bwt;
     if (st->bwt_idx > n) {
         st->last_error = BZ3_ERR_MALFORMED_HEADER;
-        return false;
+        return 0;
     }
     u8 *b1 = st->d_swap, *b2 = st->user;
     if (st->lean) {
         b1 = st->user;
         b2 = st->d_swap;
     }
-    const double t0 = now_ms();
+    int verdict = 1;
     if (n <= 1) {
-        if (st->bwt_idx != n) { st->last_error = BZ3_ERR_BWT; return false; }
+        if (st->bwt_idx != n) { st->last_error = BZ3_ERR_BWT; return 0; }
         if (n == 1) HIP_CHECK(hipMemcpyAsync(b2, b1, 1, hipMemcpyDeviceToDevice, s));
     } else {
-        if (st->bwt_idx <= 0) { st->last_error = BZ3_ERR_BWT; return false; }
-        bwt_inverse(b1, (u32)n, (u32)st->bwt_idx, b2, arena, s);
+        if (st->bwt_idx <= 0) { st->last_error = BZ3_ERR_BWT; return 0; }
+        job = UnbwtJob{b1, (u32)n, (u32)st->bwt_idx, b2};
+        verdict = 2;
     }
     st->b1 = b2;
     st->b2 = b1;
     st->size_src = n;
-    st->t[BZ3_HIP_T_BWT] = (float)(now_ms() - t0);
-    return true;
-}
-
-void decode_finish(bz3_state * st, Arena & arena) {
-    hipStream_t s = st->xs;
-    const size_t bound = bz3_bound((size_t)st->block_size);
-    (void)bound;
-    u8 *b1 = st->b1, *b2 = st->b2;
-    s32 size_src = st->size_src;
-    if (st->model & 2) {
-        size_src = (s32)read_word(s, st->d_words + 5);
-        if (size_src == -1) { st->last_error = BZ3_ERR_CRC; return; }
-        if ((size_t)size_src > st->buffer_size) { st->last_error = BZ3_ERR_DATA_SIZE_TOO_SMALL; return; }
-        u8 * tmp = b1; b1 = b2; b2 = tmp;
-    }
-    if (st->model & 4) {
-        const double t0 = now_ms();
-        bool bad = size_src < 32;
-        if (!bad) {
-            mrle_decode(b1, (u32)size_src, b2, (u32)st->orig_size, st->d_words + 4, arena, s);
-            bad = read_word(s, st->d_words + 4) != (u32)st->orig_size;
-        }
-        st->t[BZ3_HIP_T_RLE] = (float)(now_ms() - t0);
-        if (bad) { st->last_error = BZ3_ERR_CRC; return; }
-        size_src = st->orig_size;
-        u8 * tmp = b1; b1 = b2; b2 = tmp;
-    }
-    st->last_error = BZ3_OK;
-    if (size_src > st->block_size || size_src < 0) {
-        st->last_error = BZ3_ERR_MALFORMED_HEADER;
-        return;
-    }
-    if (b1 != st->user) {
-        const double t0 = now_ms();
-        HIP_CHECK(hipMemcpyAsync(st->user, b1, (size_t)size_src, hipMemcpyDeviceToDevice, s));
-        HIP_CHECK(hipStreamSynchronize(s));
-        st->t[BZ3_HIP_T_COPY] += (float)(now_ms() - t0);
-    }
-    const double t0 = now_ms();
-    crc32c_device(st->user, (u64)size_src, 1u, st->ctx->d_crc, st->d_words, s);
-    const u32 got = read_word(s, st->d_words + 1);
-    st->t[BZ3_HIP_T_CRC] = (float)(now_ms() - t0);
-    if (got != st->crc) {
-        st->last_error = BZ3_ERR_CRC;
-        return;
-    }
-    st->result = size_src;
+    return verdict;
+}
+
+void decode_finish_window(bz3_state ** sts, const std::vector<s32> & alive, const std::vector<s32> & stored, Arena & arena, hipStream_t s) {
+    struct Item {
+        bz3_state * st;
+        u8 *b1, *b2;
+        s32 size_src;
+        bool live;
+        bool rle;
+        bool rle_timed;
+    };
+    std::vector<Item> items;
+    for (s32 i : alive) items.push_back(Item{sts[i], sts[i]->b1, sts[i]->b2, sts[i]->size_src, true, false, false});
+    std::vector<const u32 *> addrs;
+    std::vector<u32> words;
+    for (const Item & it : items)
+        if (it.st->model & 2) addrs.push_back(it.st->d_words + 5);
+    read_words(s, arena, addrs, words);
+    size_t next = 0;
+    for (Item & it : items) {
+        if (!(it.st->model & 2)) continue;
+        it.size_src = (s32)words[next++];
+        if (it.size_src == -1) { it.st->last_error = BZ3_ERR_CRC; it.live = false; continue; }
+        if ((size_t)it.size_src > it.st->buffer_size) { it.st->last_error = BZ3_ERR_DATA_SIZE_TOO_SMALL; it.live = false; continue; }
+        u8 * tmp = it.b1; it.b1 = it.b2; it.b2 = tmp;
+    }
+    addrs.clear();
+    const double t_rle = now_ms();
+    size_t rle_blocks = 0;
+    for (Item & it : items) {
+        if (!it.live || !(it.st->model & 4)) continue;
+        rle_blocks++;
+        it.rle_timed = true;
+        if (it.size_src < 32) {
+            it.st->last_error = BZ3_ERR_CRC;
+            it.live = false;
+            continue;
+        }
+        mrle_decode(it.b1, (u32)it.size_src, it.b2, (u32)it.st->orig_size, it.st->d_words + 4, arena, s);
+        addrs.push_back(it.st->d_words + 4);
+        it.rle = true;
+    }
+    read_words(s, arena, addrs, words);
+    const float rle_share = rle_blocks ? (float)((now_ms() - t_rle) / (double)rle_blocks) : 0.f;
+    next = 0;
+    for (Item & it : items) {
+        if (it.rle_timed) it.st->t[BZ3_HIP_T_RLE] = rle_share;
+        if (!it.rle) continue;
+        if (words[next++] != (u32)it.st->orig_size) { it.st->last_error = BZ3_ERR_CRC; it.live = false; continue; }
+        it.size_src = it.st->orig_size;
+        u8 * tmp = it.b1; it.b1 = it.b2; it.b2 = tmp;
+    }
+    addrs.clear();
+    const double t_crc = now_ms();
+    size_t crc_blocks = 0;
+    for (Item & it : items) {
+        if (!it.live) continue;
+        bz3_state * st = it.st;
+        st->last_error = BZ3_OK;
+        if (it.size_src > st->block_size || it.size_src < 0) {
+            st->last_error = BZ3_ERR_MALFORMED_HEADER;
+            it.live = false;
+            continue;
+        }
+        if (it.b1 != st->user) HIP_CHECK(hipMemcpyAsync(st->user, it.b1, (size_t)it.size_src, hipMemcpyDeviceToDevice, s));
+        crc32c_device(st->user, (u64)it.size_src, 1u, st->ctx->d_crc, st->d_words, s);
+        addrs.push_back(st->d_words + 1);
+        crc_blocks++;
+    }
+    for (s32 i : stored) addrs.push_back(sts[i]->d_words + 1);
+    read_words(s, arena, addrs, words);
+    const float crc_share = crc_blocks ? (float)((now_ms() - t_crc) / (double)crc_blocks) : 0.f;
+    next = 0;
+    for (Item & it : items) {
+        if (!it.live) continue;
+        it.st->t[BZ3_HIP_T_CRC] = crc_share;
+        if (words[next++] != it.st->crc) {
+            it.st->last_error = BZ3_ERR_CRC;
+            continue;
+        }
+        it.st->result = it.size_src;
+    }
+    for (s32 i : stored) {
+        if (words[next++] != sts[i]->crc) sts[i]->last_error = BZ3_ERR_CRC;
+        else sts[i]->result = sts[i]->size;
+    }
 }
 
 void decode_group(bz3_state ** sts, u8 ** bufs, const size_t * buffer_sizes, const s32 * sizes, const s32 * orig_sizes, const u8 * hdrs, s32 n) {
@@ -1259,7 +1339,25 @@
             if (sts[i]->pending == bz3_state::DEC_CODED && (sts[i]->model & 2)) c++;
         if (c > lzp_in_window) lzp_in_window = c;
     }
-    Arena arena = lead->ctx->arena_for(need + (size_t)tail_slots * lzp_in_window * (LZP_LUT_WORDS * 4 + sizeof(LzpDecodeJob) + 256) + (size_t)n * 256 + cm_scratch_bytes(coded.size()) + max_round + 65536);
+    size_t ub_unit = 0, ub_block = 0;
+    for (s32 i : coded)
+        if (sts[i]->size_before_bwt > 1 && (size_t)sts[i]->size_before_bwt > ub_block) ub_block = (size_t)sts[i]->size_before_bwt;
+    ub_unit = unbwt_workspace_bytes(ub_block);
+    const size_t arena_base = need + (size_t)tail_slots * lzp_in_window * (LZP_LUT_WORDS * 4 + sizeof(LzpDecodeJob) + 256) + (size_t)n * 256 + cm_scratch_bytes(coded.size()) + max_round + 65536;
+    int ub_group = 1;
+    if (ub_block) {
+        size_t free_b = 0, total_b = 0, ring = 0;
+        if (any_lean) {
+            size_t cap_max = 0;
+            for (s32 i = 0; i < n; i++)
+                if (sts[i]->lean && sts[i]->cap > cap_max) cap_max = sts[i]->cap;
+            ring = (size_t)tail_slots * (size_t)tail_window * ((cap_max + 255) & ~(size_t)255);
+        }
+        if (hipMemGetInfo(&free_b, &total_b) != hipSuccess) free_b = 0;
+        ub_group = unbwt_group_for(free_b, lead->ctx->ws_cap, arena_base, ring, ub_unit, ub_block, ws_headroom(), unbwt_group_forced());
+        if ((s32)ub_group > tail_window) ub_group = (int)tail_window;
+    }
+    Arena arena = lead->ctx->arena_for(arena_base + (size_t)(ub_group - 1) * ub_unit);
     float cm_ms = 0.f;
     for (size_t r = 0, k0 = 0; r < round_end.size(); k0 = round_end[r++]) {
         const size_t mk = arena.mark();
@@ -1285,6 +1383,7 @@
         s32 w0 = 0, w1 = 0;
         std::vector<LzpDecodeJob> lz_jobs;
         std::vector<s32> lz_owner;
+        std::vector<s32> stored;
         std::vector<char> alive;
         LzpDecodeJob * d_lz = nullptr;
         u32 * luts = nullptr;
@@ -1300,7 +1399,7 @@
             if (sts[i]->lean && sts[i]->cap > swap_cap) swap_cap = sts[i]->cap;
         const size_t want = (size_t)tail_slots * (size_t)tail_window;
         const size_t step = (swap_cap + 255) & ~(size_t)255;
-        const size_t keep_free = need + need / 32 + 65536;
+        const size_t keep_free = need + need / 32 + 65536 + (size_t)(ub_group - 1) * ub_unit;
         while (swap_cap && arena_swaps.size() < want && arena.cap - arena.used >= keep_free + step) arena_swaps.push_back(arena.take<u8>(swap_cap));
     }
     std::vector<char> from_arena((size_t)n, 0);
@@ -1341,6 +1440,9 @@
     const s32 lag = tail_slots - 1;
     static const bool trace_rings = getenv("BZ3_HIP_TRACE_RINGS") != nullptr;
     double tr_unbwt = 0, tr_wait = 0, tr_finish = 0, tr_t0 = now_ms();
+    std::vector<UnbwtJob> ub_jobs;
+    std::vector<s32> ub_owner;
+    std::vector<s32> fin_alive;
     for (s32 k = 0; k < nwin + lag; k++) {
         const double tr_a = now_ms();
         if (k < nwin) {
@@ -1351,19 +1453,38 @@
             w.w1 = (w.w0 + tail_window < n) ? w.w0 + tail_window : n;
             w.lz_jobs.clear();
             w.lz_owner.clear();
+            w.stored.clear();
             w.alive.assign((size_t)(w.w1 - w.w0), 0);
+            ub_jobs.clear();
+            ub_owner.clear();
             for (s32 i = w.w0; i < w.w1; i++) {
                 bz3_state * st = sts[i];
                 if (st->pending == bz3_state::DEC_STORED) {
-                    HIP_CHECK(hipStreamSynchronize(st->xs));
-                    if (read_word(st->xs, st->d_words + 1) != st->crc) st->last_error = BZ3_ERR_CRC;
-                    else st->result = st->size;
+                    w.stored.push_back(i);
                     continue;
                 }
                 if (st->pending != bz3_state::DEC_CODED) continue;
                 borrow(i);
-                if (!decode_unbwt(st, arena, cm_ms)) continue;
+                UnbwtJob job{};
+                const int verdict = decode_unbwt_check(st, cm_ms, job);
+                if (!verdict) continue;
                 w.alive[(size_t)(i - w.w0)] = 1;
+                if (verdict == 2) {
+                    ub_jobs.push_back(job);
+                    ub_owner.push_back(i);
+                }
+            }
+            for (size_t g0 = 0; g0 < ub_jobs.size(); g0 += (size_t)ub_group) {
+                const size_t cnt = ub_jobs.size() - g0 < (size_t)ub_group ? ub_jobs.size() - g0 : (size_t)ub_group;
+                const double t0 = now_ms();
+                bwt_inverse_batch(ub_jobs.data() + g0, (int)cnt, arena, s);
+                HIP_CHECK(hipStreamSynchronize(s));
+                const float share = (float)((now_ms() - t0) / (double)cnt);
+                for (size_t j = g0; j < g0 + cnt; j++) sts[ub_owner[j]]->t[BZ3_HIP_T_BWT] = share;
+            }
+            for (s32 i = w.w0; i < w.w1; i++) {
+                bz3_state * st = sts[i];
+                if (!w.alive[(size_t)(i - w.w0)]) continue;
                 if (st->model & 2) {
                     if (st->lzp_size < 4) {
                         st->last_error = BZ3_ERR_CRC;
@@ -1410,16 +1531,17 @@
                     st->ctx->temp_put(big);
                 }
             }
-            for (s32 i = w.w0; i < w.w1; i++) {
-                if (w.alive[(size_t)(i - w.w0)]) decode_finish(sts[i], arena);
-                give_back(i);
-            }
+            fin_alive.clear();
+            for (s32 i = w.w0; i < w.w1; i++)
+                if (w.alive[(size_t)(i - w.w0)]) fin_alive.push_back(i);
+            decode_finish_window(sts, fin_alive, w.stored, arena, s);
+            for (s32 i = w.w0; i < w.w1; i++) give_back(i);
         }
         tr_finish += now_ms() - tr_b;
     }
     if (trace_rings)
-        fprintf(stderr, "[bz3 rings] decode tail: %d blocks, %d windows of %d x %d slots: %.1f ms = inverse BWTs + LZP launches %.1f + waiting for a window's LZP decoders %.1f + mRLE / CRC / hand-back %.1f\n",
-                (int)n, (int)nwin, (int)tail_window, (int)tail_slots, now_ms() - tr_t0, tr_unbwt, tr_wait, tr_finish - tr_wait);
+        fprintf(stderr, "[bz3 rings] decode tail: %d blocks, %d windows of %d x %d slots, inverse BWTs in groups of %d: %.1f ms = inverse BWTs + LZP launches %.1f + waiting for a window's LZP decoders %.1f + mRLE / CRC / hand-back %.1f\n",
+                (int)n, (int)nwin, (int)tail_window, (int)tail_slots, ub_group, now_ms() - tr_t0, tr_unbwt, tr_wait, tr_finish - tr_wait);
     for (s32 i = 0; i < n; i++) sts[i]->pending = bz3_state::NONE;
     if (s != s_cm) (void)hipStreamSynchronize(s);
     enforce_headroom(lead->ctx, s_cm);
@@ -2919,6 +3041,18 @@
     return 0;
 }
 
+BZIP3_API int bz3_hip_set_unbwt_group(int blocks) {
+    if (blocks < 0) return -1;
+    g_unbwt_group.store(blocks);
+    return 0;
+}
+
+BZIP3_API int bz3_hip_debug_unbwt_group(size_t free_b, size_t have, size_t base, size_t ring, size_t unit, size_t block_bytes, size_t headroom, int forced) {
+    return unbwt_group_for(free_b, have, base, ring, unit, block_bytes, headroom, forced);
+}
+BZIP3_API size_t bz3_hip_debug_unbwt_workspace(size_t n) { return unbwt_workspace_bytes((u64)n); }
+BZIP3_API uint32_t bz3_hip_debug_unbwt_splitters(uint32_t n, uint32_t idx) { return unbwt_splitter_count(n, idx); }
+
 BZIP3_API unsigned bz3_hip_cm_blocks_given_up(void) { return g_cm_given_up.load(); }
 
 BZIP3_API void bz3_hip_debug_bwt_big_rounds(int k) { bwt_set_big_rounds(k); }
@@ -3133,6 +3267,33 @@
         HIP_CHECK(hipStreamSynchronize(e.s));
         g_stage_ms.store(std::chrono::duration<float, std::milli>(std::chrono::steady_clock::now() - t0).count());
         e.down(out, o, (size_t)n);
+        return 0;
+    });
+}
+
+BZIP3_API int32_t bz3_hip_stage_unbwt_many(const uint8_t * const * ins, uint8_t * const * outs, const int32_t * ns, const int32_t * idxs, int32_t count) {
+    return stage_guard([&]() -> s32 {
+        if (count < 0) return -1;
+        size_t ws = 1u << 20;
+        for (s32 k = 0; k < count; k++) {
+            const s32 n = ns[k], idx = idxs[k];
+            if (n < 0 || (n <= 1 ? idx != n : (idx <= 0 || idx > n))) return -1;
+            ws += unbwt_workspace_bytes((u64)n + 64);
+        }
+        StageEnv e;
+        std::vector<UnbwtJob> jobs;
+        for (s32 k = 0; k < count; k++) {
+            u8 * d = e.dev((size_t)ns[k] + 64, ins[k], (size_t)ns[k]);
+            u8 * o = e.dev((size_t)ns[k] + 64);
+            jobs.push_back(UnbwtJob{d, (u32)ns[k], (u32)idxs[k], o});
+        }
+        Arena a = e.ctx->arena_for(ws);
+        HIP_CHECK(hipStreamSynchronize(e.s));
+        const auto t0 = std::chrono::steady_clock::now();
+        bwt_inverse_batch(jobs.data(), (int)count, a, e.s);
+        HIP_CHECK(hipStreamSynchronize(e.s));
+        g_stage_ms.store(std::chrono::duration<float, std::milli>(std::chrono::steady_clock::now() - t0).count());
+        for (s32 k = 0; k < count; k++) e.down(outs[k], jobs[(size_t)k].d_out, (size_t)ns[k]);
         return 0;
     });
 }
diff --git a/bzip3_amd/csrc/stages.hpp b/bzip3_amd/csrc/stages.hpp
--- a/bzip3_amd/csrc/stages.hpp
+++ b/bzip3_amd/csrc/stages.hpp
@@ -70,8 +70,15 @@
 size_t bwt_workspace_bytes(u64 n);
 void bwt_set_big_rounds(int k);
 
+struct UnbwtJob {
+    const u8 * d_in;
+    u32 n, idx;
+    u8 * d_out;
+};
+void bwt_inverse_batch(const UnbwtJob * jobs, int count, Arena & tmp, hipStream_t s);
 void bwt_inverse(const u8 * d_in, u32 n, u32 idx, u8 * d_out, Arena & tmp, hipStream_t s);
 size_t unbwt_workspace_bytes(u64 n);
+u32 unbwt_splitter_count(u32 n, u32 idx);
 
 constexpr u32 CM_NO_GAP = 0xFFFFFFFFu;
 struct CmEncodeJob {
diff --git a/bzip3_amd/csrc/unbwt.hip b/bzip3_amd/csrc/unbwt.hip
--- a/bzip3_amd/csrc/unbwt.hip
+++ b/bzip3_amd/csrc/unbwt.hip
@@ -34,25 +34,70 @@
     if (bins[threadIdx.x]) atomicAdd(&hist[threadIdx.x], bins[threadIdx.x]);
 }
 
-__global__ void __launch_bounds__(256) k_ub_cum(const u32 * __restrict__ hist, u32 * __restrict__ cum, u32 * __restrict__ psi, u32 idx) {
+constexpr int UB_MAX_JOBS = 16;
+struct UbJobArg {
+    u64 in, out;
+    u64 slab_off;
+    u32 n, idx;
+    u32 row0;
+    u32 split0;
+    u32 sblk0;
+    u32 log_stride;
+    u32 nsplit;
+    u32 pad;
+};
+struct UbBatch {
+    u32 count, pad;
+    UbJobArg j[UB_MAX_JOBS];
+};
+
+__device__ __forceinline__ u32 ub_job_of_rows(const UbBatch & b, u32 blk) {
+    u32 g = 0;
+    while (g + 1 < b.count && blk >= (b.j[g + 1].row0 / UB_BLOCK)) g++;
+    return g;
+}
+__device__ __forceinline__ u32 ub_job_of_splitters(const UbBatch & b, u32 blk) {
+    u32 g = 0;
+    while (g + 1 < b.count && blk >= b.j[g + 1].sblk0) g++;
+    return g;
+}
+
+__device__ __forceinline__ u32 ub_guard(const UbBatch & b, u32 g, const u32 * __restrict__ nsplit_dev) {
+    const u32 d = nsplit_dev[g], h = b.j[g].nsplit;
+    return d < h ? d : h;
+}
+
+__global__ void __launch_bounds__(256) k_ub_cum(const UbBatch b, const u32 * __restrict__ hist_all, u32 * __restrict__ cum_all, u32 * __restrict__ psi_all) {
     __shared__ u32 lds[256 / WAVE + 1];
+    const u32 g = blockIdx.x;
+    u32 * __restrict__ cum = cum_all + 257 * g;
     u32 tot;
-    u32 pre = block_excl_add<256>(hist[threadIdx.x], lds, tot);
+    u32 pre = block_excl_add<256>(hist_all[256 * g + threadIdx.x], lds, tot);
     cum[threadIdx.x] = pre + 1;
     if (threadIdx.x == 0) {
         cum[256] = tot + 1;
-        psi[0] = idx;
-    }
-}
-
-__global__ void __launch_bounds__(UB_BLOCK) k_ub_flags(u32 rows, u32 idx, int log_stride, u32 * __restrict__ flags) {
-    const u32 r = blockIdx.x * UB_BLOCK + threadIdx.x;
-    if (r < rows) flags[r] = ub_is_splitter(r, idx, log_stride) ? 1u : 0u;
-}
-
-__global__ void __launch_bounds__(UB_BLOCK) k_ub_collect(u32 rows, u32 idx, int log_stride, const u32 * __restrict__ sid, u32 * __restrict__ split_row) {
-    const u32 r = blockIdx.x * UB_BLOCK + threadIdx.x;
-    if (r < rows && ub_is_splitter(r, idx, log_stride)) split_row[sid[r]] = r;
+        psi_all[b.j[g].row0] = b.j[g].idx;
+    }
+}
+
+__global__ void __launch_bounds__(UB_BLOCK) k_ub_flags(const UbBatch b, u32 * __restrict__ flags_all) {
+    const u32 g = ub_job_of_rows(b, blockIdx.x);
+    const u32 row0 = b.j[g].row0;
+    const u32 R = blockIdx.x * UB_BLOCK + threadIdx.x;
+    const u32 r = R - row0;
+    flags_all[R] = (r <= b.j[g].n && ub_is_splitter(r, b.j[g].idx, (int)b.j[g].log_stride)) ? 1u : 0u;
+}
+
+__global__ void __launch_bounds__(UB_BLOCK) k_ub_collect(const UbBatch b, const u32 * __restrict__ sid_all, u32 * __restrict__ split_row, u32 * __restrict__ nsplit_dev) {
+    const u32 g = ub_job_of_rows(b, blockIdx.x);
+    const u32 row0 = b.j[g].row0, n = b.j[g].n;
+    const u32 R = blockIdx.x * UB_BLOCK + threadIdx.x;
+    const u32 r = R - row0;
+    if (r > n) return;
+    const bool sp = ub_is_splitter(r, b.j[g].idx, (int)b.j[g].log_stride);
+    const u32 id = sid_all[R];
+    if (sp && id - b.j[g].split0 < b.j[g].nsplit) split_row[id] = r;
+    if (r == n) nsplit_dev[g] = id + (sp ? 1u : 0u) - sid_all[row0];
 }
 
 __device__ __forceinline__ u32 ub_symbol_lds(const u32 * c, u32 r) {
@@ -65,21 +110,29 @@
     return lo;
 }
 
-__global__ void __launch_bounds__(UB_BLOCK) k_ub_walk(const u32 * __restrict__ psi, const u32 * __restrict__ sid, const u32 * __restrict__ split_row, u32 nsplit,
-                                                     u32 idx, int log_stride, u32 rows, const u32 * __restrict__ cum, u32 cap, u32 * __restrict__ succ,
-                                                     u32 * __restrict__ dist, u8 * __restrict__ slab, u32 * __restrict__ resume) {
+__global__ void __launch_bounds__(UB_BLOCK) k_ub_walk(const UbBatch b, const u32 * __restrict__ psi_all, const u32 * __restrict__ sid_all, const u32 * __restrict__ split_row,
+                                                     const u32 * __restrict__ nsplit_dev, const u32 * __restrict__ cum_all, u32 * __restrict__ succ, u32 * __restrict__ dist,
+                                                     u8 * __restrict__ slab_all, u32 * __restrict__ resume) {
     __shared__ u32 c[257];
+    const u32 g = ub_job_of_splitters(b, blockIdx.x);
+    const u32 * __restrict__ cum = cum_all + 257 * g;
     for (int k = threadIdx.x; k < 257; k += UB_BLOCK) c[k] = cum[k];
     __syncthreads();
-    const u32 j = blockIdx.x * UB_BLOCK + threadIdx.x;
-    if (j >= nsplit) return;
+    const u32 jl = (blockIdx.x - b.j[g].sblk0) * UB_BLOCK + threadIdx.x;
+    if (jl >= ub_guard(b, g, nsplit_dev)) return;
+    const u32 j = b.j[g].split0 + jl;
+    const u32 * __restrict__ psi = psi_all + b.j[g].row0;
+    const u32 * __restrict__ sid = sid_all + b.j[g].row0;
+    const u32 idx = b.j[g].idx, rows = b.j[g].n + 1;
+    const int log_stride = (int)b.j[g].log_stride;
+    const u32 cap = 4u << log_stride;
     u32 r = split_row[j];
     if (r == 0) {
         succ[j] = j;
         dist[j] = 0;
         return;
     }
-    u32 * __restrict__ mine = reinterpret_cast<u32 *>(slab + (size_t)j * cap);
+    u32 * __restrict__ mine = reinterpret_cast<u32 *>(slab_all + b.j[g].slab_off + (size_t)jl * cap);
     u32 len = 0, word = 0;
     do {
         const u32 nr = psi[r];
@@ -100,31 +153,36 @@
     dist[j] = len;
 }
 
-__global__ void __launch_bounds__(UB_BLOCK) k_ub_jump(const u32 * __restrict__ succ_in, const u32 * __restrict__ dist_in, u32 nsplit, u32 * __restrict__ succ_out,
-                                                     u32 * __restrict__ dist_out) {
+__global__ void __launch_bounds__(UB_BLOCK) k_ub_jump(const u32 * __restrict__ succ_in, const u32 * __restrict__ dist_in, const u32 * __restrict__ total_dev,
+                                                     u32 total_host, u32 * __restrict__ succ_out, u32 * __restrict__ dist_out) {
     const u32 j = blockIdx.x * UB_BLOCK + threadIdx.x;
-    if (j >= nsplit) return;
+    if (j >= *total_dev || j >= total_host) return;
     const u32 sj = succ_in[j];
     u64 d = (u64)dist_in[j] + dist_in[sj];
     dist_out[j] = d > 0xFFFFFFFFull ? 0xFFFFFFFFu : (u32)d;
     succ_out[j] = succ_in[sj];
 }
 
-__global__ void __launch_bounds__(UB_BLOCK) k_ub_place(const u8 * __restrict__ slab, const u32 * __restrict__ seg_len, const u32 * __restrict__ dist,
-                                                      const u32 * __restrict__ succ, const u32 * __restrict__ sid, u32 idx, u32 cap, u32 nsplit, u32 n,
-                                                      u8 * __restrict__ out) {
-    const u32 t = blockIdx.x * UB_BLOCK + threadIdx.x;
-    const u32 j = t >> 4, part = t & 15u;
-    if (j >= nsplit) return;
+__global__ void __launch_bounds__(UB_BLOCK) k_ub_place(const UbBatch b, const u8 * __restrict__ slab_all, const u32 * __restrict__ seg_len, const u32 * __restrict__ dist,
+                                                      const u32 * __restrict__ succ, const u32 * __restrict__ sid_all, const u32 * __restrict__ nsplit_dev) {
+    const u32 g = ub_job_of_splitters(b, blockIdx.x >> 4);
+    const u32 jl = ((blockIdx.x >> 4) - b.j[g].sblk0) * UB_BLOCK + (blockIdx.x & 15u) * 16u + (threadIdx.x >> 4);
+    const u32 part = threadIdx.x & 15u;
+    if (jl >= ub_guard(b, g, nsplit_dev)) return;
+    const u32 j = b.j[g].split0 + jl;
+    const u32 * __restrict__ sid = sid_all + b.j[g].row0;
+    const u32 n = b.j[g].n;
+    const u32 cap = 4u << b.j[g].log_stride;
+    u8 * __restrict__ out = global_ptr<u8>(b.j[g].out);
     if (succ[j] != sid[0]) return;
-    const u32 D = dist[sid[idx]];
+    const u32 D = dist[sid[b.j[g].idx]];
     const u32 d = dist[j];
     if (d > D) return;
     const u32 len = seg_len[j];
     const u32 m = len < cap ? len : cap;
     const u32 limit = n & ~1u;
     const u64 pos0 = (u64)D - d;
-    const u8 * __restrict__ src = slab + (size_t)j * cap;
+    const u8 * __restrict__ src = slab_all + b.j[g].slab_off + (size_t)jl * cap;
     for (u32 o = part * 16u; o < m; o += 256u) {
         if (o + 16u <= m && pos0 + o + 16u <= limit) {
             const uint4 q = *reinterpret_cast<const uint4 *>(src + o);
@@ -138,21 +196,28 @@
     }
 }
 
-__global__ void __launch_bounds__(UB_BLOCK) k_ub_walk_long(const u32 * __restrict__ psi, const u32 * __restrict__ resume, const u32 * __restrict__ seg_len,
-                                                          const u32 * __restrict__ dist, const u32 * __restrict__ succ, const u32 * __restrict__ sid, u32 idx,
-                                                          const u32 * __restrict__ cum, u32 cap, u32 nsplit, u32 n, u8 * __restrict__ out) {
+__global__ void __launch_bounds__(UB_BLOCK) k_ub_walk_long(const UbBatch b, const u32 * __restrict__ psi_all, const u32 * __restrict__ resume, const u32 * __restrict__ seg_len,
+                                                          const u32 * __restrict__ dist, const u32 * __restrict__ succ, const u32 * __restrict__ sid_all,
+                                                          const u32 * __restrict__ cum_all, const u32 * __restrict__ nsplit_dev) {
     __shared__ u32 c[257];
+    const u32 g = ub_job_of_splitters(b, blockIdx.x);
+    const u32 * __restrict__ cum = cum_all + 257 * g;
     for (int k = threadIdx.x; k < 257; k += UB_BLOCK) c[k] = cum[k];
     __syncthreads();
-    const u32 j = blockIdx.x * UB_BLOCK + threadIdx.x;
-    if (j >= nsplit) return;
+    const u32 jl = (blockIdx.x - b.j[g].sblk0) * UB_BLOCK + threadIdx.x;
+    if (jl >= ub_guard(b, g, nsplit_dev)) return;
+    const u32 j = b.j[g].split0 + jl;
+    const u32 cap = 4u << b.j[g].log_stride;
     const u32 len = seg_len[j];
     if (len <= cap) return;
+    const u32 * __restrict__ psi = psi_all + b.j[g].row0;
+    const u32 * __restrict__ sid = sid_all + b.j[g].row0;
     if (succ[j] != sid[0]) return;
-    const u32 D = dist[sid[idx]];
+    const u32 D = dist[sid[b.j[g].idx]];
     const u32 d = dist[j];
     if (d > D) return;
-    const u32 limit = n & ~1u;
+    const u32 limit = b.j[g].n & ~1u;
+    u8 * __restrict__ out = global_ptr<u8>(b.j[g].out);
     u32 r = resume[j];
     u64 pos = (u64)D - d + cap;
     for (u32 t = cap; t < len; t++) {
@@ -173,9 +238,16 @@
     return lo;
 }
 
-__global__ void __launch_bounds__(UB_BLOCK) k_ub_tail(const u8 * __restrict__ in, const u32 * __restrict__ psi, const u32 * __restrict__ cum,
-                                                     const u32 * __restrict__ dist, const u32 * __restrict__ sid, u32 idx, u32 n, u8 * __restrict__ out) {
-    const u32 D = dist[sid[idx]];
+__global__ void __launch_bounds__(UB_BLOCK) k_ub_tail(const UbBatch b, const u32 * __restrict__ psi_all, const u32 * __restrict__ cum_all, const u32 * __restrict__ dist,
+                                                     const u32 * __restrict__ sid_all) {
+    const u32 g = blockIdx.y;
+    const u8 * __restrict__ in = global_ptr<const u8>(b.j[g].in);
+    u8 * __restrict__ out = global_ptr<u8>(b.j[g].out);
+    const u32 * __restrict__ psi = psi_all + b.j[g].row0;
+    const u32 * __restrict__ sid = sid_all + b.j[g].row0;
+    const u32 * __restrict__ cum = cum_all + 257 * g;
+    const u32 n = b.j[g].n;
+    const u32 D = dist[sid[b.j[g].idx]];
     const u32 limit = n & ~1u;
     const u32 lastc = in[0];
     const u32 E = cum[lastc];
@@ -204,64 +276,171 @@
     if (gid == 0) out[n - 1] = (u8)lastc;
 }
 
+static int ub_log_stride(u32 rows) {
+    constexpr int max_log_stride = 8;
+    int log_stride = 0;
+    while (log_stride < max_log_stride && ((u64)rows >> (log_stride + 1)) >= 65536) log_stride++;
+    return log_stride;
+}
+
+static u64 ub_floor_sum(u64 n, u64 m, u64 a, u64 b) {
+    u64 ans = 0;
+    for (;;) {
+        if (a >= m) {
+            ans += n * (n - 1) / 2 * (a / m);
+            a %= m;
+        }
+        if (b >= m) {
+            ans += n * (b / m);
+            b %= m;
+        }
+        const u64 y_max = a * n + b;
+        if (y_max < m) return ans;
+        n = y_max / m;
+        b = y_max % m;
+        const u64 t = m;
+        m = a;
+        a = t;
+    }
+}
+
+u32 unbwt_splitter_count(u32 n, u32 idx) {
+    const u32 rows = n + 1;
+    const int ls = ub_log_stride(rows);
+    if (ls == 0) return rows;
+    const u64 M = 1ull << 32, T = 1ull << (32 - ls), A = 0x9E3779B1ull;
+    const u64 ge = ub_floor_sum(rows, M, A, M - T) - ub_floor_sum(rows, M, A, 0);
+    u32 c = (u32)((u64)rows - ge);
+    if (idx <= n && (((idx * 0x9E3779B1u) >> (32 - ls)) != 0u)) c++;
+    return c;
+}
+
 size_t unbwt_workspace_bytes(u64 n) {
     const u64 splitters = n + 1 < 300000 ? n + 1 : 300000 + (n >> 7);
     return (n + 64) * 8 + radix_temp_bytes(n) + scan_temp_words(n + 1) * 4 + (splitters + 4096) * 32 + (n + (n >> 3)) * 4 + (1u << 20);
 }
 
+namespace {
+struct UbLayout {
+    UbBatch b;
+    u32 slots = 0, total = 0, sblks = 0, max_split = 0;
+    u64 max_n = 0;
+    u32 *psi = nullptr, *sid = nullptr, *hist = nullptr, *cum = nullptr, *words = nullptr;
+    u32 *split_row = nullptr, *seg_len = nullptr, *resume = nullptr, *succ[2] = {nullptr, nullptr}, *dist[2] = {nullptr, nullptr};
+    u8 * slab = nullptr;
+};
+
+void ub_layout(const UnbwtJob * jobs, int count, Arena & a, UbLayout & L) {
+    L.b.count = (u32)count;
+    L.b.pad = 0;
+    u64 slab_bytes = 0;
+    for (int g = 0; g < count; g++) {
+        UbJobArg & J = L.b.j[g];
+        J.in = dev_addr(jobs[g].d_in);
+        J.out = dev_addr(jobs[g].d_out);
+        J.n = jobs[g].n;
+        J.idx = jobs[g].idx;
+        J.log_stride = (u32)ub_log_stride(J.n + 1);
+        J.row0 = L.slots;
+        J.split0 = L.total;
+        J.sblk0 = L.sblks;
+        J.slab_off = slab_bytes;
+        const u32 ns = unbwt_splitter_count(J.n, J.idx);
+        J.nsplit = ns;
+        J.pad = 0;
+        L.slots += (u32)((((u64)J.n + 1) + UB_BLOCK - 1) / UB_BLOCK * UB_BLOCK);
+        L.total += ns;
+        L.sblks += (ns + UB_BLOCK - 1) / UB_BLOCK;
+        slab_bytes += (u64)ns * (4u << J.log_stride);
+        if (ns > L.max_split) L.max_split = ns;
+        if (J.n > L.max_n) L.max_n = J.n;
+    }
+    L.psi = a.take<u32>(L.slots);
+    L.sid = a.take<u32>(L.slots);
+    L.hist = a.take<u32>(256 * (size_t)count);
+    L.cum = a.take<u32>(257 * (size_t)count);
+    L.words = a.take<u32>(1 + (size_t)count);
+    L.split_row = a.take<u32>(L.total);
+    L.seg_len = a.take<u32>(L.total);
+    L.resume = a.take<u32>(L.total);
+    for (int k = 0; k < 2; k++) {
+        L.succ[k] = a.take<u32>(L.total);
+        L.dist[k] = a.take<u32>(L.total);
+    }
+    L.slab = a.take<u8>(slab_bytes + 64);
+}
+
+constexpr u64 UB_MAX_SLOTS = (u64)1 << 31;
+
+size_t ub_group_bytes(const UnbwtJob * jobs, int count, const Arena & tmp) {
+    Arena dry;
+    dry.base = tmp.base;
+    dry.used = 0;
+    dry.cap = ~(size_t)0 >> 1;
+    UbLayout L;
+    ub_layout(jobs, count, dry, L);
+    const size_t radix = radix_temp_bytes(L.max_n), scan = scan_temp_words(L.slots) * 4;
+    return dry.used + (radix > scan ? radix : scan) + 65536;
+}
+
+void ub_run_group(const UnbwtJob * jobs, int count, Arena & tmp, hipStream_t s) {
+    const size_t mk = tmp.mark();
+    UbLayout L;
+    ub_layout(jobs, count, tmp, L);
+    const UbBatch & b = L.b;
+    HIP_CHECK(hipMemsetAsync(L.hist, 0, 256 * 4 * (size_t)count, s));
+    for (int g = 0; g < count; g++)
+        launch(k_ub_hist, dim3((u32)(((u64)b.j[g].n + UB_BLOCK * 64 - 1) / (UB_BLOCK * 64))), dim3(UB_BLOCK), 0, s, jobs[g].d_in, b.j[g].n, L.hist + 256 * g);
+    launch(k_ub_cum, dim3((u32)count), dim3(256), 0, s, b, (const u32 *)L.hist, L.cum, L.psi);
+    for (int g = 0; g < count; g++)
+        radix_pass<u8>(jobs[g].d_in, (u8 *)nullptr, (const u32 *)nullptr, L.psi + b.j[g].row0, b.j[g].n, 0, b.j[g].idx, 1u, tmp, s);
+    const dim3 grows(L.slots / UB_BLOCK), gs(L.sblks), gt((L.total + UB_BLOCK - 1) / UB_BLOCK);
+    launch(k_ub_flags, grows, dim3(UB_BLOCK), 0, s, b, L.sid);
+    exclusive_scan_u32(L.sid, L.slots, L.words, tmp, s);
+    launch(k_ub_collect, grows, dim3(UB_BLOCK), 0, s, b, (const u32 *)L.sid, L.split_row, L.words + 1);
+    launch(k_ub_walk, gs, dim3(UB_BLOCK), 0, s, b, (const u32 *)L.psi, (const u32 *)L.sid, (const u32 *)L.split_row, (const u32 *)(L.words + 1), (const u32 *)L.cum, L.succ[0],
+           L.dist[0], L.slab, L.resume);
+    HIP_CHECK(hipMemcpyAsync(L.seg_len, L.dist[0], (size_t)L.total * 4, hipMemcpyDeviceToDevice, s));
+    int cur = 0;
+    for (u64 span = 1; span < L.max_split; span <<= 1) {
+        launch(k_ub_jump, gt, dim3(UB_BLOCK), 0, s, (const u32 *)L.succ[cur], (const u32 *)L.dist[cur], (const u32 *)L.words, L.total, L.succ[cur ^ 1], L.dist[cur ^ 1]);
+        cur ^= 1;
+    }
+    launch(k_ub_place, dim3(L.sblks * 16u), dim3(UB_BLOCK), 0, s, b, (const u8 *)L.slab, (const u32 *)L.seg_len, (const u32 *)L.dist[cur], (const u32 *)L.succ[cur],
+           (const u32 *)L.sid, (const u32 *)(L.words + 1));
+    launch(k_ub_walk_long, gs, dim3(UB_BLOCK), 0, s, b, (const u32 *)L.psi, (const u32 *)L.resume, (const u32 *)L.seg_len, (const u32 *)L.dist[cur], (const u32 *)L.succ[cur],
+           (const u32 *)L.sid, (const u32 *)L.cum, (const u32 *)(L.words + 1));
+    launch(k_ub_tail, dim3(256, (u32)count), dim3(UB_BLOCK), 0, s, b, (const u32 *)L.psi, (const u32 *)L.cum, (const u32 *)L.dist[cur], (const u32 *)L.sid);
+    tmp.release(mk);
+}
+}
+
+void bwt_inverse_batch(const UnbwtJob * jobs, int count, Arena & tmp, hipStream_t s) {
+    UnbwtJob group[UB_MAX_JOBS];
+    int k = 0;
+    while (k < count) {
+        int m = 0;
+        u64 slots = 0;
+        for (; k < count && m < UB_MAX_JOBS; k++) {
+            const UnbwtJob & j = jobs[k];
+            if (j.n == 0) continue;
+            if (j.n == 1) {
+                HIP_CHECK(hipMemcpyAsync(j.d_out, j.d_in, 1, hipMemcpyDeviceToDevice, s));
+                continue;
+            }
+            group[m] = j;
+            const u64 sl = slots + ((u64)j.n + 1 + UB_BLOCK - 1) / UB_BLOCK * UB_BLOCK;
+            if (m > 0 && (sl > UB_MAX_SLOTS || ub_group_bytes(group, m + 1, tmp) > tmp.cap - tmp.used)) break;
+            slots = sl;
+            m++;
+        }
+        if (m) ub_run_group(group, m, tmp, s);
+    }
+}
+
 void bwt_inverse(const u8 * d_in, u32 n, u32 idx, u8 * d_out, Arena & tmp, hipStream_t s) {
-    if (n == 0) return;
-    if (n == 1) {
-        HIP_CHECK(hipMemcpyAsync(d_out, d_in, 1, hipMemcpyDeviceToDevice, s));
-        return;
-    }
-    const size_t mk = tmp.mark();
-    const u32 rows = n + 1;
-    u32 * psi = tmp.take<u32>(rows);
-    u32 * sid = tmp.take<u32>(rows);
-    u32 * hist = tmp.take<u32>(256);
-    u32 * cum = tmp.take<u32>(257);
-    u32 * d_total = tmp.take<u32>(1);
-
-    HIP_CHECK(hipMemsetAsync(hist, 0, 256 * 4, s));
-    launch(k_ub_hist, dim3((u32)(((u64)n + UB_BLOCK * 64 - 1) / (UB_BLOCK * 64))), dim3(UB_BLOCK), 0, s, d_in, n, hist);
-    launch(k_ub_cum, dim3(1), dim3(256), 0, s, (const u32 *)hist, cum, psi, idx);
-    radix_pass<u8>(d_in, (u8 *)nullptr, (const u32 *)nullptr, psi, n, 0, idx, 1u, tmp, s);
-
-    constexpr int max_log_stride = 8;
-    int log_stride = 0;
-    while (log_stride < max_log_stride && ((u64)rows >> (log_stride + 1)) >= 65536) log_stride++;
-    const dim3 grows((rows + UB_BLOCK - 1) / UB_BLOCK);
-    launch(k_ub_flags, grows, dim3(UB_BLOCK), 0, s, rows, idx, log_stride, sid);
-    exclusive_scan_u32(sid, rows, d_total, tmp, s);
-    u32 nsplit = 0;
-    HIP_CHECK(hipMemcpyAsync(&nsplit, d_total, 4, hipMemcpyDeviceToHost, s));
-    HIP_CHECK(hipStreamSynchronize(s));
-    u32 * split_row = tmp.take<u32>(nsplit);
-    u32 * seg_len = tmp.take<u32>(nsplit);
-    u32 * resume = tmp.take<u32>(nsplit);
-    u32 * succ[2] = {tmp.take<u32>(nsplit), tmp.take<u32>(nsplit)};
-    u32 * dist[2] = {tmp.take<u32>(nsplit), tmp.take<u32>(nsplit)};
-    const u32 cap = 4u << log_stride;
-    u8 * slab = tmp.take<u8>((size_t)nsplit * cap + 64);
-    const dim3 gs((nsplit + UB_BLOCK - 1) / UB_BLOCK);
-    launch(k_ub_collect, grows, dim3(UB_BLOCK), 0, s, rows, idx, log_stride, (const u32 *)sid, split_row);
-    launch(k_ub_walk, gs, dim3(UB_BLOCK), 0, s, (const u32 *)psi, (const u32 *)sid, (const u32 *)split_row, nsplit, idx, log_stride, rows, (const u32 *)cum, cap, succ[0],
-           dist[0], slab, resume);
-    HIP_CHECK(hipMemcpyAsync(seg_len, dist[0], (size_t)nsplit * 4, hipMemcpyDeviceToDevice, s));
-
-    int cur = 0;
-    for (u64 span = 1; span < nsplit; span <<= 1) {
-        launch(k_ub_jump, gs, dim3(UB_BLOCK), 0, s, (const u32 *)succ[cur], (const u32 *)dist[cur], nsplit, succ[cur ^ 1], dist[cur ^ 1]);
-        cur ^= 1;
-    }
-    launch(k_ub_place, dim3((u32)(((u64)nsplit * 16 + UB_BLOCK - 1) / UB_BLOCK)), dim3(UB_BLOCK), 0, s, (const u8 *)slab, (const u32 *)seg_len, (const u32 *)dist[cur],
-           (const u32 *)succ[cur], (const u32 *)sid, idx, cap, nsplit, n, d_out);
-    launch(k_ub_walk_long, gs, dim3(UB_BLOCK), 0, s, (const u32 *)psi, (const u32 *)resume, (const u32 *)seg_len, (const u32 *)dist[cur], (const u32 *)succ[cur],
-           (const u32 *)sid, idx, (const u32 *)cum, cap, nsplit, n, d_out);
-    launch(k_ub_tail, dim3(256), dim3(UB_BLOCK), 0, s, d_in, (const u32 *)psi, (const u32 *)cum, (const u32 *)dist[cur], (const u32 *)sid, idx, n, d_out);
-    HIP_CHECK(hipStreamSynchronize(s));
-    tmp.release(mk);
-}
-
-}
+    const UnbwtJob j{d_in, n, idx, d_out};
+    bwt_inverse_batch(&j, 1, tmp, s);
+}
+
+}
diff --git a/include/bz3_hip.h b/include/bz3_hip.h
--- a/include/bz3_hip.h
+++ b/include/bz3_hip.h
@@ -14,6 +14,10 @@
 BZIP3_API int bz3_hip_state_device(struct bz3_state * state);
 
 BZIP3_API int bz3_hip_set_cm_mode(int mode);
+BZIP3_API int bz3_hip_set_unbwt_group(int blocks);
+BZIP3_API int bz3_hip_debug_unbwt_group(size_t free_bytes, size_t have, size_t base, size_t ring, size_t unit, size_t block_bytes, size_t headroom, int forced);
+BZIP3_API size_t bz3_hip_debug_unbwt_workspace(size_t n);
+BZIP3_API uint32_t bz3_hip_debug_unbwt_splitters(uint32_t n, uint32_t idx);
 BZIP3_API void bz3_hip_debug_bwt_big_rounds(int k);
 BZIP3_API unsigned bz3_hip_cm_blocks_given_up(void);
 BZIP3_API unsigned bz3_hip_cm_blocks_routed_full(void);
@@ -107,6 +111,7 @@
 BZIP3_API int32_t bz3_hip_stage_lzp_decode(const uint8_t * in, int32_t n, uint8_t * out, int32_t max);
 BZIP3_API int32_t bz3_hip_stage_bwt(const uint8_t * in, uint8_t * out, int32_t n);
 BZIP3_API int32_t bz3_hip_stage_unbwt(const uint8_t * in, uint8_t * out, int32_t n, int32_t idx);
+BZIP3_API int32_t bz3_hip_stage_unbwt_many(const uint8_t * const * ins, uint8_t * const * outs, const int32_t * ns, const int32_t * idxs, int32_t count);
 BZIP3_API int32_t bz3_hip_debug_cu_masks(int cus, int reserve, uint32_t * side, uint32_t * rest);
 BZIP3_API int32_t bz3_hip_debug_scan_u32(uint32_t * data, uint32_t n, uint32_t * total);
 BZIP3_API int32_t bz3_hip_debug_sort_u32(const uint32_t * keys, uint32_t n, int key_bits, int digit_bits, uint32_t * sorted_keys, uint32_t * sorted_index);
```

Result: no change. 639.6, median of 6 (+0.7%).
